# ChristophReich1996/Multi-StyleGAN

Hardware: AMD Instinct MI355X
Metric: training images/sec (G+D step, 256^2, seq=3x2ch) (higher is better)
Workload: dtype bf16

## Files before the change

### include/msg_hip.h

```cpp
#ifndef MSG_HIP_H
#define MSG_HIP_H

#ifdef __cplusplus
extern "C" {
#endif

enum { MSG_OK = 0, MSG_EINVAL = -1, MSG_EUNSUPPORTED = -2, MSG_ELAUNCH = -3 };
enum { MSG_F32 = 0, MSG_BF16 = 1, MSG_F16 = 2, MSG_F64 = 3, MSG_F32_SPLIT = 4 };

#define MSG_ABI_VERSION 5
int msg_abi_version(void);
const char* msg_build_arch(void);
const char* msg_strerror(int code);

int msg_upfirdn2d(const void* x, const float* fir, void* y, int dtype,
                  int major, int in_h, int in_w, int minor, int kh, int kw,
                  int up_x, int up_y, int down_x, int down_y,
                  int pad_x0, int pad_x1, int pad_y0, int pad_y1, void* stream);

int msg_upfirdn2d_pitched(const void* x, const float* fir, void* y, int dtype,
                          int major, int in_h, int in_w, int minor, int in_pitch, int kh, int kw,
                          int up_x, int up_y, int down_x, int down_y,
                          int pad_x0, int pad_x1, int pad_y0, int pad_y1, void* stream);

int msg_upfirdn2d_pitched2(const void* x, const float* fir, void* y, int dtype,
                           int major, int in_h, int in_w, int minor, int in_pitch, int out_pitch, int kh, int kw,
                           int up_x, int up_y, int down_x, int down_y,
                           int pad_x0, int pad_x1, int pad_y0, int pad_y1, void* stream);

int msg_upfirdn2d_separable(const void* x, const float* fir_y, const float* fir_x, void* y, int dtype,
                            int major, int in_h, int in_w, int minor, int kh, int kw,
                            int pad_x0, int pad_x1, int pad_y0, int pad_y1, void* stream);

int msg_upfirdn2d_separable_act(const void* x, const float* fir_y, const float* fir_x, void* y, int dtype,
                                int major, int in_h, int in_w, int minor, int kh, int kw,
                                int pad_x0, int pad_x1, int pad_y0, int pad_y1,
                                const float* act_bias, const float* noise, const float* noise_weight,
                                int noise_batch, float alpha, float scale, void* stream);
int msg_upfirdn2d_separable_act_mask(const void* x, const float* fir_y, const float* fir_x, void* y, int dtype,
                                     int major, int in_h, int in_w, int minor, int kh, int kw,
                                     int pad_x0, int pad_x1, int pad_y0, int pad_y1,
                                     const float* act_bias, const float* noise, const float* noise_weight,
                                     int noise_batch, float alpha, float scale, unsigned char* mask, void* stream);

int msg_fused_bias_act(const void* x, const float* bias, const void* ref, void* y, int dtype,
                       long long size_x, int step_b, int size_b,
                       const float* noise, const float* noise_weight, int noise_batch, int pix,
                       int act, int grad, float alpha, float scale, void* stream);

long long msg_bias_act_backward_workspace(long long size_x, int step_b, int size_b, int has_noise);
int msg_bias_act_backward(const void* gy, const void* out, void* gx, int dtype,
                          long long size_x, int step_b, int size_b,
                          float* grad_bias, const float* noise, float* grad_noise_weight,
                          int noise_batch, int pix, float alpha, float scale,
                          float* ws, long long ws_floats, void* stream);
int msg_channel_sums(const void* x, float* sums, int dtype, long long size_x, int C, float* ws, long long ws_floats,
                     void* stream);
int msg_bias_act_backward_mask(const void* gy, const unsigned char* mask, int tile_m, int tile_n, void* gx, int dtype,
                               long long size_x, int size_b,
                               float* grad_bias, const float* noise, float* grad_noise_weight,
                               int noise_batch, int pix, float alpha, float scale,
                               float* ws, long long ws_floats, void* stream);
int msg_sum_rows(const float* part, float* out, long long rows, int cols, void* stream);
int msg_bias_act_backward_mask_head(const void* gy, const void* ghead, const float* whead, const float* style,
                                    float wscale, int n_head, const unsigned char* mask, int tile_m, int tile_n,
                                    void* gx, int dtype, long long size_x, int size_b,
                                    float* grad_bias, const float* noise, float* grad_noise_weight,
                                    int noise_batch, int pix, float alpha, float scale,
                                    float* ws, long long ws_floats, void* stream);

int msg_conv2d_fprop(const void* x, const void* w, const float* bias, void* y, int dtype,
                     int B, int IH, int IW, int Cx, int Ck, int OH, int OW, int N, int ldy,
                     int kh, int kw, int stride, int pad, int in_up, int pixel_shuffle,
                     long long w_batch_stride, void* stream);
enum { MSG_WGRAD_K_AUTO = -1 };
int msg_conv2d_wgrad(const void* gy, const void* x, float* gw, int dtype,
                     int B, int IH, int IW, int Cx, int I, int OH, int OW, int ldgy, int O, int ldgw,
                     int kh, int kw, int stride, int pad, int pixel_shuffle,
                     int per_sample, int k_chunks, int oi_major, float gain,
                     float* ws, long long ws_floats, void* stream);
long long msg_conv2d_wgrad_workspace(int dtype, int B, int IH, int IW, int Cx, int I, int OH, int OW, int ldgy,
                                     int O, int ldgw, int kh, int kw, int stride, int pad, int pixel_shuffle,
                                     int per_sample, int k_chunks);

int msg_demod_coeff(const float* W, const float* s, float* d, int B, int O, int I, int taps,
                    float scale, float eps, void* stream);
int msg_scale_rows_cols(const float* base, const float* rowscale, const float* colscale, void* out,
                        int dtype, int B, int R, int T, int C, int Ck, float gain, void* stream);
int msg_modulate_weights(const float* base, const float* wsq, const float* style, void* out, float* d_out,
                         int dtype, int B, int R, int O, int T, int C, int Ck, float scale, float eps, void* stream);
int msg_modulate_backward(const float* gwk, const float* W, const float* s, const float* d, float* gW,
                          float* gs_part, int B, int O, int I, int taps, int ldg, int o_group,
                          float scale, void* stream);
int msg_scale_rows_cols2(const float* base, const float* row1, const float* col1, const float* row2, const float* col2,
                         void* out, int dtype, int B, int R, int T, int C, int Ck, float gain, void* stream);
int msg_modulate_backward2(const float* gwk, const float* W, const float* s, const float* d, const float* v,
                           float* gW, float* gs_part, int B, int O, int I, int taps, int ldg, int o_group,
                           float scale, void* stream);

int msg_relayout_weight(const float* w, void* fwd, void* dgrad, float* wsq, int dtype,
                        int O, int I, int T, int Ck, int Ok, int flip, int t_major, float gain, void* stream);

int msg_gather_taps(const void* x, void* y, int dtype, int B, int H, int W, int Cx, int C, int kh, int kw,
                    int pad, int Ko, void* stream);
int msg_fold_taps(const void* g, const void* add, void* gx, int dtype, int B, int H, int W, int Ko, int C, int kh, int kw,
                  int pad, int ldx, int ld_add, void* stream);

int msg_scaled_add(const void* a, const void* b, void* y, int dtype, long long n, float beta, float gain, void* stream);
int msg_rgb_skip_merge(const void* conv, int dtype, int ld, const float* bias, const float* skip, const float* fir,
                       float* out, int B, int C, int H, int W, void* stream);
int msg_rgb_skip_merge_backward(const float* g, void* g_conv, int dtype, int ld, float* g_skip, const float* fir,
                                int B, int C, int H, int W, void* stream);
int msg_gamma_merge(const void* a, const void* b, const float* gamma, void* y, int dtype, long long n, float gain, void* stream);
long long msg_gamma_merge_backward_workspace(void);
int msg_gamma_merge_backward(const void* gy, const void* a, const float* gamma, void* ga, void* gb, float* g_gamma, int dtype,
                             long long n, float gain, float* ws, void* stream);
int msg_scaled_add_rows(const void* a, const void* b, void* y, int dtype, long long rows, int cols,
                        long long lda, long long ldb, long long ldy, float beta, float gain, void* stream);

int msg_softmax_rows(const void* x, void* y, int dtype, long long rows, int cols, void* stream);
int msg_softmax_rows_backward(const void* y, const void* gy, void* gx, int dtype, long long rows, int cols,
                              void* stream);
int msg_softmax_rows_backward2(const void* y, const void* gy, const void* v, void* d_y, void* d_gy, int dtype,
                               long long rows, int cols, void* stream);

int msg_nonlocal_attention_supported(int B, int Nq, int Nk, int dk, int dv);
int msg_nonlocal_attention_fwd(const void* q, const void* k, const void* vt, void* o, float* lse, int dtype,
                               int B, int Nq, int Nk, int dk, int dv, void* stream);
int msg_maxpool2x2_fwd(const void* x, void* y, unsigned short* idx, int dtype, int B, int H, int W, int C, long long ldx,
                       void* stream);
int msg_maxpool2x2_bwd(const void* gy, const unsigned short* idx, void* gx, int dtype, int B, int H, int W, int C,
                       void* stream);
int msg_maxpool2x2_gather(const void* v, const unsigned short* idx, void* out, int dtype, int B, int H, int W, int C,
                          long long ldv, void* stream);

int msg_nonlocal_attention_bwd_splits(int B, int Nq, int Nk);
int msg_nonlocal_attention_bwd(const void* q, const void* qt, const void* k, const void* kt, const void* v,
                               const void* dO, const void* dOt, const void* o, const float* lse, float* delta,
                               void* dq, void* dk_out, void* dv_out, float* workspace, int dtype,
                               int B, int Nq, int Nk, int dk, int dv, void* stream);

int msg_affine_warp(const float* x, float* y, const float* angle_deg, float angle_const, const float* scale_xy,
                    const float* select_u, const float* p, int rot_prob, float cx, float cy, int padding,
                    int align_corners, int B, int C, int H, int W, int backward, void* workspace, void* stream);

long long msg_minibatch_stddev_workspace(int C, int H, int W, int groups, int dtype);
int msg_minibatch_stddev(const void* x, void* y, float* stat, float* workspace, int dtype,
                         int B, int C, int H, int W, int ldx, int ldy, int groups, float alpha, void* stream);
int msg_minibatch_stddev_backward(const void* x, const void* gy, const float* gstat, void* gx, int dtype,
                                  int B, int C, int H, int W, int ldx, int ldgy, int ldgx, int groups,
                                  float alpha, void* stream);

int msg_conv2d_fprop_act(const void* x, const void* w, void* y, int dtype,
                         int B, int IH, int IW, int Cx, int Ck, int OH, int OW, int N, int ldy,
                         int kh, int kw, int stride, int pad, long long w_batch_stride,
                         const float* act_bias, const float* noise, const float* noise_weight,
                         int noise_batch, float alpha, float scale, void* stream);
int msg_conv2d_fprop_act_mask(const void* x, const void* w, void* y, int dtype,
                              int B, int IH, int IW, int Cx, int Ck, int OH, int OW, int N, int ldy,
                              int kh, int kw, int stride, int pad, long long w_batch_stride,
                              const float* act_bias, const float* noise, const float* noise_weight,
                              int noise_batch, float alpha, float scale, unsigned char* mask, void* stream);

int msg_conv2d_fprop_residual(const void* x, const void* w, void* y, int dtype,
                              int B, int IH, int IW, int Cx, int Ck, int OH, int OW, int N, int ldy,
                              int kh, int kw, int stride, int pad, long long w_batch_stride,
                              const void* residual, int res_ld, float gain, void* stream);

int msg_conv2d_fprop_act_backward(const void* x, const void* w, void* y, int dtype,
                                  int B, int IH, int IW, int Cx, int Ck, int OH, int OW, int N, int ldy,
                                  int kh, int kw, int stride, int pad, long long w_batch_stride,
                                  const void* residual, int res_ld,
                                  const unsigned char* sign_mask, int mask_tile_m, int mask_tile_n,
                                  const void* sign_map, int sign_ld, float alpha, float scale,
                                  float* grad_bias, const float* noise, int noise_batch, float* grad_noise_weight,
                                  float* ws, long long ws_floats, void* stream);

int msg_act_pointwise_head(const void* x, const float* bias, const float* w, float* y, int dtype,
                           long long npix, int C, float wscale, float alpha, float scale, void* stream);
long long msg_act_pointwise_head_backward_workspace(long long npix, int C);
int msg_act_pointwise_head_backward(const void* x, const float* bias, const float* w, const float* gy, void* gx,
                                    float* grad_bias_and_w, int dtype, long long npix, int C, float wscale,
                                    float alpha, float scale, float* ws, long long ws_floats, void* stream);

int msg_linear_fprop(const float* x, const float* w, const float* bias, float* y, int M, int N, int K,
                     float gain, float bias_gain, void* stream);
int msg_linear_dgrad(const float* gy, const float* w, float* gx, int M, int N, int K, float gain, void* stream);
int msg_linear_wgrad(const float* gy, const float* x, float* gw, float* gb, int M, int N, int K,
                     float gain, float bias_gain, void* stream);

int msg_linear_grouped_fprop(const float* x, const int* slot, const float* const* w, const float* const* bias, float* y,
                             int G, int M, int N, int K, int L, float gain, float bias_gain, void* stream);
int msg_linear_grouped_dgrad(const float* gy, const float* const* w, float* gx, int G, int M, int N, int K, float gain,
                             void* stream);
int msg_linear_grouped_wgrad(const float* gy, const float* x, const int* slot, float* gw, float* gb, int G, int M, int N,
                             int K, int L, float gain, float bias_gain, void* stream);
int msg_linear_grouped_wgrad_ptrs(const float* gy, const float* x, const int* slot, float* const* gw, float* const* gb, int G,
                                  int M, int N, int K, int L, float gain, float bias_gain, void* stream);

enum {
    MSG_PLAN_REG = 0,
    MSG_PLAN_DMA = 1,
    MSG_PLAN_PP = 2,
    MSG_PLAN_ROW3 = 3,
    MSG_PLAN_ROW3N = 4,
    MSG_PLAN_THIN = 5,
    MSG_PLAN_UPCONV = 6,
    MSG_FPLAN_FIELDS = 5
};
int msg_conv2d_fprop_launch_plan(int dtype, int B, int IH, int IW, int Cx, int Ck, int OH, int OW, int N, int ldy,
                                 int kh, int kw, int stride, int pad, int in_up, int pixel_shuffle,
                                 long long w_batch_stride, int has_bias, int epilogue, long long* out, int n_out_fields);
enum {
    MSG_WPLAN_GENERIC = 0,
    MSG_WPLAN_DMA = 1,
    MSG_WPLAN_UNI = 2,
    MSG_WPLAN_ROW3 = 3,
    MSG_WPLAN_ROW3_W32 = 4,
    MSG_WPLAN_FIELDS = 11
};
int msg_conv2d_wgrad_plan(int dtype, int B, int IH, int IW, int Cx, int I, int OH, int OW, int ldgy,
                          int O, int ldgw, int kh, int kw, int stride, int pad, int pixel_shuffle,
                          int per_sample, int k_chunks, long long* out, int n_out_fields);
int msg_conv2d_fprop_plan(int dtype, int B, int IH, int IW, int Cx, int Ck, int OH, int OW, int N,
                          int kh, int kw, long long w_batch_stride);
long long msg_conv2d_fprop_act_backward_workspace(int dtype, int B, int IH, int IW, int Cx, int Ck, int OH, int OW,
                                                  int N, int kh, int kw, long long w_batch_stride, int has_noise);
int msg_conv2d_fprop_upconv_eligible(int B, int IH, int IW, int Cx, int Ck, int OH, int OW, int N, int kh, int kw,
                                     int stride, int pad, int in_up, int pixel_shuffle, long long w_batch_stride);
int msg_conv2d_fprop_thin_eligible(int B, int IH, int IW, int Cx, int Ck, int OH, int OW, int N, int ldy, int kh, int kw,
                                   int stride, int pad, int in_up, int pixel_shuffle, int act_mode);

int msg_flat_adam(float* param, const float* grad, float* exp_avg, float* exp_avg_sq, float* ema, long long n,
                  const float* coef, float lr, float beta1, float beta2, float eps, int step, float ema_decay,
                  void* stream);
int msg_flat_ema(float* ema, const float* param, long long n, float decay, void* stream);

long long msg_tlfm_prepare_workspace(int B, int T);
int msg_tlfm_prepare(const unsigned short* raw, const unsigned char* hflip, void* out, int dtype,
                     int B, int C, int T, int H, int W, int vflip,
                     float lo1, float div1, float lo2, float div2,
                     unsigned int* ws, void* stream);

int msg_tlfm_frame_range(const unsigned short* frames, long long N, int H, int W,
                         unsigned int* range, void* stream);
int msg_tlfm_gather(const unsigned short* frames, const unsigned int* range, long long N,
                    const int* index, const unsigned char* hflip, void* out, int dtype,
                    int B, int C, int T, int H, int W, int vflip,
                    float lo1, float div1, float lo2, float div2, void* stream);

int msg_sample_sheet(const void* seq, unsigned char* out, int dtype,
                     int B, int C, int T, int H, int W, int tints, void* stream);

enum { MSG_GAN_LOGISTIC = 0, MSG_GAN_WASSERSTEIN = 1, MSG_GAN_HINGE = 2 };
enum { MSG_GAN_AUX_NONE = 0, MSG_GAN_AUX_WEIGHT = 1, MSG_GAN_AUX_LABEL = 2 };
long long msg_gan_loss_workspace(long long n_real, long long n_fake);
int msg_gan_loss(const void* pred_real, const void* pred_fake, const float* aux, float* out, int dtype, int kind,
                 int aux_mode, long long n_real, long long n_fake, long long P, float* ws, long long ws_floats,
                 void* stream);
int msg_gan_loss_backward(const void* pred_real, const void* pred_fake, const float* aux, const float* grad_out,
                          void* grad_real, void* grad_fake, int dtype, int kind, int aux_mode,
                          long long n_real, long long n_fake, long long P, void* stream);

#define MSG_ELASTIC_MAX_SIGMA 32
long long msg_elastic_workspace(int B, int H, int W);
int msg_elastic_deform(const void* in, const float* noise, float* field, void* out, int dtype,
                       int B, int F, int H, int W, int sigma, float alpha, void* ws, void* stream);

#ifdef __cplusplus
}
#endif
#endif
```

### multi_stylegan_amd/build.py

```python
import glob
import os
import shutil
import subprocess
import sys

HERE = os.path.dirname(os.path.abspath(__file__))
CSRC = os.path.join(HERE, "csrc")
LIB = os.path.join(HERE, "libmsg_hip.so")
ARCH = "gfx950"


def _hipcc():
    return shutil.which("hipcc") or "/opt/rocm/bin/hipcc"


def sources():
    return sorted(glob.glob(os.path.join(CSRC, "*.hip")))


def lib_path(variant=None):
    return LIB if not variant else os.path.join(HERE, f"libmsg_hip_{variant}.so")


def is_stale(variant=None):
    lib = lib_path(variant)
    if not os.path.exists(lib):
        return True
    t = os.path.getmtime(lib)
    deps = sources() + glob.glob(os.path.join(CSRC, "*.h")) + [os.path.join(HERE, "..", "include", "msg_hip.h")]
    return any(os.path.getmtime(d) > t for d in deps)


def build(force=False, verbose=True, extra_flags=(), variant=None):
    lib = lib_path(variant)
    if not force and not is_stale(variant):
        build_fastcall(verbose=verbose)
        return lib
    objs = []
    objdir = os.path.join(HERE, "build" if not variant else f"build_{variant}")
    os.makedirs(objdir, exist_ok=True)
    procs = []
    for src in sources():
        obj = os.path.join(objdir, os.path.basename(src) + ".o")
        deps = [src] + glob.glob(os.path.join(CSRC, "*.h"))
        objs.append(obj)
        if not force and os.path.exists(obj) and all(os.path.getmtime(obj) > os.path.getmtime(d) for d in deps):
            continue
        cmd = [_hipcc(), "-O3", "-std=c++17", f"--offload-arch={ARCH}", "-fPIC", "-c", src, "-o", obj,
               "-Wno-unused-result", *extra_flags, *os.environ.get("MSG_EXTRA_HIPCC_FLAGS", "").split()]
        if verbose:
            print(" ".join(cmd), flush=True)
        procs.append((src, subprocess.Popen(cmd)))
    for src, pr in procs:
        if pr.wait() != 0:
            raise RuntimeError(f"hipcc failed on {src}")
    cmd = [_hipcc(), "-shared", "-fPIC", f"--offload-arch={ARCH}", "-o", lib, *objs]
    if verbose:
        print(" ".join(cmd), flush=True)
    subprocess.check_call(cmd)
    build_fastcall(force=force, verbose=verbose)
    return lib


FASTCALL = os.path.join(HERE, "_msg_fastcall.so")


def build_fastcall(force=False, verbose=True):
    import sysconfig
    gen = os.path.join(HERE, "csrc_host", "gen_fastcall.py")
    deps = [gen, os.path.join(HERE, "_lib.py"), os.path.join(HERE, "..", "include", "msg_hip.h")]
    if not force and os.path.exists(FASTCALL) and all(os.path.getmtime(FASTCALL) > os.path.getmtime(d) for d in deps):
        return FASTCALL
    sys.path.insert(0, os.path.dirname(HERE))
    try:
        from multi_stylegan_amd import _lib
        from multi_stylegan_amd.csrc_host.gen_fastcall import generate
    finally:
        sys.path.pop(0)
    objdir = os.path.join(HERE, "build")
    os.makedirs(objdir, exist_ok=True)
    src = os.path.join(objdir, "msg_fastcall.c")
    with open(src, "w") as f:
        f.write(generate(_lib._SIGNATURES))
    cmd = [shutil.which("gcc") or "gcc", "-O2", "-shared", "-fPIC", f"-I{sysconfig.get_paths()['include']}", src, "-o", FASTCALL, "-ldl"]
    if verbose:
        print(" ".join(cmd), flush=True)
    subprocess.check_call(cmd)
    return FASTCALL


if __name__ == "__main__":
    import argparse
    ap = argparse.ArgumentParser()
    ap.add_argument("--force", action="store_true")
    ap.add_argument("--variant", default=None)
    ap.add_argument("--flags", default="", help="extra hipcc flags, e.g. --flags=-DMSG_TUNING")
    a = ap.parse_args()
    print(build(force=a.force, extra_flags=tuple(a.flags.split()), variant=a.variant))
```

### multi_stylegan_amd/conv_ops.py

```python
import ctypes
import functools
import math
import os
from typing import Optional, Tuple

import torch
from torch.autograd import Function

from . import _lib
from ._autograd import _derive


def _vec(dtype) -> int:
    return 8 if dtype == torch.bfloat16 else 4


def _round_up(n: int, m: int) -> int:
    return (n + m - 1) // m * m


def _padded_nhwc(b, c, h, w, dtype, device):
    cx = _round_up(c, _vec(dtype))
    buf = torch.empty((b, h, w, cx), dtype=dtype, device=device)
    if cx != c:
# ... 197 lines not shown
            offs[(ph, e - u)] = t0 + 2 * u
    dmin = min(d for _, d in offs)
    dmax = max(d for _, d in offs)
    taps = dmax - dmin + 1
    table = [[offs.get((ph, tau + dmin), -1) for tau in range(taps)] for ph in (0, 1)]
    return taps, -dmin, table


def _relay_dgrad_s2(w: torch.Tensor, dtype, pad: int) -> Tuple[torch.Tensor, int, int, int]:
    *lead, o, i, kh, kw = w.shape
    assert kh == kw
    taps, pad2, table = _s2_plan(kh, pad)
    ok = _round_up(o, 128 // (2 if dtype == torch.bfloat16 else 4))
    src = [[(table[ph][th] * kw + table[pw][tw]) if table[ph][th] >= 0 and table[pw][tw] >= 0 else kh * kw
            for th in range(taps) for tw in range(taps)] for ph in (0, 1) for pw in (0, 1)]
    idx = torch.tensor(src, dtype=torch.long, device=w.device)
    wt = w.transpose(-4, -3).reshape(*lead, i, o, kh * kw)
    wz = torch.cat([wt, wt.new_zeros((*lead, i, o, 1))], dim=-1)
    picked = wz[..., idx]
    n = len(lead)
    picked = picked.permute(*range(n), n + 2, n, n + 3, n + 1)
    out = torch.zeros((*lead, 4, i, taps * taps, ok), dtype=dtype, device=w.device)
    out[..., :o] = picked
    return out.reshape(*lead, 4 * i, taps * taps, ok), ok, taps, pad2


_WEIGHT_GENERATION = [0]


def invalidate_weight_cache(params=None) -> None:
    if params is None:
        _WEIGHT_GENERATION[0] += 1
        return
    for p in params:
        p.__dict__["_msg_gen"] = p.__dict__.get("_msg_gen", 0) + 1


def _after_optimizer_step(optimizer, *_args, **_kwargs) -> None:
    for group in optimizer.param_groups:
        invalidate_weight_cache(group["params"])


def _stamp(w):
    return (w._version, _WEIGHT_GENERATION[0], w.__dict__.get("_msg_gen", 0), w.data_ptr())


from torch.optim.optimizer import register_optimizer_step_post_hook as _register_step_hook

_register_step_hook(_after_optimizer_step)


def _cached(w, tag, dtype, wscale, build):
    if not isinstance(w, torch.nn.Parameter):
        out = build()
        return (out[0] * wscale, *out[1:]) if wscale != 1.0 else out
    store = w.__dict__.setdefault("_msg_relay", {})
    key = (tag, dtype, wscale)
    stamp = _stamp(w)
    hit = store.get(key)
    if hit is not None and hit[0] == stamp:
        return hit[1]
    with torch.no_grad():
        out = build()
        if wscale != 1.0:
            out = (out[0] * wscale, *out[1:])
    store[key] = (stamp, out)
    return out


def _param_images(w, dtype, gain, kind, modulation=False):
    key = ("img", dtype, gain, kind, modulation)
    store = w.__dict__.get("_msg_relay")
    if store is not None:
        hit = store.get(key)
        if hit is not None and hit[0] == (w._version, _WEIGHT_GENERATION[0], w.__dict__.get("_msg_gen", 0), w.data_ptr()):
            return hit[1]
    if not (isinstance(w, torch.nn.Parameter) and w.is_cuda and w.dtype == torch.float32):
        return None
    o, i = _oi(w)
    t = w.numel() // (o * i)
    if t > 16 or w.numel() != o * i * t:
        return None
    store = w.__dict__.setdefault("_msg_relay", {})
    stamp = _stamp(w)
    dev = w.device
    unit = 1 if modulation else 128 // (2 if dtype == torch.bfloat16 else 4)
    ck, ok = _round_up(i, unit), _round_up(o, unit)
    up2 = kind == "up2"
    with torch.no_grad():
        w3 = w.detach().reshape(o, i, t).contiguous()
        fwd = torch.empty((t * o, 1, ck) if up2 else (o, t, ck), dtype=dtype, device=dev)
        dgr = torch.empty((i, t, ok), dtype=dtype, device=dev)
        wsq = torch.empty((o, i), dtype=torch.float32, device=dev) if modulation else None
        with _lib.on_device(dev):
            code = _lib.lib().msg_relayout_weight(w3.data_ptr(), fwd.data_ptr(), dgr.data_ptr(), _lib.ptr(wsq),
                                                  _lib.dtype_code(fwd), o, i, t, ck, ok, int(not up2), int(up2),
                                                  float(gain), _lib.stream_of(dev))
        _lib.check(code, "msg_relayout_weight")
    out = {"f": (fwd, ck), "d": (dgr, ok), "wsq": wsq}
    store[key] = (stamp, out)
    return out


_CLOCK_SHAPES = bool(int(os.environ.get("MSG_CLOCK_SHAPES", "0")))

FP32_CONTRACTION = "exact"
MSG_F32_SPLIT = _lib.MSG_F32_SPLIT
_SPLIT_CODES = {"split_bf16x3": MSG_F32_SPLIT}


class fp32_contraction:

    def __init__(self, mode: str):
        if mode not in ("exact", "split_bf16x3"):
            raise ValueError(f"fp32 contraction mode {mode!r}: 'exact' or 'split_bf16x3'")
        self.mode, self.prev = mode, None

    def __enter__(self):
        global FP32_CONTRACTION
        self.prev, FP32_CONTRACTION = FP32_CONTRACTION, self.mode
        return self

    def __exit__(self, *exc):
        global FP32_CONTRACTION
        FP32_CONTRACTION = self.prev
        return False

    @staticmethod
    def set(mode: str) -> None:
        fp32_contraction(mode).__enter__()


def _contraction_code(t: torch.Tensor, mode: Optional[str] = None) -> int:
    code = _lib.dtype_code(t)
    mode = FP32_CONTRACTION if mode is None else mode
    return _SPLIT_CODES[mode] if (code == _lib.MSG_F32 and mode != "exact") else code


_PLANS = {_lib.MSG_PLAN_REG: ("conv_fprop_reg", None), _lib.MSG_PLAN_DMA: ("conv_fprop_dma", None),
          _lib.MSG_PLAN_PP: ("conv_fprop_pp", None), _lib.MSG_PLAN_ROW3: ("conv_fprop_row3", 256),
          _lib.MSG_PLAN_ROW3N: ("conv_fprop_row3n", 128), _lib.MSG_PLAN_THIN: ("conv_fprop_thin", None),
          _lib.MSG_PLAN_UPCONV: ("conv_fprop_upconv", None)}


@functools.lru_cache(maxsize=None)
def _fprop_plan(*args):
    out = (ctypes.c_longlong * _lib.MSG_FPLAN_FIELDS)()
    ok = _lib.lib().msg_conv2d_fprop_launch_plan(*args, ctypes.addressof(out), len(out)) == _lib.MSG_OK
    kernel = out[0] if ok else None
    return (kernel,) + _PLANS.get(kernel, ("conv_fprop", None)) + (out[3] * args[8], out[4])


@functools.lru_cache(maxsize=None)
def _wgrad_plan(*geom):
    out = (ctypes.c_longlong * _lib.MSG_WPLAN_FIELDS)()
    _lib.check(_lib.lib().msg_conv2d_wgrad_plan(*geom, _lib.MSG_WGRAD_K_AUTO, ctypes.addressof(out), len(out)),
               "msg_conv2d_wgrad_plan")
    return out[10], out[1]


def _launch_fprop(x, wk, ck, bias, n, out_hw, kh, kw, stride, pad, in_up, pixel_shuffle, per_sample, c_real,
                  flops=None, act=None, residual=None, out=None, mode=None):
    dev = _lib.require_gpu(x, wk, bias)
    xv, cx = _nhwc_view(x)
    b, _, ih, iw = xv.shape
    oh, ow = out_hw
    if out is not None:
        y, ldy = _nhwc_view(out)
        if y is not out or pixel_shuffle or out.shape != (b, n, oh, ow) or out.dtype != x.dtype or n % _vec(x.dtype):
            raise _lib.MsgHipError(f"conv fprop: destination {tuple(out.shape)} / {out.stride()} for a {(b, n, oh, ow)} result")
    elif pixel_shuffle:
        y, ldy = _alloc_out(b, n // 4, 2 * oh, 2 * ow, x.dtype, dev)
    else:
        y, ldy = _alloc_out(b, n, oh, ow, x.dtype, dev)
    rows_needed = n * (1 if pixel_shuffle else kh * kw) * ck
    if per_sample:
        ws_ = wk.stride() if wk.ndim == 4 else None
        if ws_ is None or wk.shape[0] != b or ws_[0] < rows_needed or ws_[3] != 1 or \
                (wk.shape[2] > 1 and ws_[2] != wk.shape[3]) or (wk.shape[1] > 1 and ws_[1] != wk.shape[2] * wk.shape[3]):
            raise _lib.MsgHipError(f"conv fprop: per-sample weight image {tuple(wk.shape)} for batch {b}, {n} x {kh * kw} x {ck}")
    elif wk.numel() < rows_needed or not wk.is_contiguous():
        raise _lib.MsgHipError(f"conv fprop: weight image {tuple(wk.shape)} smaller than {n} x {kh * kw} x {ck}")
    wstride = wk.stride(0) if per_sample else 0
    if flops is None:
        flops = 2.0 * b * oh * ow * n * kh * kw * c_real / (in_up * in_up)
    key, sign_tile = "conv_fprop", None
    sign_holder = act[5] if act is not None and len(act) > 5 else None
    if _lib.kernel_clock.enabled or sign_holder is not None:
        _, key, sign_tile, _, _ = _fprop_plan(_lib.dtype_code(x), b, ih, iw, cx, ck, oh, ow, n, ldy, kh, kw, stride, pad, in_up,
                                              int(pixel_shuffle), wstride, int(bias is not None),
                                              2 if residual is not None else int(act is not None))
    if _lib.kernel_clock.enabled and _CLOCK_SHAPES:
        key += f"|B{b} {ih}x{iw}->{oh}x{ow} {c_real}->{n} {kh}x{kw} s{stride} up{in_up}" \
               f"{' ps' if pixel_shuffle else ''}{' per-sample' if per_sample else ''}|"
    with _lib.on_device(dev), _lib.kernel_clock.span((key, 'bf16' if x.dtype == torch.bfloat16 else 'f32'), flops):
        if residual is not None:
            assert bias is None and act is None and in_up == 1 and not pixel_shuffle
            rv, res_ld = _nhwc_view(residual[0])
            assert rv.shape == (b, n, oh, ow) and rv.dtype == x.dtype
            code = _lib.lib().msg_conv2d_fprop_residual(
                xv.data_ptr(), wk.data_ptr(), y.data_ptr(), _contraction_code(x, mode), b, ih, iw, cx, ck, oh, ow, n, ldy, kh, kw,
                stride, pad, wstride, rv.data_ptr(), res_ld, float(residual[1]), _lib.stream_of(dev))
        elif act is None:
            code = _lib.lib().msg_conv2d_fprop(
                xv.data_ptr(), wk.data_ptr(), _lib.ptr(bias), y.data_ptr(), _contraction_code(x, mode), b, ih, iw, cx, ck, oh,
                ow, n, ldy, kh, kw, stride, pad, in_up, int(pixel_shuffle), wstride, _lib.stream_of(dev))
        else:
            assert bias is None and in_up == 1 and not pixel_shuffle
            act_bias, noise, noise_w, alpha, scale = act[:5]
            _lib.require_gpu(x, act_bias, noise, noise_w)
            mask = None
            if sign_holder is not None and sign_tile:
                from .op_static.fused_act import sign_mask_for
                mask = sign_mask_for(b, n, oh, ow, x.dtype, dev)
                if mask is not None:
                    sign_holder.append((mask, sign_tile, sign_tile))
            code = _lib.lib().msg_conv2d_fprop_act_mask(
                xv.data_ptr(), wk.data_ptr(), y.data_ptr(), _contraction_code(x, mode), b, ih, iw, cx, ck, oh, ow, n, ldy, kh, kw,
                stride, pad, wstride, _lib.ptr(act_bias), _lib.ptr(noise), _lib.ptr(noise_w),
                1 if noise is None else noise.shape[0], float(alpha), float(scale), _lib.ptr(mask), _lib.stream_of(dev))
    _lib.check(code, "msg_conv2d_fprop")
    return y


def _grad_dest(param):
    if param is None or "_msg_grad_slot" not in getattr(param, "__dict__", ()):
        return None
    from .dist import grad_destination
    return grad_destination(param)


def _launch_wgrad(gy, x, o, i, kh, kw, stride, pad, pixel_shuffle, per_sample, low_hw, raw=False, gain=1.0, out=None,
                  mode=None):
    dev = _lib.require_gpu(gy, x)
    gv, ldgy = _nhwc_view(gy)
    xv, cx = _nhwc_view(x)
    b, _, ih, iw = xv.shape
    oh, ow = low_hw if pixel_shuffle else gv.shape[2:]
    taps = kh * kw
    ldgw = _round_up(i, 4)
    geom = (_contraction_code(x, mode), b, ih, iw, cx, i, oh, ow, ldgy, o, ldgw, kh, kw, stride, pad, int(pixel_shuffle),
            int(per_sample))
    need, nz = _wgrad_plan(*geom)
    ws = _lib.scratch_ptr(need, dev) if need else None
    if per_sample or raw:
        out = None
    oi_major = (bool(need) or out is not None) and not per_sample and not raw
    if oi_major:
        gw = out.view(o, i, kh, kw) if out is not None else torch.empty((o, i, kh, kw), dtype=torch.float32, device=dev)
    elif per_sample:
        gw = torch.empty((b, o, taps, ldgw), dtype=torch.float32, device=dev)
    else:
        gw = torch.empty((o, taps, ldgw), dtype=torch.float32, device=dev)
    flops = 2.0 * b * oh * ow * o * i * taps
    key = "conv_wgrad"
    if _CLOCK_SHAPES and _lib.kernel_clock.enabled:
        key += f"|B{b} {ih}x{iw}->{oh}x{ow} {i}->{o} {kh}x{kw} s{stride}{' ps' if pixel_shuffle else ''}" \
               f"{' per-sample' if per_sample else ' shared'}{f' slabs{nz}' if need else ''}|"
    with _lib.on_device(dev), _lib.kernel_clock.span((key, 'bf16' if x.dtype == torch.bfloat16 else 'f32'), flops):
        code = _lib.lib().msg_conv2d_wgrad(
            gv.data_ptr(), xv.data_ptr(), gw.data_ptr(), *geom, _lib.MSG_WGRAD_K_AUTO, int(oi_major), float(gain), ws, need,
            _lib.stream_of(dev))
    _lib.check(code, "msg_conv2d_wgrad")
    if raw:
        return gw, ldgw
    if oi_major:
        return gw
    lead = gw.shape[:-2]
    return gw.view(*lead, kh, kw, ldgw)[..., :i].permute(*range(len(lead)), len(lead) + 2, len(lead), len(lead) + 1)


class Geometry:
    __slots__ = ("kind", "kh", "kw", "stride", "pad", "x_hw", "y_hw", "per_sample", "wscale", "mode")

    def __init__(self, kind, kh, kw, stride, pad, x_hw, per_sample, wscale=1.0, mode=None):
        self.kind, self.kh, self.kw, self.stride, self.pad = kind, kh, kw, stride, pad
        self.x_hw, self.per_sample, self.wscale = tuple(x_hw), per_sample, float(wscale)
        self.mode = FP32_CONTRACTION if mode is None else mode
        if kind == "up2":
            self.y_hw = (2 * x_hw[0], 2 * x_hw[1])
        else:
            self.y_hw = ((x_hw[0] + 2 * pad - kh) // stride + 1, (x_hw[1] + 2 * pad - kw) // stride + 1)


def _oi(w):
    return (w.shape[0], w.shape[1]) if w.ndim == 2 else (w.shape[-4], w.shape[-3])


def _relay_fwd_kind(w, dtype, kind):
    wk, ck = _relay_fwd(w, dtype)
    if kind == "up2":
        o = _oi(w)[0]
        wk = wk.transpose(-3, -2).reshape(*wk.shape[:-3], 4 * o, 1, ck).contiguous()
    return wk, ck


def _thin_ok(dtype, i, g: Geometry) -> bool:
    taps = g.kh * g.kw
    return g.kind == "conv" and g.stride == 1 and not g.per_sample and taps > 1 and \
        2 * g.pad + 1 == g.kh and g.kh == g.kw and i * taps <= 128 // (2 if dtype == torch.bfloat16 else 4)


def _gather_taps(x, i, g: Geometry):
    dev = _lib.require_gpu(x)
    xv, cx = _nhwc_view(x)
    b, _, h, w = xv.shape
    ko = 128 // x.element_size()
    out = torch.empty((b, h, w, ko), dtype=x.dtype, device=dev)
    with _lib.on_device(dev):
        code = _lib.lib().msg_gather_taps(xv.data_ptr(), out.data_ptr(), _lib.dtype_code(x), b, h, w, cx, i, g.kh, g.kw,
                                          g.pad, ko, _lib.stream_of(dev))
    _lib.check(code, "msg_gather_taps")
    return out.permute(0, 3, 1, 2), ko


def _relay_thin(w, dtype):
    o, i, kh, kw = w.shape
    ko = 128 // (2 if dtype == torch.bfloat16 else 4)
    out = torch.zeros((o, 1, ko), dtype=dtype, device=w.device)
    out[:, 0, :kh * kw * i] = w.permute(0, 2, 3, 1).reshape(o, kh * kw * i)
    return out, ko


def _f_raw(x, w, bias, g: Geometry, act=None, residual=None, out=None):
    if w.ndim == 4 and _thin_ok(x.dtype, w.shape[1], g):
        xc, ko = _gather_taps(x, w.shape[1], g)
        wk, _ = _cached(w, "thin", x.dtype, g.wscale, lambda: _relay_thin(w, x.dtype))
        return _launch_fprop(xc, wk, ko, bias, w.shape[0], g.y_hw, 1, 1, 1, 0, 1, False, False,
                             w.shape[1] * g.kh * g.kw, act=act, residual=residual, out=out, mode=g.mode)
    if g.kind == "up2" and _oi(w)[0] % _vec(x.dtype):
        o_real = _oi(w)[0]
        wp = torch.zeros((*w.shape[:-4], _round_up(o_real, _vec(x.dtype)), *w.shape[-3:]), dtype=w.dtype, device=w.device)
        wp[..., :o_real, :, :, :] = w.detach()
        assert out is None
        return _f_raw(x, wp, bias, g, act=act, residual=residual)[:, :o_real]
    img = _param_images(w, x.dtype, g.wscale, g.kind) if not g.per_sample else None
    wk, ck = img["f"] if img is not None else \
        _cached(w, "f" + g.kind, x.dtype, g.wscale, lambda: _relay_fwd_kind(w, x.dtype, g.kind))
    o, _ = _oi(w)
    if g.kind == "up2":
        assert out is None
        return _launch_fprop(x, wk, ck, None, 4 * o, g.x_hw, 1, 1, 1, 0, 1, True, g.per_sample, _oi(w)[1], mode=g.mode)
    return _launch_fprop(x, wk, ck, bias, o, g.y_hw, g.kh, g.kw, g.stride, g.pad, 1, False, g.per_sample, _oi(w)[1],
                         act=act, residual=residual, out=out, mode=g.mode)


def _act_operands(bias, noise, noise_w, y_shape):
    b32 = None if bias is None else bias.detach().to(torch.float32).contiguous()
    nz = nw = None
    if noise is not None:
        if noise.shape[0] not in (1, y_shape[0]) or noise.shape[1] != 1 or tuple(noise.shape[2:]) != tuple(y_shape[2:]):
            raise _lib.MsgHipError(f"noise shape {tuple(noise.shape)} does not match output {tuple(y_shape)}")
        nz = noise.detach().to(torch.float32).contiguous()
        nw = noise_w.detach().to(torch.float32).contiguous()
    return b32, nz, nw


ACT_BACKWARD_IN_DGRAD = bool(int(os.environ.get("MSG_ACT_BACKWARD_IN_DGRAD", "1")))


class ActHandle:
    __slots__ = ("armed", "sign", "alpha", "scale", "bias_param", "has_bias", "noise", "done")

    def __init__(self):
        self.armed, self.sign, self.done = False, None, None
        self.alpha = self.scale = 0.0
        self.bias_param, self.has_bias, self.noise = None, False, None

    def arm(self, y, mask, alpha, scale, bias_param, has_bias, noise):
        if not ACT_BACKWARD_IN_DGRAD or y.dtype != torch.bfloat16 or not y.is_cuda:
            return
        self.sign = ("mask",) + tuple(mask) if mask is not None else ("map",)
        self.alpha, self.scale = float(alpha), float(scale)
# ... 278 lines not shown
        y = _f_raw(x, w, None, g, act=(b32, nz, nw, alpha, scale, holder))
        ctx.mask = holder[0] if holder else None
        ctx.slot, ctx.out_scale = slot, out_scale
        ctx.act_handle = ctx.input_act = None
        if act_handle is not None and out_scale is None and noise is None and holder is not None:
            act_handle.arm(y, ctx.mask, alpha, scale, act_bias, act_bias is not None, None)
            ctx.act_handle = act_handle if act_handle.armed else None
        if input_act is not None and input_act.armed:
            ctx.input_act = input_act
        ctx.bias_param = act_bias
        ctx.g, ctx.cfg = g, (alpha, scale, act_bias is not None, noise is not None)
        ctx.nw_shape = None if noise_w is None else noise_w.shape
        ctx.save_for_backward(x, w, y, noise)
        return y

    @staticmethod
    def backward(ctx, gy):
        from .op_static.fused_act import FusedLeakyReLUFunctionBackward
        x, w, y, noise = ctx.saved_tensors
        alpha, scale, has_bias, has_noise = ctx.cfg
        g = ctx.g
        owed = 1.0
        if ctx.out_scale is not None and ctx.out_scale.pending is not None:
            owed, ctx.out_scale.pending = ctx.out_scale.pending, None
        handed = ctx.act_handle.done if ctx.act_handle is not None else None
        if handed is not None:
            ctx.act_handle.done = None
            gpre, (gb, gnw) = gy, handed
        else:
            gpre, gb, gnw = _derive(FusedLeakyReLUFunctionBackward, gy, y, noise if has_noise else None,
                                    ctx.bias_param if has_bias else False, alpha, scale * owed, ctx.mask)
        gx = None
        if ctx.needs_input_grad[0]:
            other = ctx.slot.g if ctx.slot is not None else None
            pre = ctx.input_act if not torch.is_grad_enabled() else None
            if _dgrad_add_ok(other, x.shape, gpre.dtype, g):
                gx = _derive(_ConvD, gpre, w, g, other) if torch.is_grad_enabled() else \
                    _d_raw(gpre, w, g, residual=(other, 1.0), act_bwd=pre, sign_map=x)
                ctx.slot.merged = True
            elif pre is not None:
                gx = _d_raw(gpre, w, g, act_bwd=pre, sign_map=x)
            else:
                gx = _derive(_ConvD, gpre, w, g)
        gw = _derive(_ConvG, gpre, x, _oi(w), w.ndim, g, w) if _consumed(ctx, 1, 1) else None
        return gx, gw, (gb if has_bias and ctx.needs_input_grad[2] else None), None, \
            (gnw.reshape(ctx.nw_shape) if has_noise and ctx.needs_input_grad[4] else None), None, None, None, None, None, None, None


class _ConvResidualF(Function):

    @staticmethod
    def forward(ctx, x, w, main, g, gain, fork, slot=None, main_scale=None, out=None):
        y = _f_raw(x, w, None, g, residual=(main, gain), out=out)
        if out is not None:
            y = out.view_as(out)
        ctx.slot, ctx.main_scale = slot, main_scale
        ctx.g, ctx.gain, ctx.fork = g, float(gain), fork
        ctx.save_for_backward(x, w)
        return (y, y.view_as(y)) if fork else y

    @staticmethod
    def backward(ctx, *grads):
        from .op_static.fused_act import _ScaledAddRows, _rows_ok
        x, w = ctx.saved_tensors
        g1 = grads[0]
        g2 = grads[1] if ctx.fork else None
        if (g1 is None or g2 is None) and ctx.main_scale is not None and ctx.needs_input_grad[2]:
            gs = g1 if g1 is not None else g2
            ctx.main_scale.pending = ctx.gain
            gg = Geometry(ctx.g.kind, ctx.g.kh, ctx.g.kw, ctx.g.stride, ctx.g.pad, ctx.g.x_hw, ctx.g.per_sample,
                          ctx.g.wscale * ctx.gain, mode=ctx.g.mode)
            gs_main = gs
            if torch.is_grad_enabled() and ctx.needs_input_grad[0] and RESIDUAL_FORK_NODE:
                gx, gs_main = _ConvDFork.apply(gs, w, gg)
            else:
                gx = _derive(_ConvD, gs, w, gg) if ctx.needs_input_grad[0] else None
            if ctx.slot is not None and gx is not None:
                ctx.slot.g = gx
            gw = _derive(_ConvG, gs, x, _oi(w), w.ndim, gg, w) if _consumed(ctx, 1, 1) else None
            return gx, gw, gs_main, None, None, None, None, None, None
        if g1 is None or g2 is None:
            gs = (g1 if g1 is not None else g2) * ctx.gain
        elif _rows_ok(g1, g2):
            gs = _derive(_ScaledAddRows, g1, g2, ctx.gain)
        else:
            gs = (g1 + g2) * ctx.gain
        gx = _derive(_ConvD, gs, w, ctx.g) if ctx.needs_input_grad[0] else None
        if ctx.slot is not None and gx is not None:
            ctx.slot.g = gx
        gw = _derive(_ConvG, gs, x, _oi(w), w.ndim, ctx.g, w) if _consumed(ctx, 1, 1) else None
        return gx, gw, (gs if ctx.needs_input_grad[2] else None), None, None, None, None, None, None


class _MultiConvF(Function):

    @staticmethod
    def forward(ctx, x, geoms, *weights):
        ctx.geoms = geoms
        ctx.save_for_backward(x, *weights)
        return tuple(_f_raw(x, w, None, g) for w, g in zip(weights, geoms))

    @staticmethod
    def backward(ctx, *grads):
        x, *weights = ctx.saved_tensors
        second_order = torch.is_grad_enabled()
        gx, gws = None, []
        for k, (gy, w, g) in enumerate(zip(grads, weights, ctx.geoms)):
            if gy is None:
                gws.append(None)
                continue
            if ctx.needs_input_grad[0]:
                if gx is None or not _dgrad_add_ok(gx, x.shape, gy.dtype, g):
                    part = _derive(_ConvD, gy, w, g)
                    gx = part if gx is None else gx + part
                elif second_order:
                    gx = _derive(_ConvD, gy, w, g, gx)
                else:
                    gx = _d_raw(gy, w, g, residual=(gx, 1.0))
            gws.append(_derive(_ConvG, gy, x, _oi(w), w.ndim, g, w) if _consumed(ctx, 2 + k, 1 + k) else None)
        return (gx, None, *gws)


def conv2d_shared_input(x, weights_and_scales, padding=0):
    p = _square(padding, "padding")
    geoms = tuple(Geometry("conv", w.shape[2], w.shape[3], 1, p, x.shape[2:], False, ws) for w, ws in weights_and_scales)
    return _MultiConvF.apply(x, geoms, *[w for w, _ in weights_and_scales])


class GradScale:
    __slots__ = ("pending",)

    def __init__(self):
        self.pending = None


class GradSlot:
    __slots__ = ("g", "merged")

    def __init__(self):
        self.g, self.merged = None, False


class HeadGradSlot:
    __slots__ = ("head", "dgrad", "armed")

    def __init__(self):
        self.head = None
        self.dgrad = None
        self.armed = False

    def take(self):
        head, dgrad, self.head, self.dgrad = self.head, self.dgrad, None, None
        return head, dgrad


class _ForkInput(Function):

    @staticmethod
    def forward(ctx, x, slot):
        ctx.slot = slot
        return x.view_as(x), x.view_as(x)

    @staticmethod
    def backward(ctx, g_main, g_res):
        slot = ctx.slot
        merged, slot.g, slot.merged = slot.merged, None, False
        if merged or g_res is None:
            return g_main, None
        if g_main is None:
            return g_res, None
        return g_main + g_res, None


def _square(value, what: str) -> int:
    if isinstance(value, int):
        return value
    value = tuple(value)
    if len(value) != 2 or value[0] != value[1]:
        raise _lib.MsgHipError(f"conv2d: only square {what} is implemented, got {value}")
    return int(value[0])


def fork_input(x, slot: GradSlot):
    return _ForkInput.apply(x, slot)


def conv2d_add_residual(x, weight, main, gain, stride=1, padding=0, wscale=1.0, fork=False, grad_slot=None,
                        main_grad_scale=None, out=None):
    s, p = _square(stride, "stride"), _square(padding, "padding")
    g = Geometry("conv", weight.shape[2], weight.shape[3], s, p, x.shape[2:], False, wscale)
    return _ConvResidualF.apply(x, weight, main, g, float(gain), bool(fork), grad_slot, main_grad_scale, out)


def conv2d_bias_act(x, weight, act_bias, stride=1, padding=0, wscale=1.0, negative_slope=0.2, scale=1.0,
                    grad_slot=None, out_grad_scale=None, act_handle=None, input_act=None):
    s, p = _square(stride, "stride"), _square(padding, "padding")
    g = Geometry("conv", weight.shape[2], weight.shape[3], s, p, x.shape[2:], False, wscale)
    return _ConvActF.apply(x, weight, act_bias, None, None, g, float(negative_slope), float(scale), grad_slot,
                           out_grad_scale, act_handle, input_act)


def conv2d(x, weight, bias=None, stride=1, padding=0, wscale=1.0):
    s, p = _square(stride, "stride"), _square(padding, "padding")
    g = Geometry("conv", weight.shape[2], weight.shape[3], s, p, x.shape[2:], False, wscale)
    return _ConvF.apply(x, weight, None if bias is None else bias.float(), g)


def conv_transpose2d_2x2(x, weight, bias=None, wscale=1.0):
    if tuple(weight.shape[2:]) != (2, 2):
        raise _lib.MsgHipError("conv_transpose2d_2x2: 2x2 kernel, stride 2, padding 0 only")
    g = Geometry("up2", 2, 2, 1, 1, x.shape[2:], False, wscale)
    y = _ConvF.apply(x, weight.transpose(0, 1), None, g)
    return y if bias is None else y + bias.view(1, -1, 1, 1).to(y.dtype)


_LINEAR_MAX_ROWS = 256


def _lin_call(name, flops, *args):
    dev = args[0].device
    with _lib.on_device(dev), _lib.kernel_clock.span((name, "f32"), flops):
        code = getattr(_lib.lib(), f"msg_{name}")(*[a.data_ptr() if isinstance(a, torch.Tensor) else
                                                   (0 if a is None else a) for a in args], _lib.stream_of(dev))
    _lib.check(code, f"msg_{name}")


def _dense32(*ts):
    for t in ts:
        if t is not None and t.dtype != torch.float32:
            raise _lib.MsgHipError("the few-row linear kernels are fp32 (mapping network / style affines / heads)")
    return [None if t is None else t.contiguous() for t in ts]


class _LinF(Function):

    @staticmethod
    def forward(ctx, x, w, bias, gain, bias_gain=1.0):
        _lib.require_gpu(x, w, bias)
        x, w, bias = _dense32(x, w, bias)
        (m, k), n = x.shape, w.shape[0]
        y = torch.empty((m, n), dtype=torch.float32, device=x.device)
        _lin_call("linear_fprop", 2.0 * m * n * k, x, w, bias, y, m, n, k, float(gain), float(bias_gain))
        ctx.save_for_backward(x, w)
        ctx.gain, ctx.has_bias, ctx.bias_gain = float(gain), bias is not None, float(bias_gain)
        ctx.bias_param = bias
        return y

    @staticmethod
    def backward(ctx, gy):
        x, w = ctx.saved_tensors
        need_x, need_w, need_b = ctx.needs_input_grad[:3]
        gx = _derive(_LinD, gy, w, ctx.gain) if need_x else None
        gw = gb = None
        if need_w and need_b and ctx.has_bias and not torch.is_grad_enabled():
            (gy_,) = _dense32(gy)
            (m, n), k = gy_.shape, x.shape[1]
            gw, gb = _grad_dest(w), _grad_dest(ctx.bias_param)
            gw = gw if gw is not None else torch.empty((n, k), dtype=torch.float32, device=x.device)
            gb = gb if gb is not None else torch.empty((n,), dtype=torch.float32, device=x.device)
            _lin_call("linear_wgrad", 2.0 * m * n * k, gy_, x, gw, gb, m, n, k, ctx.gain, ctx.bias_gain)
        else:
            if need_w:
                gw = _derive(_LinG, gy, x, ctx.gain)
            if need_b and ctx.has_bias:
                gb = gy.sum(dim=0) if ctx.bias_gain == 1.0 else gy.sum(dim=0) * ctx.bias_gain
        return gx, gw, gb, None, None


class _LinD(Function):

    @staticmethod
    def forward(ctx, gy, w, gain):
        _lib.require_gpu(gy, w)
        gy, w = _dense32(gy, w)
        (m, n), k = gy.shape, w.shape[1]
        gx = torch.empty((m, k), dtype=torch.float32, device=gy.device)
        _lin_call("linear_dgrad", 2.0 * m * n * k, gy, w, gx, m, n, k, float(gain))
        ctx.save_for_backward(gy, w)
        ctx.gain = float(gain)
        return gx

    @staticmethod
    def backward(ctx, g):
        gy, w = ctx.saved_tensors
        d_gy = _derive(_LinF, g, w, None, ctx.gain) if ctx.needs_input_grad[0] else None
        d_w = _derive(_LinG, gy, g, ctx.gain) if ctx.needs_input_grad[1] else None
        return d_gy, d_w, None


class _LinG(Function):

    @staticmethod
    def forward(ctx, gy, x, gain):
        _lib.require_gpu(gy, x)
        gy, x = _dense32(gy, x)
        (m, n), k = gy.shape, x.shape[1]
        gw = torch.empty((n, k), dtype=torch.float32, device=gy.device)
        _lin_call("linear_wgrad", 2.0 * m * n * k, gy, x, gw, None, m, n, k, float(gain), 1.0)
        ctx.save_for_backward(gy, x)
        ctx.gain = float(gain)
        return gw

    @staticmethod
    def backward(ctx, g):
        gy, x = ctx.saved_tensors
        d_gy = _derive(_LinF, x, g, None, ctx.gain) if ctx.needs_input_grad[0] else None
# ... 262 lines not shown
    if upsample:
        return _launch_wgrad(gy, x, o, i, 2, 2, 1, 0, True, True, g.x_hw, raw=True, mode=g.mode)
    return _launch_wgrad(gy, x, o, i, kh, kw, 1, kh // 2, False, True, None, raw=True, mode=g.mode)


def _fold_weight_gradient(gwk, ldg, w3, s, dd, scale, style_dtype, cotangent=None, dest=None):
    b = gwk.shape[0]
    o, i, t = w3.shape
    dev = gwk.device
    og = 2 if o >= 512 or o < 256 else 1
    groups = (o + og - 1) // og
    out = _grad_dest(dest) if cotangent is None else None
    gw3 = out.view(o, i, t) if out is not None else torch.empty((o, i, t), dtype=torch.float32, device=dev)
    gs_part = _lib.scratch_ptr(groups * b * i, dev)
    gs = torch.empty((b, i), dtype=torch.float32, device=dev)
    with _lib.on_device(dev):
        st = _lib.stream_of(dev)
        if cotangent is None:
            code = _lib.lib().msg_modulate_backward(gwk.data_ptr(), w3.data_ptr(), s.data_ptr(), _lib.ptr(dd),
                                                    gw3.data_ptr(), gs_part, b, o, i, t, ldg, og, scale, st)
        else:
            code = _lib.lib().msg_modulate_backward2(gwk.data_ptr(), w3.data_ptr(), s.data_ptr(), _lib.ptr(dd),
                                                     cotangent.data_ptr(), gw3.data_ptr(), gs_part, b, o, i, t,
                                                     ldg, og, scale, st)
        _lib.check(code, "msg_modulate_backward" + ("2" if cotangent is not None else ""))
        code = _lib.lib().msg_sum_rows(gs_part, gs.data_ptr(), groups, b * i, st)
    _lib.check(code, "msg_sum_rows")
    return (out if out is not None else gw3), (gs if style_dtype == torch.float32 else gs.to(style_dtype))


def _modconv_backward(x, weight, style, d, gy, demodulate, upsample, g, scale, need, keep_gwk=False, direct=False,
                      act_bwd=None):
    _, o, i, kh, kw = weight.shape
    b, t = x.shape[0], kh * kw
    dev = x.device
    w3 = weight.detach().reshape(o, i, t)
    s = style.detach().float().contiguous()
    dd = d if demodulate else None
    esz = 2 if gy.dtype == torch.bfloat16 else 4
    gx = None
    if need[0]:
        okp = _round_up(o, 128 // esz)
        wd = torch.empty((b, i, t, okp), dtype=gy.dtype, device=dev)
        _scale_rows_cols(_dgrad_image_base(weight, w3, upsample, g.kind), s, dd, wd, scale)
        gx = _dgrad_modconv(gy, wd, okp, o, i, kh, kw, upsample, g, act_bwd=act_bwd, sign_map=x)
    gw = gs = gwk = None
    if need[1] or need[2]:
        gwk, ldg = _wgrad_modconv(gy, x, o, i, kh, kw, upsample, g)
        gw3, gs = _fold_weight_gradient(gwk, ldg, w3, s, dd, scale, style.dtype, dest=weight if direct else None)
        gw = gw3.reshape(1, o, i, kh, kw)
    return (gx, gw, gs, gwk) if keep_gwk else (gx, gw, gs)


_NATIVE_SECOND_ORDER = True


def _modconv_second_order_composite(gy, x, weight, style, demodulate, upsample, a, cot_w, cot_s, want):
    with torch.enable_grad():
        leaves = [t.detach().requires_grad_(True) for t in (gy, x, weight, style)]
        y2 = _modulated_composite(leaves[1], leaves[2], leaves[3], demodulate, upsample)
        first = torch.autograd.grad(y2, leaves[1:], leaves[0], create_graph=True, allow_unused=True)
        terms = [(c.to(f.dtype) * f).sum() for c, f in zip((a, cot_w, cot_s), first) if c is not None and f is not None]
        if not terms:
            return (None, None, None, None)
        grads = torch.autograd.grad(sum(terms), leaves, allow_unused=True)
    return tuple(gr if w else None for gr, w in zip(grads, want))


class _ModConvGrad(Function):

    @staticmethod
    def forward(ctx, gy, x, weight, style, d, demodulate, upsample, g, scale, need):
        gx, gw, gs, gwk = _modconv_backward(x, weight, style, d, gy, demodulate, upsample, g, scale, need, keep_gwk=True)
        ctx.set_materialize_grads(False)
        ctx.save_for_backward(gy, x, weight, style, d, gwk)
        ctx.cfg = (demodulate, upsample, g, scale)
        return gx, gw, gs

    @staticmethod
    @torch.autograd.function.once_differentiable
    def backward(ctx, a, cot_w, cot_s):
        gy, x, weight, style, d, gwk = ctx.saved_tensors
        demodulate, upsample, g, scale = ctx.cfg
        want = ctx.needs_input_grad[:4]
        _, o, i, kh, kw = weight.shape
        b, t = x.shape[0], kh * kw
        tail = (None,) * 6
        if a is None and cot_w is None and cot_s is None:
            return (None, None, None, None) + tail
        if cot_w is not None or i % 4 or i > 512 or t not in (1, 4, 9) or b > _MODCONV_BWD_BATCH or \
                (cot_s is not None and gwk is None):
            return _modconv_second_order_composite(gy, x, weight, style, demodulate, upsample, a, cot_w, cot_s, want) + tail
        dev = x.device
        w3 = weight.detach().reshape(o, i, t)
        s = style.detach().float().contiguous()
        dd = d if demodulate else None
        esz = 2 if gy.dtype == torch.bfloat16 else 4
        ck, okp = _round_up(i, 128 // esz), _round_up(o, 128 // esz)
        rows = t * o if upsample else o
        ggy = gx2 = gw3 = gs2 = None
        if a is not None:
            a = a.to(x.dtype)
            if want[0]:
                wk = torch.empty((b, rows, 1 if upsample else t, ck), dtype=x.dtype, device=dev)
                base = _fwd_image_base(weight, w3, upsample, g.kind)
                if demodulate:
                    _scale_rows_cols(base, d.repeat(1, t) if upsample else d, s, wk, scale)
                else:
                    _scale_rows_cols(base, None, s, wk, scale)
                ggy = _fprop_modconv(a, wk, ck, o, i, kh, kw, upsample, g)
            if want[2] or want[3]:
                gwk_a, ldg = _wgrad_modconv(gy, a, o, i, kh, kw, upsample, g)
                gw3, gs2 = _fold_weight_gradient(gwk_a, ldg, w3, s, dd, scale, style.dtype)
        if cot_s is not None:
            v = cot_s.detach().float().contiguous()
            if want[0] or want[1]:
                hf = torch.empty((b, rows, 1 if upsample else t, ck), dtype=x.dtype, device=dev)
                hd = torch.empty((b, i, t, okp), dtype=gy.dtype, device=dev)
                base_f = _fwd_image_base(weight, w3, upsample, g.kind)
                base_d = _dgrad_image_base(weight, w3, upsample, g.kind)
                if demodulate:
                    wsq = _tap_square_sums(weight, w3, g.kind)
                    ddir = -(scale * scale) * d.pow(3) * linear(s * v, wsq)
                    rows_d, rows_dd = (d.repeat(1, t), ddir.repeat(1, t)) if upsample else (d, ddir)
                    with _lib.on_device(dev):
                        lib, st = _lib.lib(), _lib.stream_of(dev)
                        code = lib.msg_scale_rows_cols2(base_f.data_ptr(), rows_d.contiguous().data_ptr(), v.data_ptr(),
                                                        rows_dd.contiguous().data_ptr(), s.data_ptr(), hf.data_ptr(),
                                                        _lib.dtype_code(hf), b, rows, 1 if upsample else t, i, ck, scale, st)
                        _lib.check(code, "msg_scale_rows_cols2")
                        code = lib.msg_scale_rows_cols2(base_d.data_ptr(), v.data_ptr(), d.data_ptr(), s.data_ptr(),
                                                        ddir.contiguous().data_ptr(), hd.data_ptr(), _lib.dtype_code(hd), b, i, t,
                                                        o, okp, scale, st)
                        _lib.check(code, "msg_scale_rows_cols2")
                else:
                    _scale_rows_cols(base_f, None, v, hf, scale)
                    _scale_rows_cols(base_d, v, None, hd, scale)
                if want[0]:
                    ggy = _fprop_modconv(x, hf, ck, o, i, kh, kw, upsample, g, add_to=ggy)
                if want[1]:
                    gx2 = _dgrad_modconv(gy, hd, okp, o, i, kh, kw, upsample, g)
            if want[2] or want[3]:
                gw3b, gs2b = _fold_weight_gradient(gwk, gwk.shape[-1], w3, s, dd, scale, style.dtype, cotangent=v)
                gw3 = gw3b if gw3 is None else gw3 + gw3b
                gs2 = gs2b if gs2 is None else gs2 + gs2b
        gw = gw3.reshape(1, o, i, kh, kw) if (gw3 is not None and want[2]) else None
        return (ggy, gx2, gw, gs2 if want[3] else None) + tail


class _ModulatedConv(Function):

    @staticmethod
    def forward(ctx, x, weight, style, demodulate, upsample, act_bias=None, noise=None, noise_w=None, alpha=0.2,
                act_scale=1.0, fuse_act=False, head_slot=None, input_act=None):
        dev = _lib.require_gpu(x, weight, style)
        ctx.input_act = input_act if input_act is not None and input_act.armed else None
        ctx.head_slot = head_slot
        if head_slot is not None and fuse_act:
            ctx.set_materialize_grads(False)
            head_slot.armed = True
        _, o, i, kh, kw = weight.shape
        b, t = x.shape[0], kh * kw
        scale = math.sqrt(2.0) / math.sqrt(i * t)
        w3 = weight.detach().reshape(o, i, t)
        s = style.detach().float().contiguous()
        d = None
        esz = 2 if x.dtype == torch.bfloat16 else 4
        ck = _round_up(i, 128 // esz)
        kind = "up2" if upsample else "conv"
        img = _param_images(weight, torch.float32, 1.0, kind, modulation=True)
        base = img["f"][0] if img is not None else _cached(weight, "mb" + kind, torch.float32, 1.0, lambda: (
            (w3.permute(2, 0, 1).reshape(t * o, 1, i) if upsample else w3.transpose(1, 2)).contiguous(), 0))[0]
        rows = t * o if upsample else o
        wk = torch.empty((b, rows, 1 if upsample else t, ck), dtype=x.dtype, device=dev)
        if demodulate:
            wsq = img["wsq"] if img is not None else \
                _cached(weight, "wsq", torch.float32, 1.0, lambda: (w3.square().sum(dim=2).contiguous(), 0))[0]
            d = torch.empty((b, o), dtype=torch.float32, device=dev)
            with _lib.on_device(dev):
                code = _lib.lib().msg_modulate_weights(base.data_ptr(), wsq.data_ptr(), s.data_ptr(), wk.data_ptr(),
                                                       d.data_ptr(), _lib.dtype_code(wk), b, rows, o,
                                                       1 if upsample else t, i, ck, scale, 1e-8, _lib.stream_of(dev))
            _lib.check(code, "msg_modulate_weights")
        else:
            _scale_rows_cols(base, None, s, wk, scale)
        g = Geometry(kind, kh, kw, 1, kh // 2, x.shape[2:], True)
        act = None
        holder = [] if any(ctx.needs_input_grad) else None
        if fuse_act:
            assert not upsample, "the upsampling layers blur before their activation"
            act = (*_act_operands(act_bias, noise, noise_w, (b, o, *g.y_hw)), alpha, act_scale, holder)
        if upsample:
            y = _launch_fprop(x, wk, ck, None, 4 * o, g.x_hw, 1, 1, 1, 0, 1, True, True, i, mode=g.mode)
        else:
            y = _launch_fprop(x, wk, ck, None, o, g.y_hw, kh, kw, 1, kh // 2, 1, False, True, i, act=act, mode=g.mode)
        ctx.save_for_backward(x, weight, style, d if d is not None else torch.empty(0, device=dev),
                              y if fuse_act else None, noise if fuse_act else None)
        ctx.cfg = (demodulate, upsample, g, scale)
        ctx.act = (alpha, act_scale, act_bias is not None, noise is not None,
                   None if noise_w is None else noise_w.shape) if fuse_act else None
        ctx.bias_param = act_bias
        ctx.mask = holder[0] if holder else None
        return y

    @staticmethod
    def backward(ctx, gy):
        x, weight, style, d, y_act, noise = ctx.saved_tensors
        demodulate, upsample, g, scale = ctx.cfg
        _, o, i, kh, kw = weight.shape
        b, t = x.shape[0], kh * kw
        need = list(ctx.needs_input_grad)
        need[1], need[2] = _consumed(ctx, 1, 1), _consumed(ctx, 2, 2)
        gb = gnw = None
        slot = ctx.head_slot
        if ctx.act is not None:
            from .op_static.fused_act import FusedLeakyReLUFunctionBackward, act_backward_with_head
            alpha, act_scale, has_bias, has_noise, nw_shape = ctx.act
            head, head_dgrad = slot.take() if slot is not None else (None, None)
            fused = None
            if head is not None:
                fused = act_backward_with_head(gy, head, y_act.shape, noise if has_noise else None,
                                               ctx.bias_param if has_bias else None, has_bias, alpha, act_scale, ctx.mask)
                if fused is None:
                    gh = head_dgrad()
                    gy = gh if gy is None else gy + gh
            if fused is not None:
                gy, gb, gnw = fused
            elif gy is None:
                return (None,) * 13
            else:
                gy, gb, gnw = _derive(FusedLeakyReLUFunctionBackward, gy, y_act, noise if has_noise else None,
                                      ctx.bias_param if has_bias else False, alpha, act_scale, ctx.mask)
            gb = gb if has_bias and need[5] else None
            gnw = gnw.reshape(nw_shape) if has_noise and need[7] else None
        tail = (None, None, gb, None, gnw, None, None, None, None, None)
        if ctx.act is None and slot is not None and slot.armed and need[0] and not torch.is_grad_enabled() and \
                fused_head_ok(gy, weight, b, demodulate, upsample):
            gyc, wt, st = gy, weight, style
            slot.head = (gyc, weight.detach().reshape(o, i).float().contiguous(), style.detach().float().contiguous(), scale)
            slot.dgrad = lambda: _modconv_backward(x, wt, st, d, gyc, demodulate, upsample, g, scale,
                                                   [True, False, False])[0]
            need[0] = False
        fused_ok = i <= 512 and t <= 9
        if torch.is_grad_enabled() and fused_ok and _NATIVE_SECOND_ORDER and b <= _MODCONV_BWD_BATCH and x.is_cuda:
            gx, gw, gs = _derive(_ModConvGrad, gy, x, weight, style, d if demodulate else None, demodulate, upsample, g, scale,
                                            tuple(need[:3]))
            return (gx, gw, gs) + tail
        if torch.is_grad_enabled() or not fused_ok:
            with torch.enable_grad():
                ins = [v for v, n in zip((x, weight, style), need[:3]) if n]
                y2 = _modulated_composite(x, weight, style, demodulate, upsample)
                grads = list(torch.autograd.grad(y2, ins, gy, create_graph=torch.is_grad_enabled(), allow_unused=True))
            out = [grads.pop(0) if n else None for n in need[:3]]
            return (out[0], out[1], out[2]) + tail
        if b > _MODCONV_BWD_BATCH:
            gxs, gws, gss = [], [], []
            for lo in range(0, b, _MODCONV_BWD_BATCH):
                hi = min(b, lo + _MODCONV_BWD_BATCH)
                cgx, cgw, cgs = _modconv_backward(x[lo:hi], weight, style[lo:hi], d[lo:hi] if demodulate else d,
                                                  gy[lo:hi], demodulate, upsample, g, scale, need)
                gxs.append(cgx); gws.append(cgw); gss.append(cgs)
            gx = torch.cat(gxs) if need[0] else None
            gw = torch.stack(gws).sum(dim=0) if gws[0] is not None else None
            gs = torch.cat(gss) if gss[0] is not None else None
            return (gx, gw, gs) + tail
        gx, gw, gs = _modconv_backward(x, weight, style, d, gy, demodulate, upsample, g, scale, need, direct=True,
                                       act_bwd=ctx.input_act)
        return (gx, gw, gs) + tail


def fused_head_ok(gy, weight, b, demodulate, upsample) -> bool:
    _, o, _, kh, kw = weight.shape
    return gy is not None and gy.is_cuda and gy.dtype == torch.bfloat16 and kh == 1 and kw == 1 and o <= 8 and \
        not demodulate and not upsample and b <= _MODCONV_BWD_BATCH and HEAD_GRAD_FUSION


HEAD_GRAD_FUSION = bool(int(os.environ.get("MSG_HEAD_GRAD_FUSION", "1")))


def modulated_conv2d_bias_act(x, weight, style, demodulate, act_bias, noise, noise_weight, negative_slope=0.2,
                              scale=1.0, head_slot=None, input_act=None):
    return _ModulatedConv.apply(x, weight, style, bool(demodulate), False, act_bias, noise, noise_weight,
                                float(negative_slope), float(scale), True, head_slot, input_act)


def modulated_conv2d(x, weight, style, demodulate, upsample, head_slot=None):
    if head_slot is None:
        return _ModulatedConv.apply(x, weight, style, bool(demodulate), bool(upsample))
    return _ModulatedConv.apply(x, weight, style, bool(demodulate), bool(upsample), None, None, None, 0.2, 1.0, False,
                                head_slot)
```

### multi_stylegan_amd/csrc/conv_dispatch.h

```cpp
#pragma once
#include "msg_common.h"

struct ConvProblem {
    int dtype;
    int split;
    int B, IH, IW, Cx, Ck, OH, OW, N, ldy;
    int kh, kw, stride, pad, in_up, pixel_shuffle;
    long long w_batch_stride;

    bool per_sample() const { return w_batch_stride != 0; }
    int samples() const { return per_sample() ? B : 1; }
    long long mtot() const { return per_sample() ? (long long)OH * OW : (long long)B * OH * OW; }
    int esz() const { return dtype == MSG_BF16 ? 2 : 4; }
    long long x_bstride() const { return (long long)IH * IW * Cx; }
    long long y_bstride() const { return (pixel_shuffle ? 4ll : 1ll) * OH * OW * ldy; }
    long long x_bytes() const { return (long long)(per_sample() ? 1 : B) * IH * IW * Cx * esz(); }
    long long w_bytes() const { return (long long)N * kh * kw * Ck * esz(); }
    bool fits31() const { return x_bytes() < 0x7ffffff0ll && w_bytes() < 0x7ffffff0ll; }
};

enum ConvKernel {
    CONV_THIN_N, CONV_THIN_K,
    CONV_UPCONV,
    CONV_ROW3, CONV_ROW3N,
    CONV_PP,
    CONV_DMA, CONV_REG, CONV_REG_LEAN, CONV_REG_SPLIT
};

struct ConvPlan {
    ConvKernel kernel;
    int tile_m, tile_n;
    bool supported;
};

inline int conv_act_mode(const ActEpilogue* act) { return act ? act->enabled : 0; }

template <typename P>
inline void conv_fill_common(P& p, const ConvProblem& q, const ActEpilogue* act) {
    p.B = q.B; p.IH = q.IH; p.IW = q.IW; p.Cx = q.Cx; p.Ck = q.Ck; p.OH = q.OH; p.OW = q.OW; p.N = q.N; p.ldy = q.ldy;
    p.per_sample = q.per_sample();
    if (act) p.act = *act;
    p.x_bstride = q.x_bstride();
    p.w_bstride = q.w_batch_stride;
    p.y_bstride = q.y_bstride();
    p.Mtot = (int)q.mtot();
}
template <typename P>
inline void conv_fill_taps(P& p, const ConvProblem& q) {
    p.kh = q.kh; p.kw = q.kw; p.stride = q.stride; p.pad = q.pad; p.in_up = q.in_up; p.pixel_shuffle = q.pixel_shuffle;
}

ConvPlan conv_fprop_select(const ConvProblem& q, const ActEpilogue* act, bool has_bias);

bool conv_thin_eligible(const ConvProblem& q, const ActEpilogue* act, ConvPlan* plan);
void conv_thin_launch(const ConvProblem& q, const ConvPlan& plan, const void* x, const void* w, const float* bias, void* y,
                      const ActEpilogue* act, void* stream);
bool conv_upconv_eligible(const ConvProblem& q, const ActEpilogue* act, bool has_bias, ConvPlan* plan);
void conv_upconv_launch(const ConvProblem& q, const ConvPlan& plan, const void* x, const void* w, void* y, void* stream);
bool conv_row3_eligible(const ConvProblem& q, const ActEpilogue* act, bool has_bias, ConvPlan* plan);
void conv_row3_launch(const ConvProblem& q, const ConvPlan& plan, const void* x, const void* w, const float* bias, void* y,
                      const ActEpilogue* act, void* stream);
bool conv_pp_eligible(const ConvProblem& q, ConvPlan* plan);
void conv_pp_launch(const ConvProblem& q, const ConvPlan& plan, const void* x, const void* w, const float* bias, void* y,
                    const ActEpilogue* act, void* stream);

struct WgradProblem {
    int dtype, split;
    int B, IH, IW, Cx, I, OH, OW, ldgy, O, ldgw;
    int kh, kw, stride, pad, pixel_shuffle;
    int per_sample, k_chunks, oi_major;
    float gain;
    int esz() const { return dtype == MSG_BF16 ? 2 : 4; }
    long long gy_bytes() const { return (long long)(pixel_shuffle ? 4 : 1) * OH * OW * ldgy * esz(); }
    long long x_bytes() const { return (long long)IH * IW * Cx * esz(); }
    long long slab() const { return (long long)O * kh * kw * ldgw; }
    long long gw_zstride() const { return oi_major ? (long long)O * I * kh * kw : slab(); }
};

enum WgradKernel {
    WGRAD_GENERIC, WGRAD_DMA, WGRAD_UNI,
    WGRAD_ROW3, WGRAD_ROW3_W32
};

struct WgradPlan {
    WgradKernel kernel;
    int nz, slice_pixels;
    int chunks_per_out, n_out;
    int OWv, OHv;
    int fold, xcd_slices;
    long long blocks, need;
    bool supported;
};

struct WgradSplitModel { int round_wgs, fixed_steps, slab_steps; long long max_chunks, max_wgs; bool by8; };
inline long long conv_wgrad_ksplit(long long steps, long long wgs, const WgradSplitModel& m) {
    long long chunks = 1, best = -1;
    for (long long c = 1; c <= m.max_chunks; c += (m.by8 && c >= 8 ? 8 : 1)) {
        if (m.by8 && c > 1 && c < 8) continue;
        const long long rounds = (wgs * c + m.round_wgs - 1) / m.round_wgs;
        const long long cost = rounds * ((steps + c - 1) / c + m.fixed_steps + (c > 1 ? m.slab_steps : 0));
        if (best < 0 || cost < best) { best = cost; chunks = c; }
        if (wgs * c > m.max_wgs) break;
    }
    return chunks;
}

inline int conv_wgrad_default_chunks(const WgradProblem& q) {
    const long long kp = q.dtype == MSG_BF16 ? 64 : 32, npix = (long long)q.OH * q.OW;
    long long tiles = (long long)((q.O + 127ll) / 128) * ((q.I + 127ll) / 128);
    for (const int n : {q.kh, q.kw, q.B}) tiles = tiles < 1024 ? tiles * n : 1024;
    if (q.per_sample) {
        if (tiles >= 256) return 1;
        return (int)std::max(1ll, std::min(npix / (16 * kp), 1024 / tiles));
    }
    long long chunks = std::max(1ll, std::min((npix + 4 * kp - 1) / (4 * kp), (1024 + tiles - 1) / tiles));
    while (q.B * chunks > 65535) --chunks;
    return (int)chunks;
}

WgradPlan conv_wgrad_select(const WgradProblem& q);
bool conv_wgrad_row3_eligible(const WgradProblem& q, WgradPlan* plan);
void conv_wgrad_row3_launch(const WgradProblem& q, const WgradPlan& plan, const void* gy, const void* x, float* gw, float* ws,
                            void* stream);
```

### multi_stylegan_amd/csrc/conv_fprop.hip

```cpp
#include "conv_dispatch.h"
#include <stdlib.h>

typedef __bf16 bf16v8 __attribute__((ext_vector_type(8)));
typedef const __attribute__((address_space(1))) char* gptr_t;
typedef const __attribute__((address_space(1))) u32x4* gvec_t;
typedef __attribute__((address_space(3))) char* lds_t;

struct ConvParams {
    int B, IH, IW, Cx, Ck, OH, OW, N, ldy;
    int kh, kw, stride, pad, in_up, pixel_shuffle, per_sample;
    long long x_bstride, w_bstride, y_bstride;
    int Mtot, n_chunks, n_iters, m_tiles, n_tiles;
    ActEpilogue act;
};

constexpr int BM = 128, BN = 128, ROWB = 128;
constexpr int STAGE_BYTES = (BM + BN) * ROWB;
__device__ __attribute__((aligned(256))) unsigned int g_zero_page[16384];

__device__ __forceinline__ int swz(int row, int slot) { return row * ROWB + ((slot ^ ((row >> 1) & 7)) << 4); }

template <int SPLIT>
__device__ __forceinline__ void split_park(const u32x4& raw, char* dst) {
    uint2 pl[3];
// ... 324 lines not shown
        const bool want_noise = p.act.enabled == 1 && p.act.noise;
        const float nw = want_noise ? p.act.noise_w[0] : 0.f;
        if (p.act.enabled == 1) {
#pragma unroll
            for (int e = 0; e < VEC; ++e) a_bias[e] = (p.act.bias && n + e < p.N) ? p.act.bias[n + e] : 0.f;
        }
#pragma unroll
        for (int pass = 0; pass < NPASS; ++pass) {
            const bool ok = m0 + wm * 64 + pass * RPP + er < p.Mtot;
            const int pix = oh * p.OW + ow;
            const int g = p.pixel_shuffle ? ((b * 2 * p.OH + 2 * oh + (q >> 1)) * (2 * p.OW) + 2 * ow + (q & 1))
                                          : b * ohw + pix;
            gp[pass] = ok ? g : -1;
            a_noise[pass] = (want_noise && ok) ? nw * p.act.noise[(long long)(p.act.noise_batch == 1 ? 0 : b) * ohw + pix] : 0.f;
            ow += RPP;
            while (ow >= p.OW) { ow -= p.OW; ++oh; }
            if (!p.per_sample) while (oh >= p.OH) { oh -= p.OH; ++b; }
        }
    }
    __syncthreads();
    u32x4 v[NPASS];
#pragma unroll
    for (int pass = 0; pass < NPASS; ++pass) {
        const int row = pass * RPP + er;
        if constexpr (sizeof(T) == 2)
            v[pass] = *reinterpret_cast<const u32x4*>(ep + row * PITCH + (((lane & 7) ^ ((row & 15) >> 1)) << 4));
        else
            v[pass] = *reinterpret_cast<const u32x4*>(ep + row * PITCH + (((lane & 15) ^ (row & 15)) << 4));
    }
    if constexpr (sizeof(T) == 2) {
        if (er & 1) {
#pragma unroll
            for (int pass = 0; pass < NPASS; ++pass) v[pass] = u32x4{v[pass][2], v[pass][3], v[pass][0], v[pass][1]};
        }
    }
    if (p.act.enabled == 1) {
#pragma unroll
        for (int pass = 0; pass < NPASS; ++pass) v[pass] = act_epilogue_apply<T>(v[pass], a_bias, a_noise[pass], p.act.alpha, p.act.scale);
    } else if (p.act.enabled == 2) {
        const T* rbase = reinterpret_cast<const T*>(p.act.residual) + (n_ok ? n : 0);
        u32x4 r[NPASS];
#pragma unroll
        for (int pass = 0; pass < NPASS; ++pass)
            r[pass] = *reinterpret_cast<const u32x4*>(rbase + (long long)max(gp[pass], 0) * p.act.res_ld);
#pragma unroll
        for (int pass = 0; pass < NPASS; ++pass) v[pass] = residual_epilogue_apply<T>(v[pass], r[pass], p.act.res_gain);
    }
    T* ybase = y + (p.pixel_shuffle ? nn : n);
    if (n_ok && lim >= VEC) {
#pragma unroll
        for (int pass = 0; pass < NPASS; ++pass)
            if (gp[pass] >= 0) *reinterpret_cast<u32x4*>(ybase + (long long)gp[pass] * p.ldy) = v[pass];
    } else if (n_ok) {
#pragma unroll
        for (int pass = 0; pass < NPASS; ++pass) {
            if (gp[pass] < 0) continue;
            T tmp[VEC];
            *reinterpret_cast<u32x4*>(tmp) = v[pass];
            T* dst = ybase + (long long)gp[pass] * p.ldy;
            for (int e = 0; e < lim; ++e) dst[e] = tmp[e];
        }
    }
}

static ConvPlan conv_generic_select(const ConvProblem& q) {
    const int n_iters = q.kh * q.kw * (q.Ck / (ROWB / q.esz()));
    static const int variant = msg_tunable("MSG_CONV_VARIANT", 0);
    const bool dma = q.fits31() && (variant == 1 || (variant == 0 && n_iters >= 8));
    static const int lean_max = msg_tunable("MSG_CONV_LEAN", 4);
    ConvPlan plan{CONV_REG, BM, BN, true};
    if (q.split) plan.kernel = CONV_REG_SPLIT;
    else if (dma) plan.kernel = CONV_DMA;
    else if (q.dtype == MSG_BF16 && n_iters <= lean_max) plan.kernel = CONV_REG_LEAN;
    const long long mtot = q.mtot(), blocks = ((mtot + BM - 1) / BM) * ((q.N + BN - 1) / BN);
    plan.supported = mtot < (1ll << 31) && blocks < (1ll << 31) &&
                     (long long)(n_iters + 1) * ROWB + 128 <= 65536;
    return plan;
}

static void conv_generic_launch(const ConvProblem& q, const ConvPlan& plan, const void* x, const void* w, const float* bias, void* y,
                                const ActEpilogue* act, void* stream) {
    ConvParams p{};
    conv_fill_common(p, q, act);
    conv_fill_taps(p, q);
    p.n_chunks = q.Ck / (ROWB / q.esz());
    p.n_iters = q.kh * q.kw * p.n_chunks;
    p.m_tiles = (int)((q.mtot() + BM - 1) / BM);
    p.n_tiles = (q.N + BN - 1) / BN;
    dim3 grid((unsigned)((long long)p.m_tiles * p.n_tiles), 1, q.samples());
#define GENERIC(T, ...) hipLaunchKernelGGL((conv_fprop_kernel<T, __VA_ARGS__>), grid, dim3(256), 0, (hipStream_t)stream, \
                                           (const T*)x, (const T*)w, (T*)y, bias, p)
    const bool bf16 = q.dtype == MSG_BF16;
    if (bf16 && plan.kernel == CONV_REG_LEAN) GENERIC(bf16_t, false, 3);
    else if (bf16 && plan.kernel == CONV_DMA) GENERIC(bf16_t, true);
    else if (bf16) GENERIC(bf16_t, false);
    else if (plan.kernel == CONV_REG_SPLIT) GENERIC(float, false, 0, 3);
    else if (plan.kernel == CONV_DMA) GENERIC(float, true);
    else GENERIC(float, false);
#undef GENERIC
}

ConvPlan conv_fprop_select(const ConvProblem& q, const ActEpilogue* act, bool has_bias) {
    ConvPlan plan;
    if (conv_thin_eligible(q, act, &plan)) return plan;
    if (conv_upconv_eligible(q, act, has_bias, &plan)) return plan;
    if (conv_row3_eligible(q, act, has_bias, &plan)) return plan;
    if (conv_pp_eligible(q, &plan)) return plan;
    return conv_generic_select(q);
}

static ConvProblem conv_problem(int dtype, int B, int IH, int IW, int Cx, int Ck, int OH, int OW, int N, int ldy,
                                int kh, int kw, int stride, int pad, int in_up, int pixel_shuffle, long long w_batch_stride) {
    const int split = dtype == MSG_F32_SPLIT ? 3 : 0;
    return ConvProblem{split ? (int)MSG_F32 : dtype, split, B, IH, IW, Cx, Ck, OH, OW, N, ldy, kh, kw, stride, pad, in_up, pixel_shuffle,
                       w_batch_stride};
}

static ConvPlan fprop_select(const ConvProblem& q, int act_mode, bool has_bias) {
    ActEpilogue act{};
    act.enabled = act_mode;
    return conv_fprop_select(q, &act, has_bias);
}

static int fprop_check(const ConvProblem& q, const void* const* io) {
    if (q.B < 0 || q.IH <= 0 || q.IW <= 0 || q.OH <= 0 || q.OW <= 0 || q.N <= 0 || q.kh <= 0 || q.kw <= 0 || q.stride <= 0 ||
        q.in_up <= 0 || q.Cx <= 0 || q.Ck <= 0 || q.ldy <= 0 || (io && (!io[0] || !io[1] || !io[2])))
        return MSG_EINVAL;
    if (q.dtype != MSG_F32 && q.dtype != MSG_BF16) return MSG_EUNSUPPORTED;
    const int vec = 16 / q.esz(), bke = ROWB / q.esz();
    if (q.Ck % bke || q.Cx % vec || (io && (((uintptr_t)io[0] | (uintptr_t)io[1] | (uintptr_t)io[2]) & 15u))) return MSG_EUNSUPPORTED;
    if (q.ldy % vec || (q.pixel_shuffle && (q.N % 4 || (q.N / 4) % vec))) return MSG_EUNSUPPORTED;
    if (q.in_up > 1 && q.stride != 1) return MSG_EUNSUPPORTED;
    return MSG_OK;
}

static int fprop_plan_for(const ConvProblem& q, int act_mode, bool has_bias, const void* const* io, ConvPlan* plan) {
    if (q.B == 0) return MSG_OK;
    const int rc = fprop_check(q, io);
    if (rc != MSG_OK) return rc;
    *plan = fprop_select(q, act_mode, has_bias);
    return plan->supported ? MSG_OK : MSG_EUNSUPPORTED;
}

static bool is_row3(const ConvPlan& plan) { return plan.kernel == CONV_ROW3 || plan.kernel == CONV_ROW3N; }

static void act_backward_partials(const ConvProblem& q, const ConvPlan& plan, long long* rows, long long* entries) {
    *rows = *entries = 0;
    if (!is_row3(plan) || q.ldy != q.N) return;
    const long long tiles = (q.mtot() / plan.tile_m) * q.samples();
    *rows = tiles * 2;
    *entries = tiles * (q.N / plan.tile_n) * 4;
}

static int plan_code(ConvKernel kernel) {
    switch (kernel) {
        case CONV_THIN_N: case CONV_THIN_K: return MSG_PLAN_THIN;
        case CONV_UPCONV: return MSG_PLAN_UPCONV;
        case CONV_ROW3: return MSG_PLAN_ROW3;
        case CONV_ROW3N: return MSG_PLAN_ROW3N;
        case CONV_PP: return MSG_PLAN_PP;
        case CONV_DMA: return MSG_PLAN_DMA;
        default: return MSG_PLAN_REG;
    }
}

extern "C" int msg_conv2d_fprop_launch_plan(int dtype, int B, int IH, int IW, int Cx, int Ck, int OH, int OW, int N, int ldy,
                                            int kh, int kw, int stride, int pad, int in_up, int pixel_shuffle,
                                            long long w_batch_stride, int has_bias, int epilogue, long long* out, int n_out_fields) {
    if (epilogue < 0 || epilogue > 3 || (epilogue && (has_bias || in_up != 1 || pixel_shuffle))) return MSG_EINVAL;
    const ConvProblem q = conv_problem(dtype, B, IH, IW, Cx, Ck, OH, OW, N, ldy, kh, kw, stride, pad, in_up, pixel_shuffle, w_batch_stride);
    ConvPlan plan;
    const int rc = fprop_plan_for(q, epilogue, has_bias != 0, nullptr, &plan);
    if (rc != MSG_OK) return rc;
    long long fields[MSG_FPLAN_FIELDS] = {};
    if (q.B) {
        fields[0] = plan_code(plan.kernel); fields[1] = plan.tile_m; fields[2] = plan.tile_n;
        if (epilogue == 3) act_backward_partials(q, plan, &fields[3], &fields[4]);
    }
    for (int k = 0; k < MSG_FPLAN_FIELDS && k < n_out_fields; ++k) out[k] = fields[k];
    return MSG_OK;
}

static ConvProblem conv_query_problem(int dtype, int B, int IH, int IW, int Cx, int Ck, int OH, int OW, int N, int kh, int kw,
                                      long long w_batch_stride) {
    return conv_problem(dtype, B, IH, IW, Cx, Ck, OH, OW, N, N <= 8 ? 8 : (N + 7) / 8 * 8, kh, kw, 1, kh / 2, 1, 0, w_batch_stride);
}
extern "C" int msg_conv2d_fprop_plan(int dtype, int B, int IH, int IW, int Cx, int Ck, int OH, int OW, int N,
                                     int kh, int kw, long long w_batch_stride) {
    return plan_code(fprop_select(conv_query_problem(dtype, B, IH, IW, Cx, Ck, OH, OW, N, kh, kw, w_batch_stride), 0, false).kernel);
}
extern "C" long long msg_conv2d_fprop_act_backward_workspace(int dtype, int B, int IH, int IW, int Cx, int Ck, int OH, int OW,
                                                             int N, int kh, int kw, long long w_batch_stride, int has_noise) {
    const ConvProblem q = conv_query_problem(dtype, B, IH, IW, Cx, Ck, OH, OW, N, kh, kw, w_batch_stride);
    long long rows, entries;
    act_backward_partials(q, fprop_select(q, 3, false), &rows, &entries);
    return rows ? rows * N + (has_noise ? entries : 0) : 0;
}
extern "C" int msg_conv2d_fprop_upconv_eligible(int B, int IH, int IW, int Cx, int Ck, int OH, int OW, int N, int kh, int kw,
                                                int stride, int pad, int in_up, int pixel_shuffle, long long w_batch_stride) {
    return fprop_select(conv_problem(MSG_BF16, B, IH, IW, Cx, Ck, OH, OW, N, N / 4, kh, kw, stride, pad, in_up, pixel_shuffle,
                                     w_batch_stride), 0, false).kernel == CONV_UPCONV;
}
extern "C" int msg_conv2d_fprop_thin_eligible(int B, int IH, int IW, int Cx, int Ck, int OH, int OW, int N, int ldy,
                                              int kh, int kw, int stride, int pad, int in_up, int pixel_shuffle,
                                              int act_mode) {
    const ConvKernel kernel = fprop_select(conv_problem(MSG_BF16, B, IH, IW, Cx, Ck, OH, OW, N, ldy, kh, kw, stride, pad, in_up,
                                                        pixel_shuffle, 0), act_mode, false).kernel;
    return kernel == CONV_THIN_N ? 1 : kernel == CONV_THIN_K ? 2 : 0;
}

static int conv2d_fprop_impl(const void* x, const void* w, const float* bias, void* y, const ConvProblem& q,
                             const ActEpilogue& act, void* stream) {
    const void* const io[3] = {x, w, y};
    ConvPlan plan;
    const int rc = fprop_plan_for(q, act.enabled, bias != nullptr, io, &plan);
    if (rc != MSG_OK || q.B == 0) return rc;
    if (act.mask && !is_row3(plan)) return MSG_EUNSUPPORTED;
    switch (plan.kernel) {
        case CONV_THIN_N: case CONV_THIN_K: conv_thin_launch(q, plan, x, w, bias, y, &act, stream); break;
        case CONV_UPCONV: conv_upconv_launch(q, plan, x, w, y, stream); break;
        case CONV_ROW3: case CONV_ROW3N: conv_row3_launch(q, plan, x, w, bias, y, &act, stream); break;
        case CONV_PP: conv_pp_launch(q, plan, x, w, bias, y, &act, stream); break;
        case CONV_DMA: case CONV_REG: case CONV_REG_LEAN: case CONV_REG_SPLIT:
            conv_generic_launch(q, plan, x, w, bias, y, &act, stream); break;
    }
    return MSG_CHECK_LAUNCH();
}

extern "C" int msg_conv2d_fprop(const void* x, const void* w, const float* bias, void* y, int dtype,
                                int B, int IH, int IW, int Cx, int Ck, int OH, int OW, int N, int ldy,
                                int kh, int kw, int stride, int pad, int in_up, int pixel_shuffle,
                                long long w_batch_stride, void* stream) {
    ActEpilogue act{};
    return conv2d_fprop_impl(x, w, bias, y, conv_problem(dtype, B, IH, IW, Cx, Ck, OH, OW, N, ldy, kh, kw, stride, pad, in_up,
                                                         pixel_shuffle, w_batch_stride), act, stream);
}

extern "C" int msg_conv2d_fprop_act_mask(const void* x, const void* w, void* y, int dtype,
                                         int B, int IH, int IW, int Cx, int Ck, int OH, int OW, int N, int ldy,
                                         int kh, int kw, int stride, int pad, long long w_batch_stride,
                                         const float* act_bias, const float* noise, const float* noise_weight,
                                         int noise_batch, float alpha, float scale, unsigned char* mask, void* stream) {
    if (noise && (!noise_weight || (noise_batch != 1 && noise_batch != B))) return MSG_EINVAL;
    ActEpilogue act{act_bias, noise, noise_weight, noise_batch, 1, alpha, scale, nullptr, 0, 0.f, mask};
    return conv2d_fprop_impl(x, w, nullptr, y, conv_problem(dtype, B, IH, IW, Cx, Ck, OH, OW, N, ldy, kh, kw, stride, pad, 1, 0,
                                                            w_batch_stride), act, stream);
}

extern "C" int msg_conv2d_fprop_act(const void* x, const void* w, void* y, int dtype,
                                    int B, int IH, int IW, int Cx, int Ck, int OH, int OW, int N, int ldy,
                                    int kh, int kw, int stride, int pad, long long w_batch_stride,
                                    const float* act_bias, const float* noise, const float* noise_weight,
                                    int noise_batch, float alpha, float scale, void* stream) {
    return msg_conv2d_fprop_act_mask(x, w, y, dtype, B, IH, IW, Cx, Ck, OH, OW, N, ldy, kh, kw, stride, pad, w_batch_stride,
                                     act_bias, noise, noise_weight, noise_batch, alpha, scale, nullptr, stream);
}

extern "C" int msg_conv2d_fprop_residual(const void* x, const void* w, void* y, int dtype,
                                         int B, int IH, int IW, int Cx, int Ck, int OH, int OW, int N, int ldy,
                                         int kh, int kw, int stride, int pad, long long w_batch_stride,
                                         const void* residual, int res_ld, float gain, void* stream) {
    if (!residual || res_ld < N || (((uintptr_t)residual) & 15u) || res_ld % (dtype == MSG_BF16 ? 8 : 4)) return MSG_EINVAL;
    ActEpilogue act{};
    act.enabled = 2; act.residual = residual; act.res_ld = res_ld; act.res_gain = gain;
    return conv2d_fprop_impl(x, w, nullptr, y, conv_problem(dtype, B, IH, IW, Cx, Ck, OH, OW, N, ldy, kh, kw, stride, pad, 1, 0,
                                                            w_batch_stride), act, stream);
}

extern "C" int msg_conv2d_fprop_act_backward(const void* x, const void* w, void* y, int dtype,
                                             int B, int IH, int IW, int Cx, int Ck, int OH, int OW, int N, int ldy,
                                             int kh, int kw, int stride, int pad, long long w_batch_stride,
                                             const void* residual, int res_ld,
                                             const unsigned char* sign_mask, int mask_tile_m, int mask_tile_n,
                                             const void* sign_map, int sign_ld, float alpha, float scale,
                                             float* grad_bias, const float* noise, int noise_batch, float* grad_noise_weight,
                                             float* ws, long long ws_floats, void* stream) {
    if (B == 0) return MSG_OK;
    if (!sign_mask == !sign_map) return MSG_EINVAL;
    const ConvProblem q = conv_problem(dtype, B, IH, IW, Cx, Ck, OH, OW, N, ldy, kh, kw, stride, pad, 1, 0, w_batch_stride);
    const void* const io[3] = {x, w, y};
    ConvPlan plan;
    const int rc = fprop_plan_for(q, 3, false, io, &plan);
    if (rc != MSG_OK) return rc;
    long long rows, entries;
    act_backward_partials(q, plan, &rows, &entries);
    if (!rows) return MSG_EUNSUPPORTED;
    if (sign_mask && (mask_tile_m <= 0 || mask_tile_n <= 0 || mask_tile_n % 128 || N % mask_tile_n || (((uintptr_t)sign_mask) & 15u) ||
                      (mask_tile_m != 1 && mask_tile_m % 64) || ((long long)B * OH * OW) % mask_tile_m))
        return MSG_EINVAL;
    if (sign_map && (sign_ld < N || sign_ld % 8 || (((uintptr_t)sign_map) & 15u))) return MSG_EINVAL;
    if (residual && (res_ld < N || res_ld % 8 || (((uintptr_t)residual) & 15u))) return MSG_EINVAL;
    const bool has_noise = noise && grad_noise_weight;
    if (has_noise && noise_batch != 1 && noise_batch != B) return MSG_EINVAL;
    const long long need_b = grad_bias ? rows * N : 0, need_n = has_noise ? entries : 0;
    if (need_b + need_n > 0 && (!ws || ws_floats < need_b + need_n)) return MSG_EINVAL;
    ActEpilogue act{};
    act.enabled = 3; act.alpha = alpha; act.scale = scale;
    act.residual = residual; act.res_ld = res_ld; act.res_gain = 1.f;
    act.mask = const_cast<unsigned char*>(sign_mask); act.mask_tile_m = mask_tile_m; act.mask_tile_n = mask_tile_n;
    act.sign_src = sign_map; act.sign_ld = sign_ld;
    act.noise = has_noise ? noise : nullptr; act.noise_batch = noise_batch;
    act.part_b = grad_bias ? ws : nullptr;
    act.part_n = has_noise ? ws + need_b : nullptr;
    conv_row3_launch(q, plan, x, w, nullptr, y, &act, stream);
    if (MSG_CHECK_LAUNCH() != MSG_OK) return MSG_ELAUNCH;
    return msg_bias_act_reduce_launch(act.part_b, grad_bias, N, rows, act.part_n, grad_noise_weight, entries, stream);
}
```

### multi_stylegan_amd/csrc/conv_fprop_row3.hip

```cpp
#include "conv_dispatch.h"
#include <stdlib.h>
#include <type_traits>

typedef __bf16 bf16v8 __attribute__((ext_vector_type(8)));
typedef __attribute__((address_space(3))) char* lds_t;

struct ConvParamsR3 {
    int B, IH, IW, Cx, Ck, OH, OW, N, ldy;
    int per_sample, seg_len, n_seg;
    long long x_bstride, w_bstride, y_bstride;
    int Mtot, n_chunks, n_iters, m_tiles, n_tiles;
    int seg_magic;
    int ow_shift, ohw_shift;
    ActEpilogue act;
};

constexpr int HROW = 128;
constexpr int H_OOB = (int)0x80000000;

#ifdef MSG_ROW3_STAMPS
__device__ unsigned long long g_row3_stamps[256 * 4 * 3 * 8];
#define R3_STAMP(k) do { if (it >= 9 && it < 12 && L + 256 >= gridDim.x && blockIdx.z == gridDim.z - 1 && lane == 0) { unsigned long long tt; \
    asm volatile("s_memtime %0\n\ts_waitcnt lgkmcnt(0)" : "=s"(tt) :: "memory"); \
    g_row3_stamps[(((L + 256 - gridDim.x) * 4 + wid_u) * 3 + (it - 9)) * 8 + (k)] = tt; } } while (0)
extern "C" int msg_row3_debug_read(void* host_dst, int nbytes) {
    return hipMemcpyFromSymbol(host_dst, HIP_SYMBOL(g_row3_stamps), nbytes) == hipSuccess ? 0 : -1;
}
__device__ unsigned long long g_row3_clock[256 * 4 * 8];
#define R3_CLOCK(k) do { if (L + 256 >= gridDim.x && blockIdx.z == gridDim.z - 1 && lane == 0) { unsigned long long tc, tr; \
    const unsigned cl_ = L + 256 - gridDim.x; \
    asm volatile("s_memtime %0\n\ts_memrealtime %1\n\ts_waitcnt lgkmcnt(0)" : "=s"(tc), "=s"(tr) :: "memory"); \
    g_row3_clock[(cl_ * 4 + wid_u) * 8 + 2 * (k)] = tc; g_row3_clock[(cl_ * 4 + wid_u) * 8 + 2 * (k) + 1] = tr; } } while (0)
extern "C" int msg_row3_clock_read(void* host_dst, int nbytes) {
    return hipMemcpyFromSymbol(host_dst, HIP_SYMBOL(g_row3_clock), nbytes) == hipSuccess ? 0 : -1;
}
#else
#define R3_STAMP(k) do {} while (0)
#define R3_CLOCK(k) do {} while (0)
#endif

template <int MI, int NCOLB, bool S16, int EPI = 0>
__global__ __launch_bounds__(256, MI == 2 ? 2 : 1) void conv_fprop_row3_kernel(const bf16_t* __restrict__ x, const bf16_t* __restrict__ w,
                                                                 bf16_t* __restrict__ y, const float* __restrict__ bias,
                                                                 ConvParamsR3 p) {
    constexpr int VEC = 8, ESZ = 2;
    constexpr int HN = 64 * NCOLB, HB = HN * HROW, WN = 32 * NCOLB;
    constexpr int NBP = 2 * NCOLB;
    constexpr int HM = 64 * MI, WM = 32 * MI;
    constexpr int NAP = 2 * MI;
    constexpr int HA = (HM + 8) * HROW;
#if defined(MSG_ROW3_NO_STAGGER)
    constexpr bool STAGGER = false;
#else
    constexpr bool STAGGER = true;
#endif
    constexpr int EP_OFF = 2 * HA + 2 * HB;
    constexpr int SIGN_OFF = EP_OFF + (HM + HN) * 4;
    __shared__ __attribute__((aligned(16))) char smem[SIGN_OFF + (EPI == 1 ? HM * (HN / 8) : 0)];
    float* const ep_noise = reinterpret_cast<float*>(smem + EP_OFF);
    float* const ep_bias = ep_noise + HM;

    const int tid = threadIdx.x, lane = tid & 63, wid = tid >> 6;
    const int wid_u = __builtin_amdgcn_readfirstlane(wid);
    const int wm = wid_u >> 1, wn = wid_u & 1;
    constexpr int BLK = S16 ? 16 : 32;
    constexpr int NSUB = S16 ? 2 : 4, SLOTS = S16 ? 4 : 2;
    constexpr int NA = WM / BLK, NB = WN / BLK;
    const int lr = lane & (BLK - 1), lh = lane / BLK;
    const unsigned L = xcd_remap(blockIdx.x, gridDim.x);
    const int n0 = (int)(L % p.n_tiles) * HN;
    const int m0 = (int)(L / p.n_tiles) * HM;
    const int bz = blockIdx.z;
    const int ohw = p.OH * p.OW;
    const int seg = p.seg_len;
    R3_CLOCK(0);
    if (p.act.enabled == 1 || (EPI == 1 && p.act.noise)) {
        const bool want_noise = p.act.noise != nullptr;
        const float nw = EPI == 1 ? 1.f : (want_noise ? p.act.noise_w[0] : 0.f);
        for (int t = tid; t < HM; t += 256) {
            const int m = m0 + t;
            const bool ok = want_noise && m < p.Mtot;
            const int mm = ok ? m : 0;
            long long idx = p.per_sample ? (long long)(p.act.noise_batch == 1 ? 0 : bz) * ohw + mm : (long long)mm;
            if (!p.per_sample && p.act.noise_batch == 1) idx = p.ohw_shift >= 0 ? mm & (ohw - 1) : mm % ohw;
            ep_noise[t] = ok ? nw * p.act.noise[idx] : 0.f;
        }
        if (EPI == 0)
            for (int t = tid; t < HN; t += 256) ep_bias[t] = (p.act.bias && n0 + t < p.N) ? p.act.bias[n0 + t] : 0.f;
    }
    if constexpr (EPI == 1) {
        if (p.act.mask) {
            constexpr int UPR = HN / 128;
            const int vpt = p.act.mask_tile_n >> 3, ntn = p.N / p.act.mask_tile_n;
            for (int t = tid; t < HM * UPR; t += 256) {
                const int row = t / UPR, un = t - row * UPR;
                const long long qg = (p.per_sample ? (long long)bz * ohw : 0) + m0 + row;
                const int cvg = (n0 >> 3) + 16 * un;
                const long long trow = qg / p.act.mask_tile_m;
                const int tn = cvg / vpt;
                const unsigned char* src = p.act.mask +
                    ((trow * ntn + tn) * p.act.mask_tile_m + (qg - trow * p.act.mask_tile_m)) * vpt + (cvg - tn * vpt);
                *reinterpret_cast<u32x4*>(smem + SIGN_OFF + row * (HN / 8) + 16 * un) = *reinterpret_cast<const u32x4*>(src);
            }
        }
    }

    const int slot_phys = lane & 7;
    const char* xb = (const char*)x + (p.per_sample ? (long long)bz * p.x_bstride * ESZ : 0);
    const char* wb = (const char*)w + (p.per_sample ? (long long)bz * p.w_bstride * ESZ : 0);
    const __amdgpu_buffer_rsrc_t rs_a = __builtin_amdgcn_make_buffer_rsrc((void*)xb, 0, 0x7ffffff0, 0x00020000);
    const __amdgpu_buffer_rsrc_t rs_b = __builtin_amdgcn_make_buffer_rsrc((void*)wb, 0, 0x7ffffff0, 0x00020000);
    int a_b32[NAP + 1];
    unsigned a_flags = 0;
    auto piece_offsets = [&](auto pow2_tag) __attribute__((always_inline)) {
        constexpr bool POW2 = decltype(pow2_tag)::value;
#pragma unroll
        for (int j = 0; j < NAP + 1; ++j) {
            const int row = (j < NAP ? wid * (HM / 4) + 8 * j : HM) + (lane >> 3);
            const int sl = slot_phys ^ ((row >> 1) & 7);
            const int s = (row * p.seg_magic) >> 16, pos = row - s * (seg + 2);
            const int inner = min(max(pos - 1, 0), seg - 1);
            const int m = m0 + s * seg + inner;
            bool ok = (s < p.n_seg) & (m < p.Mtot) & (j < NAP || wid == 0);
            const int mm = ok ? m : 0;
            int b, pix, oh, ow;
            if (POW2) {
                b = p.per_sample ? 0 : mm >> p.ohw_shift;
                pix = p.per_sample ? mm : mm & (ohw - 1);
                oh = pix >> p.ow_shift, ow = pix & (p.OW - 1);
            } else {
                b = p.per_sample ? 0 : mm / ohw;
                pix = p.per_sample ? mm : mm - b * ohw;
                oh = pix / p.OW, ow = pix - oh * p.OW;
            }
            const int iw = ow + (pos == 0 ? -1 : (pos == seg + 1 ? 1 : 0));
            ok = ok & ((unsigned)iw < (unsigned)p.IW);
            a_flags |= (ok ? 1u : 0u) << j | (oh == 0 ? 1u : 0u) << (9 + j) | (oh == p.IH - 1 ? 1u : 0u) << (18 + j);
            a_b32[j] = (int)(((long long)b * p.x_bstride + sl * VEC) * ESZ) + ((oh - 1) * p.IW + iw) * p.Cx * ESZ;
        }
    };
    if (p.ow_shift >= 0) piece_offsets(std::true_type{});
    else piece_offsets(std::false_type{});
    static_assert(NAP + 1 <= 9, "flag bits");
    int vb2[2];
#pragma unroll
    for (int j = 0; j < 2; ++j) {
        const int wrow = wid * (WN / 2) + 8 * j + (lane >> 3);
        const int slb = slot_phys ^ ((wrow >> 1) & 7);
        vb2[j] = (int)(((long long)(n0 + wrow) * 9 * p.Ck + slb * VEC) * ESZ);
    }
    const int w_piece2 = 16 * 9 * p.Ck * ESZ;
    int va[NAP + 1];
    auto set_kh = [&](int kh) __attribute__((always_inline)) {
        const int tap_off = kh * p.IW * p.Cx * ESZ;
        const unsigned bad = kh >= 3 ? ~0u : (~a_flags | (kh == 0 ? a_flags >> 9 : 0u) | (kh == 2 ? a_flags >> 18 : 0u));
#pragma unroll
        for (int j = 0; j < NAP + 1; ++j) va[j] = ((bad >> j) & 1u) ? H_OOB : a_b32[j] + tap_off;
    };
    auto dma_a = [&](int j, int abuf, int chunk) __attribute__((always_inline)) {
        if (j == NAP && wid_u != 0) return;
        lds_t la = (lds_t)(smem + abuf * HA + (j < NAP ? wid_u * (HM / 4) + 8 * j : HM) * HROW);
#if defined(__HIP_DEVICE_COMPILE__)
        __builtin_amdgcn_raw_ptr_buffer_load_lds(rs_a, la, 16, va[j], chunk * HROW, 0, 0);
#endif
    };
    auto dma_b = [&](int j, int bbuf, int tap, int chunk, bool live) __attribute__((always_inline)) {
        lds_t la = (lds_t)(smem + 2 * HA + bbuf * HB + (wid_u * (WN / 2) + 8 * j) * HROW);
#if defined(__HIP_DEVICE_COMPILE__)
        __builtin_amdgcn_raw_ptr_buffer_load_lds(rs_b, la, 16, live ? vb2[j & 1] : H_OOB,
                                                 (tap * p.n_chunks + chunk) * HROW + (j >> 1) * w_piece2, 0, 0);
#endif
    };

    typedef float accv_t __attribute__((ext_vector_type(S16 ? 4 : 16)));
    accv_t acc[NA][NB];
#pragma unroll
    for (int i = 0; i < NA; ++i)
#pragma unroll
        for (int j = 0; j < NB; ++j)
#pragma unroll
            for (int e = 0; e < (S16 ? 4 : 16); ++e) acc[i][j][e] = 0.f;

    set_kh(0);
#pragma unroll
    for (int j = 0; j < NAP + 1; ++j) dma_a(j, 0, 0);
#pragma unroll
    for (int j = 0; j < NBP; ++j) dma_b(j, 0, 0, 0, true);

    int seg_of[MI];
#pragma unroll
    for (int i = 0; i < MI; ++i) seg_of[i] = (wm * WM + i * 32) / seg;
    const int sxb = (lr >> 1) & 7;
    const int fb_base = 2 * HA + (wn * WN + lr) * HROW;

    struct Pos { int kh, chunk, kw; };
    auto k_loop = [&](auto wv_tag) __attribute__((always_inline)) {
        constexpr int WV = decltype(wv_tag)::value;
        constexpr int RPG = 3;
        constexpr int ACT_IN_FLIGHT = NAP + (WV == 0 ? 1 : 0);
        bf16v8 fa[2][NA], fb[2][NB];
        int a_addr[MI][NSUB];
        auto frag_row = [&](int i, int kw_, int buf) __attribute__((always_inline)) {
            const int r = wm * WM + i * 32 + lr + kw_ + 2 * seg_of[i];
            const int row = buf * HA + r * HROW, sx = (r >> 1) & 7;
#pragma unroll
            for (int sub = 0; sub < NSUB; ++sub) a_addr[i][sub] = row + (((SLOTS * sub + lh) ^ sx) << 4);
        };
        auto read_a = [&](int sub, int ia) __attribute__((always_inline)) {
            const int i32 = ia * BLK / 32, extra = (ia * BLK % 32) * HROW;
            fa[sub & 1][ia] = *reinterpret_cast<const bf16v8*>(smem + a_addr[i32][sub] + extra);
        };
        auto read_b = [&](int sub, int jb, const char* sB) __attribute__((always_inline)) {
            fb[sub & 1][jb] = *reinterpret_cast<const bf16v8*>(sB + fb_base + jb * BLK * HROW + (((SLOTS * sub + lh) ^ sxb) << 4));
        };
        auto read_nth = [&](int sub, int t, const char* sB) __attribute__((always_inline)) {
            if (t == 0) read_b(sub, 0, sB);
            else if (t == 1) read_a(sub, 0);
            else if (t <= NB) read_b(sub, t - 1, sB);
            else read_a(sub, t - NB);
        };
        auto mfma = [&](int set, int ia, int jb) __attribute__((always_inline)) {
            if constexpr (S16) {
                accv_t& c = acc[ia][jb];
                const bf16v8& wf = fb[set][jb];
                const bf16v8& xf = fa[set][ia];
#if defined(__HIP_DEVICE_COMPILE__)
                asm("v_mfma_f32_16x16x32_bf16 %0, %1, %2, %0" : "+a"(c) : "v"(wf), "v"(xf));
#endif
            } else {
                acc[ia][jb] = __builtin_amdgcn_mfma_f32_32x32x16_bf16(fb[set][jb], fa[set][ia], acc[ia][jb], 0, 0, 0);
            }
        };
        int kh = 0, chunk = 0;
        int kh_l = 0, chunk_l = 0;
        int abuf = 0;
        asm volatile("s_waitcnt vmcnt(0)" ::: "memory");
        __syncthreads();
#pragma unroll
        for (int i = 0; i < MI; ++i) frag_row(i, 0, 0);
#pragma unroll
        for (int t = 0; t < NA + NB; ++t) read_nth(0, t, smem);
#pragma unroll
        for (int q = 0; q < (WV >= 0 ? NA : 2 * NA); ++q) if (q < NBP) dma_b(q, 1, 1, 0, true);

        auto k_step = [&](auto kw_tag, int it) __attribute__((always_inline)) {
            constexpr int KW = decltype(kw_tag)::value;
            R3_STAMP(0);
            const int bbuf = it & 1;
            const bool live1 = it + 1 < p.n_iters, live2 = it + 2 < p.n_iters;
            const int abuf_n = KW == 2 ? abuf ^ 1 : abuf;
            if (KW == 0) {
                chunk_l = chunk + 1; kh_l = kh;
                if (chunk_l == p.n_chunks) { chunk_l = 0; ++kh_l; }
                if (kh_l != kh) set_kh(kh_l);
            }
            const Pos n1 = KW < 2 ? Pos{kh, chunk, KW + 1} : Pos{kh_l, chunk_l, 0};
// ... 54 lines not shown
                                }
                            }
                        }
                        __builtin_amdgcn_sched_barrier(0);
                    }
                }
                R3_STAMP(tail ? 6 : 1 + sub);
            }
            if (KW == 2) { kh = kh_l; chunk = chunk_l; }
        };
        R3_CLOCK(1);
        for (int it = 0; it < p.n_iters; it += 3) {
            k_step(std::integral_constant<int, 0>{}, it);
            k_step(std::integral_constant<int, 1>{}, it + 1);
            k_step(std::integral_constant<int, 2>{}, it + 2);
        }
        R3_CLOCK(2);
    };
    if (STAGGER) {
        switch (wid_u) {
            case 0: k_loop(std::integral_constant<int, 0>{}); break;
            case 1: k_loop(std::integral_constant<int, 1>{}); break;
            case 2: k_loop(std::integral_constant<int, 2>{}); break;
            default: k_loop(std::integral_constant<int, 3>{}); break;
        }
    } else {
        k_loop(std::integral_constant<int, -1>{});
    }
    if (S16) asm volatile("s_nop 7\n\ts_nop 7\n\ts_nop 7" ::: "memory");
    asm volatile("s_waitcnt vmcnt(0)" ::: "memory");
    __syncthreads();

    constexpr int PITCH = WN * ESZ;
    char* ep = smem + wid * (WM * PITCH);
    constexpr int G = S16 ? 1 : 4;
#pragma unroll
    for (int j = 0; j < NB; ++j)
#pragma unroll
        for (int g = 0; g < G; ++g) {
            const int unit = S16 ? 4 * j + lh : 8 * j + 2 * g + lh;
            float bv[4] = {0.f, 0.f, 0.f, 0.f};
            if (bias) {
                const int nb = n0 + wn * WN + 4 * unit;
#pragma unroll
                for (int e = 0; e < 4; ++e) bv[e] = bias[nb + e];
            }
#pragma unroll
            for (int i = 0; i < NA; ++i) {
                const int row = i * BLK + lr;
                uint2 pk;
                pk.x = (unsigned)f2bf(acc[i][j][4 * g + 0] + bv[0]) | ((unsigned)f2bf(acc[i][j][4 * g + 1] + bv[1]) << 16);
                pk.y = (unsigned)f2bf(acc[i][j][4 * g + 2] + bv[2]) | ((unsigned)f2bf(acc[i][j][4 * g + 3] + bv[3]) << 16);
                *reinterpret_cast<uint2*>(ep + row * PITCH + ((unit ^ (row & 15)) << 3)) = pk;
            }
        }
    constexpr int LPR = WN / VEC;
    constexpr int RPP = 64 / LPR;
    constexpr int NP = 64 / RPP;
    const int er = lane / LPR, u16 = lane % LPR, ec = u16 * VEC;
    const int n = n0 + wn * WN + ec;
    if constexpr (EPI == 1) {
        float cs[VEC], sn = 0.f;
#pragma unroll
        for (int e = 0; e < VEC; ++e) cs[e] = 0.f;
        const unsigned char* ep_sign = reinterpret_cast<const unsigned char*>(smem + SIGN_OFF) + (wn * WN + ec) / 8;
#pragma unroll 1
        for (int half = 0; half < MI / 2; ++half) {
            const int m_first = m0 + wm * WM + half * 64 + er;
            const long long qg = (p.per_sample ? (long long)bz * ohw : 0) + m_first;
            float a_noise[NP];
            if (p.act.noise) {
#pragma unroll
                for (int pass = 0; pass < NP; ++pass) a_noise[pass] = ep_noise[wm * WM + half * 64 + pass * RPP + er];
            }
            if (half == 0) __syncthreads();
            u32x4 v[NP];
#pragma unroll
            for (int pass = 0; pass < NP; ++pass) {
                const int row = half * 64 + pass * RPP + er;
                v[pass] = *reinterpret_cast<const u32x4*>(ep + row * PITCH + ((u16 ^ ((row & 15) >> 1)) << 4));
            }
            unsigned sbits[NP];
            if (p.act.mask) {
#pragma unroll
                for (int pass = 0; pass < NP; ++pass) sbits[pass] = ep_sign[(wm * WM + half * 64 + pass * RPP + er) * (HN / 8)];
            } else {
                const bf16_t* srow = reinterpret_cast<const bf16_t*>(p.act.sign_src) + n + qg * p.act.sign_ld;
                u32x4 sv[NP];
#pragma unroll
                for (int pass = 0; pass < NP; ++pass)
                    sv[pass] = *reinterpret_cast<const u32x4*>(srow + (long long)(pass * RPP) * p.act.sign_ld);
#pragma unroll
                for (int pass = 0; pass < NP; ++pass) sbits[pass] = act_sign_byte(sv[pass]);
            }
            u32x4 r[NP];
            const bool has_res = p.act.residual != nullptr;
            if (has_res) {
                const bf16_t* rrow = reinterpret_cast<const bf16_t*>(p.act.residual) + n + qg * p.act.res_ld;
#pragma unroll
                for (int pass = 0; pass < NP; ++pass)
                    r[pass] = *reinterpret_cast<const u32x4*>(rrow + (long long)(pass * RPP) * p.act.res_ld);
            }
            if (er & 1) {
#pragma unroll
                for (int pass = 0; pass < NP; ++pass) v[pass] = u32x4{v[pass][2], v[pass][3], v[pass][0], v[pass][1]};
            }
#pragma unroll
            for (int pass = 0; pass < NP; ++pass) {
#pragma clang fp contract(off)
                float f[VEC], rowsum = 0.f;
#pragma unroll
                for (int e = 0; e < VEC; ++e) {
                    const unsigned w = v[pass][e >> 1];
                    float val = (e & 1) ? __uint_as_float(w & 0xffff0000u) : __uint_as_float(w << 16);
                    if (has_res) {
                        const unsigned wr = r[pass][e >> 1];
                        val += (e & 1) ? __uint_as_float(wr & 0xffff0000u) : __uint_as_float(wr << 16);
                        val = bf2f(f2bf(val));
                    }
                    f[e] = val * p.act.scale * (((sbits[pass] >> e) & 1u) ? 1.f : p.act.alpha);
                    cs[e] += f[e];
                    rowsum += f[e];
                }
                if (p.act.noise) sn = fmaf(rowsum, a_noise[pass], sn);
#pragma unroll
                for (int e = 0; e < 4; ++e) v[pass][e] = (unsigned)f2bf(f[2 * e]) | ((unsigned)f2bf(f[2 * e + 1]) << 16);
            }
            bf16_t* yrow = y + (p.per_sample ? (long long)bz * p.y_bstride : 0) + n + (long long)m_first * p.ldy;
#pragma unroll
            for (int pass = 0; pass < NP; ++pass) *reinterpret_cast<u32x4*>(yrow + (long long)(pass * RPP) * p.ldy) = v[pass];
        }
        const long long mt = (long long)(p.per_sample ? bz : 0) * p.m_tiles + L / p.n_tiles;
        if (p.act.part_b) {
#pragma unroll
            for (int e = 0; e < VEC; ++e) {
                float t = cs[e];
#pragma unroll
                for (int off = 32; off >= LPR; off >>= 1) t += __shfl_xor(t, off, 64);
                cs[e] = t;
            }
            if (er == 0) {
                float* dst = p.act.part_b + (mt * 2 + wm) * p.N + n;
#pragma unroll
                for (int e = 0; e < VEC; ++e) dst[e] = cs[e];
            }
        }
        if (p.act.part_n) {
            sn = wave_sum(sn);
            if (lane == 0) p.act.part_n[(mt * p.n_tiles + L % p.n_tiles) * 4 + wid] = sn;
        }
        R3_CLOCK(3);
        return;
    }
#pragma unroll 1
    for (int half = 0; half < MI / 2; ++half) {
        const int m_first = m0 + wm * WM + half * 64 + er;
        float a_bias[VEC], a_noise[NP];
        if (p.act.enabled == 1) {
#pragma unroll
            for (int e = 0; e < VEC; ++e) a_bias[e] = ep_bias[wn * WN + ec + e];
#pragma unroll
            for (int pass = 0; pass < NP; ++pass) a_noise[pass] = ep_noise[wm * WM + half * 64 + pass * RPP + er];
        }
        if (half == 0) __syncthreads();
        u32x4 v[NP];
#pragma unroll
        for (int pass = 0; pass < NP; ++pass) {
            const int row = half * 64 + pass * RPP + er;
            v[pass] = *reinterpret_cast<const u32x4*>(ep + row * PITCH + ((u16 ^ ((row & 15) >> 1)) << 4));
        }
        if (er & 1) {
#pragma unroll
            for (int pass = 0; pass < NP; ++pass) v[pass] = u32x4{v[pass][2], v[pass][3], v[pass][0], v[pass][1]};
        }
        if (p.act.enabled == 1) {
            if (p.act.alpha >= 0.f && p.act.alpha <= 1.f) {
#pragma unroll
                for (int pass = 0; pass < NP; ++pass)
                    v[pass] = act_epilogue_apply<bf16_t, true>(v[pass], a_bias, a_noise[pass], p.act.alpha, p.act.scale);
            } else {
#pragma unroll
                for (int pass = 0; pass < NP; ++pass)
                    v[pass] = act_epilogue_apply<bf16_t>(v[pass], a_bias, a_noise[pass], p.act.alpha, p.act.scale);
            }
        } else if (p.act.enabled == 2) {
            const bf16_t* rrow = reinterpret_cast<const bf16_t*>(p.act.residual) + n +
                                 ((p.per_sample ? (long long)bz * ohw : 0) + m_first) * p.act.res_ld;
            u32x4 r[NP];
#pragma unroll
            for (int pass = 0; pass < NP; ++pass)
                r[pass] = *reinterpret_cast<const u32x4*>(rrow + (long long)(pass * RPP) * p.act.res_ld);
#pragma unroll
            for (int pass = 0; pass < NP; ++pass) v[pass] = residual_epilogue_apply<bf16_t>(v[pass], r[pass], p.act.res_gain);
        }
        bf16_t* yrow = y + (p.per_sample ? (long long)bz * p.y_bstride : 0) + n + (long long)m_first * p.ldy;
#pragma unroll
        for (int pass = 0; pass < NP; ++pass) *reinterpret_cast<u32x4*>(yrow + (long long)(pass * RPP) * p.ldy) = v[pass];
        if (p.act.enabled == 1 && p.act.mask) {
            const long long tile = (long long)((p.per_sample ? (long long)bz * ohw : 0) + m0) / HM * p.n_tiles + n0 / HN;
            unsigned char* mb = p.act.mask + tile * (HM * (HN / 8)) + (wn * WN + ec) / 8 + (wm * WM + half * 64 + er) * (HN / 8);
#pragma unroll
            for (int pass = 0; pass < NP; ++pass) mb[pass * RPP * (HN / 8)] = (unsigned char)act_sign_byte(v[pass]);
        }
    }
    R3_CLOCK(3);
}

static int row3_tile_columns(int N) {
    if (N >= 256 && (long long)((N + 255) / 256) * 256 * 100 <= (long long)N * 115) return 256;
    if (N >= 128 && (long long)((N + 127) / 128) * 128 * 100 <= (long long)N * 115) return 128;
    return 0;
}

bool conv_row3_eligible(const ConvProblem& q, const ActEpilogue* act, bool has_bias, ConvPlan* plan) {
    static const int enabled = msg_tunable("MSG_CONV_ROW3", 1);
    const int IH = q.IH, IW = q.IW, Cx = q.Cx, Ck = q.Ck, OH = q.OH, OW = q.OW, N = q.N;
    if (q.dtype != MSG_BF16 || q.stride != 1 || q.pad != 1 || q.in_up != 1 || q.pixel_shuffle) return false;
    if (!enabled || q.kh != 3 || q.kw != 3 || IH != OH || IW != OW || Ck % 64 || Cx % 64) return false;
    if (conv_act_mode(act) == 3 && has_bias) return false;
    const long long mtot = q.mtot();
    static const int narrow = msg_tunable("MSG_CONV_ROW3_NARROW", 1);
    static const int w32 = msg_tunable("MSG_CONV_ROW3_W32", 1);
    int hn = row3_tile_columns(N);
    static const int shortk = msg_tunable("MSG_CONV_ROW3_SHORTK", 128);
    if (hn == 256 && Ck <= shortk && N % 128 == 0) hn = 128;
    if (OW == 32 && w32 && N >= 128 && (long long)((N + 127) / 128) * 128 * 100 <= (long long)N * 115) hn = 128;
    if (!hn || (hn == 128 && !narrow) || N % hn) return false;
    const int hm = hn;
    if (!((OW >= 64 && hm % OW == 0) || OW % hm == 0 || (OW == 32 && hm == 128))) return false;
    if (mtot < 1024 || mtot >= (1ll << 31) || mtot % hm) return false;
    if (!q.fits31()) return false;
    if ((long long)9 * (Ck / 64) * HROW >= (1ll << 24)) return false;
    const long long blocks = (mtot / hm) * ((N + hn - 1) / hn);
    if (blocks * q.samples() < (hm == 256 ? 224 : 448) || blocks >= (1ll << 31)) return false;
    const int seg_len = OW < hm ? OW : hm, seg_magic = 65536 / (seg_len + 2) + 1;
    for (int row = 0; row < hm + 16; ++row)
        if (((row * seg_magic) >> 16) != row / (seg_len + 2)) return false;
    *plan = ConvPlan{hm == 256 ? CONV_ROW3 : CONV_ROW3N, hm, hn, true};
    return true;
}

void conv_row3_launch(const ConvProblem& q, const ConvPlan& plan, const void* x, const void* w, const float* bias, void* y,
                      const ActEpilogue* act, void* stream) {
    const int hm = plan.tile_m, hn = plan.tile_n, n_chunks = q.Ck / 64;
    ConvParamsR3 p{};
    conv_fill_common(p, q, act);
    p.seg_len = q.OW < hm ? q.OW : hm;
    p.n_seg = hm / p.seg_len;
    p.n_chunks = n_chunks;
    p.n_iters = 9 * n_chunks;
    p.m_tiles = (int)(q.mtot() / hm);
    p.seg_magic = 65536 / (p.seg_len + 2) + 1;
    auto log2_exact = [](long long v) { int sh = 0; while ((1ll << sh) < v) ++sh; return (1ll << sh) == v ? sh : -1; };
    p.ow_shift = log2_exact(q.OW);
    p.ohw_shift = log2_exact((long long)q.OH * q.OW);
    if (p.ohw_shift < 0) p.ow_shift = -1;
    p.n_tiles = (q.N + hn - 1) / hn;
    dim3 grid((unsigned)((long long)p.m_tiles * p.n_tiles), 1, q.samples());
    static const int s16 = msg_tunable("MSG_CONV_ROW3_S16", 1);
    static const int s16n = msg_tunable("MSG_CONV_ROW3N_S16", 1);
#define ROW3(...) hipLaunchKernelGGL((conv_fprop_row3_kernel<__VA_ARGS__>), grid, dim3(256), 0, (hipStream_t)stream, (const bf16_t*)x, \
                                     (const bf16_t*)w, (bf16_t*)y, bias, p)
    if (p.act.enabled == 3 && hn == 256) ROW3(4, 4, true, 1);
    else if (p.act.enabled == 3) ROW3(2, 2, true, 1);
    else if (hn == 256 && s16) ROW3(4, 4, true);
    else if (hn == 256) ROW3(4, 4, false);
    else if (s16n) ROW3(2, 2, true);
    else ROW3(2, 2, false);
#undef ROW3
}
```

### multi_stylegan_amd/csrc/rgb_skip.hip

```cpp
#include "msg_common.h"

namespace {

struct RgbSkipParams {
    int B, C, H, W, ld;
    const float* fir;
};

struct Taps {
    float kf[16];
    __device__ __forceinline__ explicit Taps(const float* fir) {
#pragma unroll
        for (int i = 0; i < 16; ++i) kf[i] = fir ? fir[15 - i] : 0.f;
    }
};

template <typename T> __device__ __forceinline__ float ld_elem(const T* p);
template <> __device__ __forceinline__ float ld_elem<float>(const float* p) { return *p; }
template <> __device__ __forceinline__ float ld_elem<bf16_t>(const bf16_t* p) { return bf2f(*p); }
template <typename T> __device__ __forceinline__ void st_elem(T* p, float v);
template <> __device__ __forceinline__ void st_elem<float>(float* p, float v) { *p = v; }
template <> __device__ __forceinline__ void st_elem<bf16_t>(bf16_t* p, float v) { *p = f2bf(v); }

template <typename T, int MAXC>
__global__ __launch_bounds__(256) void rgb_skip_fwd_kernel(const T* __restrict__ conv, const float* __restrict__ bias,
                                                          const float* __restrict__ skip, float* __restrict__ out,
                                                          RgbSkipParams p) {
    const int w4 = p.W >> 2;
    const Taps tp(p.fir);
    const long long t = (long long)blockIdx.x * 256 + threadIdx.x;
    if (t >= (long long)p.B * p.H * w4) return;
    const int x0 = (int)(t % w4) * 4;
    const int oy = (int)((t / w4) % p.H);
    const int b = (int)(t / ((long long)w4 * p.H));
    const int h2 = p.H >> 1, w2 = p.W >> 1;
    const T* cp = conv + ((long long)(b * p.H + oy) * p.W + x0) * p.ld;
    const int py = oy & 1;
    const int sy0 = (oy >> 1) - 1 + py;
    const int sx0 = (x0 >> 1) - 1;
    float cv[4][MAXC];
    if (sizeof(T) == 2 && p.ld == 8 && !((uintptr_t)conv & 15u)) {
#pragma unroll
        for (int e = 0; e < 4; ++e) {
            Vec16<bf16_t> q;
            q.raw = *reinterpret_cast<const uint4*>(reinterpret_cast<const bf16_t*>(cp) + e * 8);
#pragma unroll
            for (int c = 0; c < MAXC; ++c) cv[e][c] = q.get(c);
        }
    } else {
#pragma unroll
        for (int e = 0; e < 4; ++e)
#pragma unroll
            for (int c = 0; c < MAXC; ++c) cv[e][c] = c < p.C ? ld_elem<T>(cp + e * p.ld + c) : 0.f;
    }
#pragma unroll
    for (int c = 0; c < MAXC; ++c) {
        if (c >= p.C) break;
        float v[4];
        const float bc = bias ? bias[c] : 0.f;
#pragma unroll
        for (int e = 0; e < 4; ++e) v[e] = cv[e][c] + bc;
        if (skip) {
            const float* sp = skip + ((long long)b * p.C + c) * h2 * w2;
            float up[4] = {0.f, 0.f, 0.f, 0.f};
#pragma unroll
            for (int a = 0; a < 2; ++a) {
                const int sy = sy0 + a, ky = py + 2 * a;
                if ((unsigned)sy >= (unsigned)h2) continue;
                float s[4];
#pragma unroll
                for (int k = 0; k < 4; ++k) s[k] = (unsigned)(sx0 + k) < (unsigned)w2 ? sp[(long long)sy * w2 + sx0 + k] : 0.f;
#pragma unroll
                for (int e = 0; e < 4; ++e) {
                    const int px = e & 1, k0 = (e >> 1) + px;
                    up[e] = fmaf(s[k0], tp.kf[ky * 4 + px], up[e]);
                    up[e] = fmaf(s[k0 + 1], tp.kf[ky * 4 + px + 2], up[e]);
                }
            }
#pragma unroll
            for (int e = 0; e < 4; ++e) v[e] += up[e];
        }
        *reinterpret_cast<f32x4*>(out + (((long long)b * p.C + c) * p.H + oy) * p.W + x0) = f32x4{v[0], v[1], v[2], v[3]};
    }
}

template <typename T, int MAXC>
__global__ __launch_bounds__(256) void rgb_skip_bwd_kernel(const float* __restrict__ g, T* __restrict__ g_conv,
                                                          float* __restrict__ g_skip, RgbSkipParams p) {
    const int h2 = p.H >> 1, w2 = p.W >> 1;
    const Taps tp(p.fir);
    const long long t = (long long)blockIdx.x * 256 + threadIdx.x;
    if (t >= (long long)p.B * h2 * w2) return;
    const int sx = (int)(t % w2), sy = (int)((t / w2) % h2), b = (int)(t / ((long long)w2 * h2));
    const int oy_hi = 2 * sy + 2, ox_hi = 2 * sx + 2;
    float ownv[4][MAXC];
#pragma unroll
    for (int c = 0; c < MAXC; ++c) {
#pragma unroll
        for (int q = 0; q < 4; ++q) ownv[q][c] = 0.f;
        if (c >= p.C) continue;
        const float* gp = g + ((long long)b * p.C + c) * p.H * p.W;
        float acc = 0.f;
#pragma unroll
        for (int ky = 0; ky < 4; ++ky) {
            const int oy = oy_hi - ky;
            if ((unsigned)oy >= (unsigned)p.H) continue;
#pragma unroll
            for (int kx = 0; kx < 4; ++kx) {
                const int ox = ox_hi - kx;
                if ((unsigned)ox >= (unsigned)p.W) continue;
                const float gv = gp[(long long)oy * p.W + ox];
                acc = fmaf(gv, tp.kf[ky * 4 + kx], acc);
                if (ky >= 1 && ky <= 2 && kx >= 1 && kx <= 2) ownv[(2 - ky) * 2 + (2 - kx)][c] = gv;
            }
        }
        if (g_skip) g_skip[(((long long)b * p.C + c) * h2 + sy) * w2 + sx] = acc;
    }
    if (!g_conv) return;
#pragma unroll
    for (int q = 0; q < 4; ++q) {
        T* dst = g_conv + ((long long)(b * p.H + 2 * sy + (q >> 1)) * p.W + 2 * sx + (q & 1)) * p.ld;
        if (sizeof(T) == 2 && p.ld == 8 && !((uintptr_t)g_conv & 15u)) {
            Vec16<bf16_t> o;
#pragma unroll
            for (int e = 0; e < 4; ++e) o.set2(e, ownv[q][2 * e], ownv[q][2 * e + 1]);
            *reinterpret_cast<uint4*>(dst) = o.raw;
        } else {
#pragma unroll
            for (int c = 0; c < MAXC; ++c)
                if (c < p.ld) st_elem<T>(dst + c, ownv[q][c]);
            for (int c = MAXC; c < p.ld; ++c) st_elem<T>(dst + c, 0.f);
        }
    }
}

bool fill(RgbSkipParams& p, const float* fir, int B, int C, int H, int W, int ld) {
    if (B <= 0 || C <= 0 || C > 8 || H <= 0 || W <= 0 || (W & 3) || (H & 1) || ld < C) return false;
    p = RgbSkipParams{B, C, H, W, ld, fir};
    return true;
}

}

extern "C" int msg_rgb_skip_merge(const void* conv, int dtype, int ld, const float* bias, const float* skip,
                                  const float* fir, float* out, int B, int C, int H, int W, void* stream) {
    if (B == 0) return MSG_OK;
    if (!conv || !out || (skip && !fir)) return MSG_EINVAL;
    if (dtype != MSG_F32 && dtype != MSG_BF16) return MSG_EUNSUPPORTED;
    RgbSkipParams p;
    if (!fill(p, fir, B, C, H, W, ld)) return MSG_EUNSUPPORTED;
    if (((uintptr_t)out & 15u) || ((uintptr_t)conv & 3u)) return MSG_EUNSUPPORTED;
    const long long threads = (long long)B * H * (W / 4);
    const dim3 grid((unsigned)((threads + 255) / 256));
    if (dtype == MSG_BF16)
        hipLaunchKernelGGL((rgb_skip_fwd_kernel<bf16_t, 8>), grid, dim3(256), 0, (hipStream_t)stream, (const bf16_t*)conv, bias, skip, out, p);
    else
        hipLaunchKernelGGL((rgb_skip_fwd_kernel<float, 8>), grid, dim3(256), 0, (hipStream_t)stream, (const float*)conv, bias, skip, out, p);
    return MSG_CHECK_LAUNCH();
}

extern "C" int msg_rgb_skip_merge_backward(const float* g, void* g_conv, int dtype, int ld, float* g_skip,
                                           const float* fir, int B, int C, int H, int W, void* stream) {
    if (B == 0) return MSG_OK;
    if (!g || (!g_conv && !g_skip) || (g_skip && !fir)) return MSG_EINVAL;
    if (dtype != MSG_F32 && dtype != MSG_BF16) return MSG_EUNSUPPORTED;
    RgbSkipParams p;
    if (!fill(p, fir, B, C, H, W, ld)) return MSG_EUNSUPPORTED;
    const long long threads = (long long)B * (H / 2) * (W / 2);
    const dim3 grid((unsigned)((threads + 255) / 256));
    if (dtype == MSG_BF16)
        hipLaunchKernelGGL((rgb_skip_bwd_kernel<bf16_t, 8>), grid, dim3(256), 0, (hipStream_t)stream, g, (bf16_t*)g_conv, g_skip, p);
    else
        hipLaunchKernelGGL((rgb_skip_bwd_kernel<float, 8>), grid, dim3(256), 0, (hipStream_t)stream, g, (float*)g_conv, g_skip, p);
    return MSG_CHECK_LAUNCH();
}
```

### multi_stylegan_amd/multi_stylegan_generator.py

```python
import math
from typing import Any, Dict, Iterable, List, Optional, Tuple, Union

import numpy as np
import torch
import torch.nn as nn

from . import conv_ops, equalized_layer
from .op_static import FusedLeakyReLU, blur_bias_act, fused_bias_noise_leaky_relu, rgb_skip, upfirdn2d



def _fir2d(taps, gain=1.0):
    t = torch.tensor(list(taps), dtype=torch.float32)
    k = torch.outer(t, t)
    return k / k.sum() * gain


class Upsample(nn.Module):

    def __init__(self, blur_kernel: List[int] = [1, 3, 3, 1], factor: int = 2) -> None:
        super().__init__()
        self.factor = factor
        self.register_buffer("kernel", _fir2d(blur_kernel))
        p = len(blur_kernel) - factor
        self.padding = ((p + 1) // 2 + factor - 1, p // 2)

    def forward(self, input: torch.Tensor) -> torch.Tensor:
        return upfirdn2d(input, self.kernel, up=self.factor, pad=self.padding)


class Blur(nn.Module):
    def __init__(self, kernel: List[int], sampling_factor: int = 1, sampling_factor_padding: int = 2,
                 kernel_size: int = 3) -> None:
        super().__init__()
        p = (len(kernel) - sampling_factor_padding) + (kernel_size - 1)
        self.padding = ((p + 1) // 2, p // 2)
        self.register_buffer("kernel", _fir2d(kernel, float(sampling_factor ** 2) if sampling_factor > 1 else 1.0))

    def forward(self, input: torch.Tensor) -> torch.Tensor:
        return upfirdn2d(input, self.kernel, pad=self.padding)


class ConstantInput(nn.Module):
    def __init__(self, channel: int, size: Tuple[int, int] = (4, 4)) -> None:
        super().__init__()
        self.input = nn.Parameter(torch.ones(1, channel, size[0], size[1]))

    def forward(self, input: torch.Tensor) -> torch.Tensor:
        return self.input.expand(input.shape[0], -1, -1, -1)


class NoiseInjection(nn.Module):

    def __init__(self) -> None:
        super().__init__()
        self.weight = nn.Parameter(torch.zeros(1, dtype=torch.float32))

    @staticmethod
    def draw(input: torch.Tensor) -> torch.Tensor:
        return torch.randn(input.shape[0], 1, input.shape[2], input.shape[3], device=input.device,
                           dtype=torch.float32)

    def forward(self, input: torch.Tensor, noise: Optional[torch.Tensor] = None) -> torch.Tensor:
        if noise is None:
            noise = self.draw(input)
        return input + (self.weight * noise).to(input.dtype)


class _Premodulated:
    __slots__ = ("value",)

    def __init__(self, value: torch.Tensor) -> None:
        self.value = value


def _modulated_style(mc: "ModulatedConv2d", style, bsz: int) -> torch.Tensor:
    if isinstance(style, _Premodulated):
        return style.value.view(bsz, 1, mc.in_channels, 1, 1)
    if mc.modulation_mapping is not None:
        return mc.modulation_mapping(style).view(bsz, 1, mc.in_channels, 1, 1)
    return style


class ModulatedConv2d(nn.Module):
    def __init__(self, in_channels: int, out_channels: int, style_dimension: int,
                 kernel_size: Union[int, Tuple[int, int]] = (3, 3), demodulate: bool = True, upsampling: bool = True,
                 blur_kernel: List[int] = [1, 3, 3, 1], modulation_mapping: bool = True) -> None:
        super().__init__()
        self.in_channels, self.out_channels = in_channels, out_channels
        self.demodulate, self.upsampling = demodulate, upsampling
        self.kernel_size = kernel_size if isinstance(kernel_size, tuple) else (kernel_size, kernel_size)
        self.blur = Blur(kernel=blur_kernel, sampling_factor=2, sampling_factor_padding=2,
                         kernel_size=self.kernel_size[0]) if upsampling else None
        self.scale = math.sqrt(2) / math.sqrt(in_channels * self.kernel_size[0] * self.kernel_size[1])
        self.weight = nn.Parameter(torch.randn(1, out_channels, in_channels, *self.kernel_size))
        self.modulation_mapping = None
        if modulation_mapping:
            self.modulation_mapping = equalized_layer.EqualizedLinear(style_dimension, in_channels, bias=True)
            self.modulation_mapping.bias.data.fill_(1.0)

    def extra_repr(self):
        return f"{self.in_channels}, {self.out_channels}, kernel_size={self.kernel_size}, " \
               f"demodulate={self.demodulate}, upsampling={self.upsampling}"

    def forward(self, input: torch.Tensor, style: torch.Tensor, skip_blur: bool = False):
        bsz, feats = input.shape[:2]
        assert feats == self.in_channels, f"Expect input feature shape of {self.in_channels} but get {feats}."
        modulated_style = _modulated_style(self, style, bsz)
        output = conv_ops.modulated_conv2d(input, self.weight, modulated_style.reshape(bsz, self.in_channels),
                                           demodulate=self.demodulate, upsample=self.upsampling)
        if self.upsampling and not skip_blur:
            output = self.blur(output)
        if self.modulation_mapping is not None:
            return output, modulated_style
        return output


class StyledConv2d(nn.Module):
    def __init__(self, in_channels: int, out_channels: int, kernel_size: Union[int, Tuple[int, int]],
                 style_dimension: int, demodulate: bool = True, upsampling: bool = False,
                 blur_kernel: List[int] = [1, 3, 3, 1], modulation_mapping: bool = True) -> None:
        super().__init__()
        self.modulation_mapping = modulation_mapping
        self.modulated_convolution = ModulatedConv2d(in_channels, out_channels, style_dimension, kernel_size,
                                                     demodulate, upsampling, blur_kernel, modulation_mapping)
        self.noise_injection = NoiseInjection()
        self.activation = FusedLeakyReLU(out_channels)

    def forward(self, input: torch.Tensor, style: torch.Tensor, noise: torch.Tensor = None, head_slot=None, act_handle=None,
                input_act=None):
        mc = self.modulated_convolution
        if not mc.upsampling and input.is_cuda:
            bsz = input.shape[0]
            style_out = _modulated_style(mc, style, bsz)
            if noise is None:
                noise = torch.randn(bsz, 1, input.shape[2], input.shape[3], device=input.device, dtype=torch.float32)
            output = conv_ops.modulated_conv2d_bias_act(
                input, mc.weight, style_out.reshape(bsz, mc.in_channels), mc.demodulate, self.activation.bias, noise,
                self.noise_injection.weight, self.activation.negative_slope, self.activation.scale, head_slot=head_slot,
                input_act=input_act)
            return (output, style_out) if self.modulation_mapping else output
        if mc.upsampling and input.is_cuda:
            result = mc(input, style, skip_blur=True)
            output, style_out = result if self.modulation_mapping else (result, None)
            p0, p1 = mc.blur.padding
            oh, ow = output.shape[2] + p0 + p1 - 3, output.shape[3] + p0 + p1 - 3
            if noise is None:
                noise = torch.randn(output.shape[0], 1, oh, ow, device=input.device, dtype=torch.float32)
            output = blur_bias_act(output, mc.blur.kernel, mc.blur.padding, self.activation.bias, noise,
                                   self.noise_injection.weight, self.activation.negative_slope, self.activation.scale,
                                   act_handle=act_handle)
            return (output, style_out) if self.modulation_mapping else output
        result = self.modulated_convolution(input, style)
        output, style_out = result if self.modulation_mapping else (result, None)
        if noise is None:
            noise = NoiseInjection.draw(output)
        output = fused_bias_noise_leaky_relu(output, self.activation.bias, noise, self.noise_injection.weight,
                                             self.activation.negative_slope, self.activation.scale)
        if self.modulation_mapping:
            return output, style_out
        return output


def _merge_rgb(conv: torch.Tensor, bias: torch.Tensor, skip: Optional[torch.Tensor], upsampling: nn.Module) -> torch.Tensor:
    fir = getattr(upsampling, "kernel", None) if skip is not None else None
    if skip is None or isinstance(upsampling, Upsample):
        factor, pad = (upsampling.factor, upsampling.padding) if skip is not None else (2, (2, 1))
        if rgb_skip.supported(conv, skip, fir, factor, pad):
            return rgb_skip.rgb_skip_merge(conv, bias.reshape(-1).float(), skip, fir)
    output = conv.float().contiguous() + bias
    if skip is not None:
        output = output + upsampling(skip)
    return output


class OutputBlock(nn.Module):

    def __init__(self, in_channels: int, style_dimension: int, out_channels: int = 1, upsampling: bool = False,
                 blur_kernel: List[int] = [1, 3, 3, 1], modulation_mapping: bool = True) -> None:
        super().__init__()
        self.modulation_mapping = modulation_mapping
        self.upsampling = Upsample(blur_kernel=blur_kernel, factor=2) if upsampling else nn.Identity()
        self.modulated_convolution = ModulatedConv2d(in_channels, out_channels, style_dimension, (1, 1),
                                                     demodulate=False, upsampling=False,
                                                     modulation_mapping=modulation_mapping)
        self.bias = nn.Parameter(torch.zeros(1, 1, 1, 1, dtype=torch.float32))

    def forward(self, input: torch.Tensor, style: torch.Tensor, skip: torch.Tensor = None):
        result = self.modulated_convolution(input, style)
        output, style_out = result if self.modulation_mapping else (result, None)
        output = _merge_rgb(output, self.bias.expand(1, output.shape[1], 1, 1), skip, self.upsampling)
        if self.modulation_mapping:
            return output, style_out
        return output


class StyleMapping(nn.Module):
    def __init__(self, latent_dimensions: int = 512, depth: int = 8) -> None:
        super().__init__()
        layers: List[nn.Module] = [equalized_layer.PixelwiseNormalization()]
        for _ in range(depth):
            layers += [equalized_layer.EqualizedLinear(latent_dimensions, latent_dimensions, bias=False),
                       FusedLeakyReLU(latent_dimensions)]
        self.layers = nn.Sequential(*layers)

    def forward(self, noise: torch.Tensor) -> torch.Tensor:
        return self.layers(noise)


class Generator(nn.Module):
    def __init__(self, config: Dict[str, Any]) -> None:
        super().__init__()
        channels = [int(c // config["channel_factor"]) for c in config["channels"]]
        self.out_channels: int = 3
        self.latent_dimensions: int = config["latent_dimensions"]
        self.starting_resolution: Tuple[int, int] = config["starting_resolution"]
        ld, c0 = self.latent_dimensions, channels[0]
        self.style_mapping = StyleMapping(latent_dimensions=ld, depth=config["depth_style_mapping"])
        self.constant_input_1 = ConstantInput(channel=c0, size=self.starting_resolution)
        self.constant_input_2 = ConstantInput(channel=c0, size=self.starting_resolution)
        self.starting_convolution_1 = StyledConv2d(c0, c0, (3, 3), ld)
        self.starting_convolution_2 = StyledConv2d(c0, c0, (3, 3), ld, modulation_mapping=False)
        self.starting_output_block_1 = OutputBlock(c0, ld, self.out_channels)
        self.starting_output_block_2 = OutputBlock(c0, ld, self.out_channels, modulation_mapping=False)
        self.main_convolutions_1, self.output_blocks_1 = nn.ModuleList(), nn.ModuleList()
        self.main_convolutions_2, self.output_blocks_2 = nn.ModuleList(), nn.ModuleList()
        for c_in, c_out in zip(channels[:-1], channels[1:]):
            for convs, heads, mapped in ((self.main_convolutions_1, self.output_blocks_1, True),
                                         (self.main_convolutions_2, self.output_blocks_2, False)):
                convs.append(StyledConv2d(c_in, c_out, (2, 2), ld, upsampling=True, modulation_mapping=mapped))
                convs.append(StyledConv2d(c_out, c_out, (3, 3), ld, modulation_mapping=mapped))
                heads.append(OutputBlock(c_out, ld, self.out_channels, upsampling=True, modulation_mapping=mapped))
        self.noises = nn.Module()
        self.noises.register_buffer("noise_start", torch.randn(1, 1, *self.starting_resolution))
        for level in range(len(channels) - 1):
            res = 2 ** (level + 3)
            self.noises.register_buffer(f"noise_{2 * level}", torch.randn(1, 1, res, res))
            self.noises.register_buffer(f"noise_{2 * level + 1}", torch.randn(1, 1, res, res))
        self.compute_dtype = torch.float32
        self.elide_dead_branch = False

    def get_parameters(self, lr_main: float = 1e-03, lr_style: float = 1e-05) -> Iterable:
        order = ["constant_input_1", "starting_convolution_1", "starting_output_block_1", "main_convolutions_1",
                 "output_blocks_1", "constant_input_2", "starting_convolution_2", "starting_output_block_2",
                 "main_convolutions_2", "output_blocks_2"]
        groups = [{"params": getattr(self, name).parameters(), "lr": lr_main} for name in order]
        groups.append({"params": self.style_mapping.parameters(), "lr": lr_style})
        return groups

    def live_parameters(self) -> List[nn.Parameter]:
        return [p for n, p in self.named_parameters() if not n.startswith("main_convolutions_2.")]

    def _latent(self, input, inject_index, input_is_latent):
        n = len(self.main_convolutions_1) + 2
        if input_is_latent:
            if input.ndim < 3:
                return input.unsqueeze(1).repeat(1, n, 1)
            if input.shape[1] != n:
                return input.repeat(1, n, 1)
            return input
        if isinstance(input, (list, tuple)):
            if len(input) > 1 and all(z.shape == input[0].shape for z in input):
                styles = self.style_mapping(torch.cat(list(input), dim=0)).chunk(len(input), dim=0)
            else:
                styles = [self.style_mapping(z) for z in input]
            if inject_index is None:
                inject_index = np.random.randint(1, n - 1)
            return torch.cat([styles[0].unsqueeze(1).repeat(1, inject_index, 1),
                              styles[1].unsqueeze(1).repeat(1, n - inject_index, 1)], dim=1)
        return self.style_mapping(input).unsqueeze(1).repeat(1, n, 1)

    def _style_groups(self):
        groups = [(self.starting_convolution_1.modulated_convolution, 0),
                  (self.starting_output_block_1.modulated_convolution, 1)]
        for i in range(len(self.main_convolutions_1) // 2):
            groups += [(self.main_convolutions_1[2 * i].modulated_convolution, 2 * i + 1),
                       (self.main_convolutions_1[2 * i + 1].modulated_convolution, 2 * i + 2),
                       (self.output_blocks_1[i].modulated_convolution, 2 * i + 3)]
        return groups

    def _all_styles(self, latent: torch.Tensor):
        if not (latent.is_cuda and latent.dtype == torch.float32):
            return None
        groups = self._style_groups()
        maps = [mc.modulation_mapping for mc, _ in groups]
        first = maps[0]
        if any(m is None or m.bias is None or m.weight.shape != first.weight.shape for m in maps):
            return None
        out = conv_ops.grouped_linear(latent, [slot for _, slot in groups], [m.weight for m in maps],
                                      [m.bias for m in maps], first.scale, first.scale_bias)
        return out.unbind(0)

    def _heads_pairable(self, features: torch.Tensor) -> bool:
        if not features.is_cuda:
            return False
        for h1, h2 in zip(self.output_blocks_1, self.output_blocks_2):
            m1, m2 = h1.modulated_convolution, h2.modulated_convolution
            if m1.modulation_mapping is None or m2.modulation_mapping is not None or m1.demodulate or m2.demodulate \
                    or m1.weight.shape != m2.weight.shape:
                return False
        return True

    @staticmethod
    def _paired_heads(head1: "OutputBlock", head2: "OutputBlock", features: torch.Tensor, latent_w, skip: torch.Tensor,
                      head_slot=None):
        mc1, mc2 = head1.modulated_convolution, head2.modulated_convolution
        bsz, o1, o2 = features.shape[0], mc1.out_channels, mc2.out_channels
        style = _modulated_style(mc1, latent_w, bsz)
        both = conv_ops.modulated_conv2d(features, torch.cat([mc1.weight, mc2.weight], dim=1),
                                         style.reshape(bsz, mc1.in_channels), demodulate=False, upsample=False,
                                         head_slot=head_slot)
        bias = torch.cat([head1.bias.expand(1, o1, 1, 1), head2.bias.expand(1, o2, 1, 1)], dim=1)
        return _merge_rgb(both, bias, skip, head1.upsampling), style

    def forward(self, input: Union[List[torch.Tensor], torch.Tensor], return_main_style_vectors: bool = False,
                noise: Optional[List[torch.Tensor]] = None, randomize_noise: bool = True,
                inject_index: Optional[int] = None, input_is_latent: bool = False,
                return_path_length_grads: bool = False, path_length_noise: Optional[torch.Tensor] = None):
        return self._forward(input, return_main_style_vectors, noise, randomize_noise, inject_index, input_is_latent,
                             bool(return_path_length_grads), path_length_noise)

    def _draw_layer_noise(self, latent):
        if not latent.is_cuda:
            return None
        b = latent.shape[0]
        res0 = tuple(self.constant_input_1.input.shape[2:])
        shapes = [res0, res0]
        h, w = res0
        for i in range(len(self.main_convolutions_1)):
            if i % 2 == 0:
                h, w = 2 * h, 2 * w
            shapes += [(h, w), (h, w)]
        sizes = [b * hh * ww for hh, ww in shapes]
        flat = torch.randn(sum(sizes), device=latent.device, dtype=torch.float32)
        maps = [t.view(b, 1, hh, ww) for t, (hh, ww) in zip(flat.split(sizes), shapes)]
        return maps[0], maps[1], maps[2::2], maps[3::2]

    def _forward(self, input, return_main_style_vectors, noise, randomize_noise, inject_index, input_is_latent,
                 return_path_length_grads, path_length_noise):
        latent = self._latent(input, inject_index, input_is_latent)
        n_main = len(self.main_convolutions_1)
        layer_noise_2 = None
        if noise is None:
            if randomize_noise:
                noise_start, layer_noise = None, [None] * n_main
                drawn = self._draw_layer_noise(latent)
                if drawn is not None:
                    noise_start, noise_start_2, layer_noise, layer_noise_2 = drawn
            else:
                noise_start = self.noises.noise_start
                layer_noise = [getattr(self.noises, f"noise_{i}") for i in range(n_main)]
        else:
            noise_start, layer_noise = noise[0], list(noise[1:])
        dt = self.compute_dtype
        pre = self._all_styles(latent)
        w_of = (lambda group, slot: _Premodulated(pre[group])) if pre is not None else \
            (lambda group, slot: latent[:, slot])
        out1 = conv_ops.to_compute_layout(self.constant_input_1(latent), dt)
        out2 = conv_ops.to_compute_layout(self.constant_input_2(latent), dt)
        out1, style = self.starting_convolution_1(out1, w_of(0, 0), noise=noise_start)
        out2 = self.starting_convolution_2(out2, style, noise=noise_start if layer_noise_2 is None else noise_start_2)
        skip1, style = self.starting_output_block_1(out1, w_of(1, 1))
        skip2 = self.starting_output_block_2(out2, style)
        run_stream2 = not self.elide_dead_branch
        paired = n_main >= 2 and skip1.shape == skip2.shape and self._heads_pairable(out1)
        skip = torch.cat([skip1, skip2], dim=1) if paired else None
        for i in range(n_main // 2):
            handle = conv_ops.ActHandle() if out1.is_cuda and torch.is_grad_enabled() and not return_path_length_grads else None
            out1, style = self.main_convolutions_1[2 * i](out1, w_of(2 + 3 * i, 2 * i + 1),
                                                           noise=layer_noise[2 * i], act_handle=handle)
            if run_stream2:
                out2 = self.main_convolutions_2[2 * i](out2, style, noise=(layer_noise_2 or layer_noise)[2 * i])
            slot = conv_ops.HeadGradSlot() if paired and out1.dtype == torch.bfloat16 and torch.is_grad_enabled() and \
                not return_path_length_grads else None
            out1, style = self.main_convolutions_1[2 * i + 1](out1, w_of(3 + 3 * i, 2 * i + 2),
                                                               noise=layer_noise[2 * i + 1], head_slot=slot, input_act=handle)
            if run_stream2:
                out2 = self.main_convolutions_2[2 * i + 1](out2, style, noise=(layer_noise_2 or layer_noise)[2 * i + 1])
            if paired:
                skip, style = self._paired_heads(self.output_blocks_1[i], self.output_blocks_2[i], out1,
                                                 w_of(4 + 3 * i, 2 * i + 3), skip, head_slot=slot)
            else:
                skip1, style = self.output_blocks_1[i](out1, w_of(4 + 3 * i, 2 * i + 3), skip=skip1)
                skip2 = self.output_blocks_2[i](out1, style, skip=skip2)
        if paired:
            image = skip.view(skip.shape[0], 2, skip.shape[1] // 2, *skip.shape[2:])
        else:
            image = torch.stack([skip1, skip2], dim=1)
        if return_path_length_grads:
            if path_length_noise is None:
                path_length_noise = torch.randn(image.shape, device=image.device, dtype=torch.float32)
            pl_noise = path_length_noise / math.sqrt(image.shape[2] * image.shape[3] * image.shape[4])
            return torch.autograd.grad((image * pl_noise).sum(), latent, create_graph=True, retain_graph=True)[0]
        if return_main_style_vectors:
            return image, latent
        return image
```

### multi_stylegan_amd/op_static/rgb_skip.py

```python
from typing import Optional

import torch
from torch.autograd import Function

from .. import _lib
from .._autograd import _derive


def supported(conv: torch.Tensor, skip: Optional[torch.Tensor], fir: Optional[torch.Tensor], up: int, pad) -> bool:
    if not (conv.is_cuda and conv.ndim == 4 and conv.dtype in (torch.float32, torch.bfloat16)):
        return False
    b, c, h, w = conv.shape
    if c > 8 or w % 4 or h % 2:
        return False
    if skip is None:
        return True
    return (fir is not None and tuple(fir.shape) == (4, 4) and fir.dtype == torch.float32 and up == 2
            and tuple(pad) == (2, 1) and skip.dtype == torch.float32 and tuple(skip.shape) == (b, c, h // 2, w // 2))


def _launch_fwd(conv, bias, skip, fir):
    from .. import conv_ops
    dev = _lib.require_gpu(conv, bias, skip, fir)
    b, c, h, w = conv.shape
    cv, ld = conv_ops._nhwc_view(conv)
    out = torch.empty((b, c, h, w), dtype=torch.float32, device=dev)
    skip_c = skip.contiguous() if skip is not None else None
    bias_c = bias.contiguous() if bias is not None else None
    nbytes = conv.numel() * conv.element_size() + out.numel() * 4 + (skip.numel() * 4 if skip is not None else 0)
    with _lib.on_device(dev), _lib.kernel_clock.span("rgb_skip_merge/f32", nbytes):
        code = _lib.lib().msg_rgb_skip_merge(cv.data_ptr(), _lib.dtype_code(conv), ld, _lib.ptr(bias_c), _lib.ptr(skip_c),
                                             _lib.ptr(fir if skip is not None else None), out.data_ptr(), b, c, h, w,
                                             _lib.stream_of(dev))
    _lib.check(code, "msg_rgb_skip_merge")
    return out


def _launch_bwd(g, conv_dtype, want_conv, want_skip, fir):
    from .. import conv_ops
    dev = _lib.require_gpu(g, fir)
    b, c, h, w = g.shape
    g = g.contiguous()
    g_conv, ld = (conv_ops._alloc_out(b, c, h, w, conv_dtype, dev) if want_conv else (None, 8))
    g_skip = torch.empty((b, c, h // 2, w // 2), dtype=torch.float32, device=dev) if want_skip else None
    nbytes = g.numel() * 4 + (g_conv.numel() * g_conv.element_size() if want_conv else 0) + \
        (g_skip.numel() * 4 if want_skip else 0)
    with _lib.on_device(dev), _lib.kernel_clock.span("rgb_skip_merge_bwd/f32", nbytes):
        code = _lib.lib().msg_rgb_skip_merge_backward(g.data_ptr(), _lib.ptr(g_conv), _lib.dtype_code(
            g_conv if want_conv else g), ld, _lib.ptr(g_skip), _lib.ptr(fir if want_skip else None), b, c, h, w,
            _lib.stream_of(dev))
    _lib.check(code, "msg_rgb_skip_merge_backward")
    return g_conv, g_skip


class _RgbSkipMerge(Function):
    @staticmethod
    def forward(ctx, conv, bias, skip, fir):
        ctx.save_for_backward(fir)
        ctx.meta = (conv.dtype, skip is not None, bias is not None)
        return _launch_fwd(conv, bias, skip, fir)

    @staticmethod
    def backward(ctx, g):
        fir, = ctx.saved_tensors
        conv_dtype, has_skip, has_bias = ctx.meta
        need = ctx.needs_input_grad
        g_conv, g_bias, g_skip = _derive(_RgbSkipMergeBackward, g, fir, conv_dtype, need[0], has_bias and need[1],
                                                             has_skip and need[2])
        return g_conv if need[0] else None, g_bias if has_bias and need[1] else None, \
            g_skip if has_skip and need[2] else None, None


class _RgbSkipMergeBackward(Function):

    @staticmethod
    def forward(ctx, g, fir, conv_dtype, want_conv, want_bias, want_skip):
        ctx.save_for_backward(fir)
        ctx.meta = (want_conv, want_bias, want_skip, g.shape)
        g_conv, g_skip = (None, None)
        if want_conv or want_skip:
            g_conv, g_skip = _launch_bwd(g, conv_dtype, want_conv, want_skip, fir)
        g_bias = g.sum(dim=(0, 2, 3)) if want_bias else None
        zero = g.new_zeros(0)
        outs = (g_conv if want_conv else zero, g_bias if want_bias else zero, g_skip if want_skip else zero)
        ctx.mark_non_differentiable(*[o for o, wanted in zip(outs, (want_conv, want_bias, want_skip)) if not wanted])
        return outs

    @staticmethod
    def backward(ctx, gg_conv, gg_bias, gg_skip):
        fir, = ctx.saved_tensors
        want_conv, want_bias, want_skip, shape = ctx.meta
        b, c, h, w = shape
        if not want_conv:
            gg_conv = torch.zeros((b, c, h, w), dtype=torch.float32, device=fir.device).contiguous(
                memory_format=torch.channels_last)
        gg = _RgbSkipMerge.apply(gg_conv, gg_bias if want_bias else None, gg_skip if want_skip else None, fir)
        return gg, None, None, None, None, None


def rgb_skip_merge(conv: torch.Tensor, bias: Optional[torch.Tensor], skip: Optional[torch.Tensor],
                   fir: Optional[torch.Tensor]) -> torch.Tensor:
    return _RgbSkipMerge.apply(conv, bias, skip, fir)
```

Measured before the change: 156.9.

## Fuse the 1x1 RGB head projection into the preceding conv's activation epilogue

The modulated 1x1 output-head convolution is folded into the epilogue of the preceding fused-activation 3x3 conv. Each N-tile writes per-tile partial 8-channel projections, and a new rgb_skip_merge_partials kernel sums them with the bias and the upsampled skip. The standalone head conv then returns a placeholder tensor and skips its own launch. This removes one re-read of the full feature map and one kernel launch per resolution, at the cost of extra partial-plane traffic, more epilogue work, and more complex autograd plumbing.

After: 157.2 (median of 6 runs). Within noise of the previous version (+0.2%).

```diff
diff --git a/include/msg_hip.h b/include/msg_hip.h
--- a/include/msg_hip.h
+++ b/include/msg_hip.h
@@ -111,6 +111,8 @@
                        float* out, int B, int C, int H, int W, void* stream);
 int msg_rgb_skip_merge_backward(const float* g, void* g_conv, int dtype, int ld, float* g_skip, const float* fir,
                                 int B, int C, int H, int W, void* stream);
+int msg_rgb_skip_merge_partials(const float* parts, int n_parts, const float* bias, const float* skip, const float* fir,
+                                float* out, int B, int C, int H, int W, void* stream);
 int msg_gamma_merge(const void* a, const void* b, const float* gamma, void* y, int dtype, long long n, float gain, void* stream);
 long long msg_gamma_merge_backward_workspace(void);
 int msg_gamma_merge_backward(const void* gy, const void* a, const float* gamma, void* ga, void* gb, float* g_gamma, int dtype,
@@ -162,6 +164,14 @@
                               const float* act_bias, const float* noise, const float* noise_weight,
                               int noise_batch, float alpha, float scale, unsigned char* mask, void* stream);
 
+int msg_conv2d_fprop_act_head(const void* x, const void* w, void* y, int dtype,
+                              int B, int IH, int IW, int Cx, int Ck, int OH, int OW, int N, int ldy,
+                              int kh, int kw, int stride, int pad, long long w_batch_stride,
+                              const float* act_bias, const float* noise, const float* noise_weight,
+                              int noise_batch, float alpha, float scale, unsigned char* mask,
+                              const void* head_w, int head_rows, float* head_part, long long head_part_floats, int tile,
+                              void* stream);
+
 int msg_conv2d_fprop_residual(const void* x, const void* w, void* y, int dtype,
                               int B, int IH, int IW, int Cx, int Ck, int OH, int OW, int N, int ldy,
                               int kh, int kw, int stride, int pad, long long w_batch_stride,
@@ -206,7 +216,8 @@
     MSG_PLAN_ROW3N = 4,
     MSG_PLAN_THIN = 5,
     MSG_PLAN_UPCONV = 6,
-    MSG_FPLAN_FIELDS = 5
+    MSG_FPLAN_FIELDS = 5,
+    MSG_EPILOGUE_ACT_HEAD = 5
 };
 int msg_conv2d_fprop_launch_plan(int dtype, int B, int IH, int IW, int Cx, int Ck, int OH, int OW, int N, int ldy,
                                  int kh, int kw, int stride, int pad, int in_up, int pixel_shuffle,
diff --git a/multi_stylegan_amd/build.py b/multi_stylegan_amd/build.py
--- a/multi_stylegan_amd/build.py
+++ b/multi_stylegan_amd/build.py
@@ -42,7 +42,7 @@
     procs = []
     for src in sources():
         obj = os.path.join(objdir, os.path.basename(src) + ".o")
-        deps = [src] + glob.glob(os.path.join(CSRC, "*.h"))
+        deps = [src] + glob.glob(os.path.join(CSRC, "*.h")) + [os.path.join(HERE, "..", "include", "msg_hip.h")]
         objs.append(obj)
         if not force and os.path.exists(obj) and all(os.path.getmtime(obj) > os.path.getmtime(d) for d in deps):
             continue
diff --git a/multi_stylegan_amd/conv_ops.py b/multi_stylegan_amd/conv_ops.py
--- a/multi_stylegan_amd/conv_ops.py
+++ b/multi_stylegan_amd/conv_ops.py
@@ -373,6 +373,13 @@
 
 
 @functools.lru_cache(maxsize=None)
+def _head_plan(*args):
+    out = (ctypes.c_longlong * _lib.MSG_FPLAN_FIELDS)()
+    ok = _lib.lib().msg_conv2d_fprop_launch_plan(*args, _lib.MSG_EPILOGUE_ACT_HEAD, ctypes.addressof(out), len(out)) == _lib.MSG_OK
+    return (out[3], out[4]) if ok else (0, 0)
+
+
+@functools.lru_cache(maxsize=None)
 def _wgrad_plan(*geom):
     out = (ctypes.c_longlong * _lib.MSG_WPLAN_FIELDS)()
     _lib.check(_lib.lib().msg_conv2d_wgrad_plan(*geom, _lib.MSG_WGRAD_K_AUTO, ctypes.addressof(out), len(out)),
@@ -407,10 +414,19 @@
         flops = 2.0 * b * oh * ow * n * kh * kw * c_real / (in_up * in_up)
     key, sign_tile = "conv_fprop", None
     sign_holder = act[5] if act is not None and len(act) > 5 else None
+    head = act[6] if act is not None and len(act) > 6 else None
+    parts = None
+    if head is not None and ldy == n and per_sample:
+        floats, n_parts = _head_plan(_lib.dtype_code(x), b, ih, iw, cx, ck, oh, ow, n, ldy, kh, kw, stride, pad, in_up,
+                                     int(pixel_shuffle), wstride, 0)
+        if floats:
+            parts = torch.empty((n_parts, b, oh, ow, 8), dtype=torch.float32, device=dev)
     if _lib.kernel_clock.enabled or sign_holder is not None:
         _, key, sign_tile, _, _ = _fprop_plan(_lib.dtype_code(x), b, ih, iw, cx, ck, oh, ow, n, ldy, kh, kw, stride, pad, in_up,
                                               int(pixel_shuffle), wstride, int(bias is not None),
                                               2 if residual is not None else int(act is not None))
+        if parts is not None:
+            key += "_head"
     if _lib.kernel_clock.enabled and _CLOCK_SHAPES:
         key += f"|B{b} {ih}x{iw}->{oh}x{ow} {c_real}->{n} {kh}x{kw} s{stride} up{in_up}" \
                f"{' ps' if pixel_shuffle else ''}{' per-sample' if per_sample else ''}|"
@@ -436,10 +452,18 @@
                 mask = sign_mask_for(b, n, oh, ow, x.dtype, dev)
                 if mask is not None:
                     sign_holder.append((mask, sign_tile, sign_tile))
-            code = _lib.lib().msg_conv2d_fprop_act_mask(
-                xv.data_ptr(), wk.data_ptr(), y.data_ptr(), _contraction_code(x, mode), b, ih, iw, cx, ck, oh, ow, n, ldy, kh, kw,
-                stride, pad, wstride, _lib.ptr(act_bias), _lib.ptr(noise), _lib.ptr(noise_w),
-                1 if noise is None else noise.shape[0], float(alpha), float(scale), _lib.ptr(mask), _lib.stream_of(dev))
+            if parts is not None:
+                code = _lib.lib().msg_conv2d_fprop_act_head(
+                    xv.data_ptr(), wk.data_ptr(), y.data_ptr(), _contraction_code(x, mode), b, ih, iw, cx, ck, oh, ow, n, ldy, kh,
+                    kw, stride, pad, wstride, _lib.ptr(act_bias), _lib.ptr(noise), _lib.ptr(noise_w),
+                    1 if noise is None else noise.shape[0], float(alpha), float(scale), _lib.ptr(mask), head[0].data_ptr(),
+                    head[1], parts.data_ptr(), parts.numel(), 0, _lib.stream_of(dev))
+                head[2].parts = parts
+            else:
+                code = _lib.lib().msg_conv2d_fprop_act_mask(
+                    xv.data_ptr(), wk.data_ptr(), y.data_ptr(), _contraction_code(x, mode), b, ih, iw, cx, ck, oh, ow, n, ldy, kh,
+                    kw, stride, pad, wstride, _lib.ptr(act_bias), _lib.ptr(noise), _lib.ptr(noise_w),
+                    1 if noise is None else noise.shape[0], float(alpha), float(scale), _lib.ptr(mask), _lib.stream_of(dev))
     _lib.check(code, "msg_conv2d_fprop")
     return y
 
@@ -1024,6 +1048,26 @@
     def take(self):
         head, dgrad, self.head, self.dgrad = self.head, self.dgrad, None, None
         return head, dgrad
+
+
+class HeadForward:
+    __slots__ = ("weight", "style", "style_out", "parts")
+
+    def __init__(self, weight, style, style_out=None):
+        self.weight, self.style, self.style_out, self.parts = weight, style, style_out, None
+
+    def image(self, b: int, n: int, dtype, dev):
+        _, o, i, kh, kw = self.weight.shape
+        if not HEAD_EPILOGUE or dtype != torch.bfloat16 or kh != 1 or kw != 1 or o > 8 or i != n or i % 64 or \
+                self.style.shape != (b, i):
+            return None
+        base = torch.nn.functional.pad(self.weight.detach().reshape(o, 1, i).float(), (0, 0, 0, 0, 0, 8 - o))
+        image = torch.empty((b, 8, 1, i), dtype=dtype, device=dev)
+        _scale_rows_cols(base, None, self.style.detach().float().contiguous(), image, math.sqrt(2.0) / math.sqrt(i))
+        return image, o
+
+
+HEAD_EPILOGUE = bool(int(os.environ.get("MSG_HEAD_EPILOGUE", "1")))
 
 
 class _ForkInput(Function):
@@ -1592,7 +1636,7 @@
 
     @staticmethod
     def forward(ctx, x, weight, style, demodulate, upsample, act_bias=None, noise=None, noise_w=None, alpha=0.2,
-                act_scale=1.0, fuse_act=False, head_slot=None, input_act=None):
+                act_scale=1.0, fuse_act=False, head_slot=None, input_act=None, head_fwd=None):
         dev = _lib.require_gpu(x, weight, style)
         ctx.input_act = input_act if input_act is not None and input_act.armed else None
         ctx.head_slot = head_slot
@@ -1602,6 +1646,12 @@
         _, o, i, kh, kw = weight.shape
         b, t = x.shape[0], kh * kw
         scale = math.sqrt(2.0) / math.sqrt(i * t)
+        if head_fwd is not None and not fuse_act and head_fwd.parts is not None:
+            assert not demodulate and not upsample and t == 1
+            ctx.save_for_backward(x, weight, style, torch.empty(0, device=dev), None, None)
+            ctx.cfg = (False, False, Geometry("conv", 1, 1, 1, 0, x.shape[2:], True), scale)
+            ctx.act = ctx.bias_param = ctx.mask = None
+            return x.new_empty(1).expand(b, o, *x.shape[2:])
         w3 = weight.detach().reshape(o, i, t)
         s = style.detach().float().contiguous()
         d = None
@@ -1629,7 +1679,9 @@
         holder = [] if any(ctx.needs_input_grad) else None
         if fuse_act:
             assert not upsample, "the upsampling layers blur before their activation"
-            act = (*_act_operands(act_bias, noise, noise_w, (b, o, *g.y_hw)), alpha, act_scale, holder)
+            head = head_fwd.image(b, o, x.dtype, dev) if head_fwd is not None else None
+            act = (*_act_operands(act_bias, noise, noise_w, (b, o, *g.y_hw)), alpha, act_scale, holder,
+                   None if head is None else (*head, head_fwd))
         if upsample:
             y = _launch_fprop(x, wk, ck, None, 4 * o, g.x_hw, 1, 1, 1, 0, 1, True, True, i, mode=g.mode)
         else:
@@ -1667,13 +1719,13 @@
             if fused is not None:
                 gy, gb, gnw = fused
             elif gy is None:
-                return (None,) * 13
+                return (None,) * 14
             else:
                 gy, gb, gnw = _derive(FusedLeakyReLUFunctionBackward, gy, y_act, noise if has_noise else None,
                                       ctx.bias_param if has_bias else False, alpha, act_scale, ctx.mask)
             gb = gb if has_bias and need[5] else None
             gnw = gnw.reshape(nw_shape) if has_noise and need[7] else None
-        tail = (None, None, gb, None, gnw, None, None, None, None, None)
+        tail = (None, None, gb, None, gnw, None, None, None, None, None, None)
         if ctx.act is None and slot is not None and slot.armed and need[0] and not torch.is_grad_enabled() and \
                 fused_head_ok(gy, weight, b, demodulate, upsample):
             gyc, wt, st = gy, weight, style
@@ -1719,13 +1771,13 @@
 
 
 def modulated_conv2d_bias_act(x, weight, style, demodulate, act_bias, noise, noise_weight, negative_slope=0.2,
-                              scale=1.0, head_slot=None, input_act=None):
+                              scale=1.0, head_slot=None, input_act=None, head_fwd=None):
     return _ModulatedConv.apply(x, weight, style, bool(demodulate), False, act_bias, noise, noise_weight,
-                                float(negative_slope), float(scale), True, head_slot, input_act)
-
-
-def modulated_conv2d(x, weight, style, demodulate, upsample, head_slot=None):
-    if head_slot is None:
+                                float(negative_slope), float(scale), True, head_slot, input_act, head_fwd)
+
+
+def modulated_conv2d(x, weight, style, demodulate, upsample, head_slot=None, head_fwd=None):
+    if head_slot is None and head_fwd is None:
         return _ModulatedConv.apply(x, weight, style, bool(demodulate), bool(upsample))
     return _ModulatedConv.apply(x, weight, style, bool(demodulate), bool(upsample), None, None, None, 0.2, 1.0, False,
-                                head_slot)
+                                head_slot, None, head_fwd)
diff --git a/multi_stylegan_amd/csrc/conv_dispatch.h b/multi_stylegan_amd/csrc/conv_dispatch.h
--- a/multi_stylegan_amd/csrc/conv_dispatch.h
+++ b/multi_stylegan_amd/csrc/conv_dispatch.h
@@ -58,8 +58,9 @@
 bool conv_upconv_eligible(const ConvProblem& q, const ActEpilogue* act, bool has_bias, ConvPlan* plan);
 void conv_upconv_launch(const ConvProblem& q, const ConvPlan& plan, const void* x, const void* w, void* y, void* stream);
 bool conv_row3_eligible(const ConvProblem& q, const ActEpilogue* act, bool has_bias, ConvPlan* plan);
+bool conv_row3_fits(const ConvProblem& q, int tile);
 void conv_row3_launch(const ConvProblem& q, const ConvPlan& plan, const void* x, const void* w, const float* bias, void* y,
-                      const ActEpilogue* act, void* stream);
+                      const ActEpilogue* act, void* stream, const void* head_w = nullptr, float* head_part = nullptr);
 bool conv_pp_eligible(const ConvProblem& q, ConvPlan* plan);
 void conv_pp_launch(const ConvProblem& q, const ConvPlan& plan, const void* x, const void* w, const float* bias, void* y,
                     const ActEpilogue* act, void* stream);
diff --git a/multi_stylegan_amd/csrc/conv_fprop.hip b/multi_stylegan_amd/csrc/conv_fprop.hip
--- a/multi_stylegan_amd/csrc/conv_fprop.hip
+++ b/multi_stylegan_amd/csrc/conv_fprop.hip
@@ -500,6 +500,13 @@
     *entries = tiles * (q.N / plan.tile_n) * 4;
 }
 
+static long long head_stage_tiles(const ConvProblem& q, const ConvPlan& plan) {
+    static const int narrow = msg_tunable("MSG_CONV_HEAD_ROW3N", 1);
+    if (!is_row3(plan) || q.ldy != q.N || !q.per_sample() || q.dtype != MSG_BF16) return 0;
+    if (plan.kernel == CONV_ROW3N && !narrow) return 0;
+    return q.N / plan.tile_n;
+}
+
 static int plan_code(ConvKernel kernel) {
     switch (kernel) {
         case CONV_THIN_N: case CONV_THIN_K: return MSG_PLAN_THIN;
@@ -515,15 +522,19 @@
 extern "C" int msg_conv2d_fprop_launch_plan(int dtype, int B, int IH, int IW, int Cx, int Ck, int OH, int OW, int N, int ldy,
                                             int kh, int kw, int stride, int pad, int in_up, int pixel_shuffle,
                                             long long w_batch_stride, int has_bias, int epilogue, long long* out, int n_out_fields) {
-    if (epilogue < 0 || epilogue > 3 || (epilogue && (has_bias || in_up != 1 || pixel_shuffle))) return MSG_EINVAL;
+    if (epilogue < 0 || epilogue == 4 || epilogue > MSG_EPILOGUE_ACT_HEAD || (epilogue && (has_bias || in_up != 1 || pixel_shuffle))) return MSG_EINVAL;
     const ConvProblem q = conv_problem(dtype, B, IH, IW, Cx, Ck, OH, OW, N, ldy, kh, kw, stride, pad, in_up, pixel_shuffle, w_batch_stride);
     ConvPlan plan;
-    const int rc = fprop_plan_for(q, epilogue, has_bias != 0, nullptr, &plan);
+    const int rc = fprop_plan_for(q, epilogue == MSG_EPILOGUE_ACT_HEAD ? 1 : epilogue, has_bias != 0, nullptr, &plan);
     if (rc != MSG_OK) return rc;
     long long fields[MSG_FPLAN_FIELDS] = {};
     if (q.B) {
         fields[0] = plan_code(plan.kernel); fields[1] = plan.tile_m; fields[2] = plan.tile_n;
         if (epilogue == 3) act_backward_partials(q, plan, &fields[3], &fields[4]);
+        if (epilogue == MSG_EPILOGUE_ACT_HEAD) {
+            fields[4] = head_stage_tiles(q, plan);
+            fields[3] = fields[4] * q.B * q.OH * q.OW * 8;
+        }
     }
     for (int k = 0; k < MSG_FPLAN_FIELDS && k < n_out_fields; ++k) out[k] = fields[k];
     return MSG_OK;
@@ -602,6 +613,35 @@
                                     int noise_batch, float alpha, float scale, void* stream) {
     return msg_conv2d_fprop_act_mask(x, w, y, dtype, B, IH, IW, Cx, Ck, OH, OW, N, ldy, kh, kw, stride, pad, w_batch_stride,
                                      act_bias, noise, noise_weight, noise_batch, alpha, scale, nullptr, stream);
+}
+
+extern "C" int msg_conv2d_fprop_act_head(const void* x, const void* w, void* y, int dtype,
+                                         int B, int IH, int IW, int Cx, int Ck, int OH, int OW, int N, int ldy,
+                                         int kh, int kw, int stride, int pad, long long w_batch_stride,
+                                         const float* act_bias, const float* noise, const float* noise_weight,
+                                         int noise_batch, float alpha, float scale, unsigned char* mask,
+                                         const void* head_w, int head_rows, float* head_part, long long head_part_floats,
+                                         int tile, void* stream) {
+    if (B == 0) return MSG_OK;
+    if (noise && (!noise_weight || (noise_batch != 1 && noise_batch != B))) return MSG_EINVAL;
+    const bool head = head_w || head_part;
+    if (head && (!head_w || !head_part || head_rows <= 0 || ((((uintptr_t)head_w) | ((uintptr_t)head_part)) & 15u))) return MSG_EINVAL;
+    if (!head && !tile) return MSG_EINVAL;
+    const ConvProblem q = conv_problem(dtype, B, IH, IW, Cx, Ck, OH, OW, N, ldy, kh, kw, stride, pad, 1, 0, w_batch_stride);
+    const void* const io[3] = {x, w, y};
+    ConvPlan plan;
+    const int rc = fprop_plan_for(q, 1, false, io, &plan);
+    if (rc != MSG_OK) return rc;
+    if (tile) {
+        if (!conv_row3_fits(q, tile)) return MSG_EUNSUPPORTED;
+        plan = ConvPlan{tile == 256 ? CONV_ROW3 : CONV_ROW3N, tile, tile, true};
+    }
+    const long long tiles = head ? head_stage_tiles(q, plan) : 1;
+    if (!tiles || (head && head_rows > 8)) return MSG_EUNSUPPORTED;
+    if (head && head_part_floats < tiles * q.B * q.OH * q.OW * 8) return MSG_EINVAL;
+    ActEpilogue act{act_bias, noise, noise_weight, noise_batch, 1, alpha, scale, nullptr, 0, 0.f, mask};
+    conv_row3_launch(q, plan, x, w, nullptr, y, &act, stream, head_w, head_part);
+    return MSG_CHECK_LAUNCH();
 }
 
 extern "C" int msg_conv2d_fprop_residual(const void* x, const void* w, void* y, int dtype,
diff --git a/multi_stylegan_amd/csrc/conv_fprop_row3.hip b/multi_stylegan_amd/csrc/conv_fprop_row3.hip
--- a/multi_stylegan_amd/csrc/conv_fprop_row3.hip
+++ b/multi_stylegan_amd/csrc/conv_fprop_row3.hip
@@ -13,6 +13,8 @@
     int seg_magic;
     int ow_shift, ohw_shift;
     ActEpilogue act;
+    const bf16_t* head_w;
+    float* head_part;
 };
 
 constexpr int HROW = 128;
@@ -56,7 +58,8 @@
 #endif
     constexpr int EP_OFF = 2 * HA + 2 * HB;
     constexpr int SIGN_OFF = EP_OFF + (HM + HN) * 4;
-    __shared__ __attribute__((aligned(16))) char smem[SIGN_OFF + (EPI == 1 ? HM * (HN / 8) : 0)];
+    constexpr int HEAD_OFF = SIGN_OFF, RED_OFF = HEAD_OFF + 8 * HN * ESZ;
+    __shared__ __attribute__((aligned(16))) char smem[SIGN_OFF + (EPI == 1 ? HM * (HN / 8) : 0) + (EPI == 2 ? 8 * HN * ESZ + 2 * HM * 8 * 4 : 0)];
     float* const ep_noise = reinterpret_cast<float*>(smem + EP_OFF);
     float* const ep_bias = ep_noise + HM;
 
@@ -85,7 +88,7 @@
             if (!p.per_sample && p.act.noise_batch == 1) idx = p.ohw_shift >= 0 ? mm & (ohw - 1) : mm % ohw;
             ep_noise[t] = ok ? nw * p.act.noise[idx] : 0.f;
         }
-        if (EPI == 0)
+        if (EPI != 1)
             for (int t = tid; t < HN; t += 256) ep_bias[t] = (p.act.bias && n0 + t < p.N) ? p.act.bias[n0 + t] : 0.f;
     }
     if constexpr (EPI == 1) {
@@ -102,6 +105,14 @@
                     ((trow * ntn + tn) * p.act.mask_tile_m + (qg - trow * p.act.mask_tile_m)) * vpt + (cvg - tn * vpt);
                 *reinterpret_cast<u32x4*>(smem + SIGN_OFF + row * (HN / 8) + 16 * un) = *reinterpret_cast<const u32x4*>(src);
             }
+        }
+    }
+    if constexpr (EPI == 2) {
+        constexpr int UPR = HN / VEC;
+        const bf16_t* hw = p.head_w + (long long)bz * 8 * p.N + n0;
+        for (int t = tid; t < 8 * UPR; t += 256) {
+            const int r = t / UPR, u = t - r * UPR;
+            *reinterpret_cast<u32x4*>(smem + HEAD_OFF + t * 16) = *reinterpret_cast<const u32x4*>(hw + (long long)r * p.N + u * VEC);
         }
     }
 
@@ -462,6 +473,19 @@
         R3_CLOCK(3);
         return;
     }
+    constexpr int HKS = WN / 32;
+    const int hl = lane & 15, hh = lane >> 4;
+    bf16v8 hwf[EPI == 2 ? HKS : 1];
+    if constexpr (EPI == 2) {
+#pragma unroll
+        for (int ks = 0; ks < HKS; ++ks) {
+            hwf[ks] = *reinterpret_cast<const bf16v8*>(smem + HEAD_OFF + (((hl & 7) * HN + wn * WN + 32 * ks + 8 * hh) * ESZ));
+            if (hl >= 8) {
+#pragma unroll
+                for (int e = 0; e < 8; ++e) hwf[ks][e] = (__bf16)0.f;
+            }
+        }
+    }
 #pragma unroll 1
     for (int half = 0; half < MI / 2; ++half) {
         const int m_first = m0 + wm * WM + half * 64 + er;
@@ -503,14 +527,46 @@
 #pragma unroll
             for (int pass = 0; pass < NP; ++pass) v[pass] = residual_epilogue_apply<bf16_t>(v[pass], r[pass], p.act.res_gain);
         }
+        if constexpr (EPI == 2) {
+#pragma unroll
+            for (int pass = 0; pass < NP; ++pass) {
+                const int row = half * 64 + pass * RPP + er;
+                *reinterpret_cast<u32x4*>(ep + row * PITCH + ((u16 ^ ((row & 15) >> 1)) << 4)) = v[pass];
+            }
+        }
         bf16_t* yrow = y + (p.per_sample ? (long long)bz * p.y_bstride : 0) + n + (long long)m_first * p.ldy;
 #pragma unroll
         for (int pass = 0; pass < NP; ++pass) *reinterpret_cast<u32x4*>(yrow + (long long)(pass * RPP) * p.ldy) = v[pass];
+        if constexpr (EPI == 2) {
+            __builtin_amdgcn_wave_barrier();
+#pragma unroll
+            for (int i = 0; i < 4; ++i) {
+                f32x4 hp = {0.f, 0.f, 0.f, 0.f};
+                const int row = half * 64 + i * 16 + hl;
+#pragma unroll
+                for (int ks = 0; ks < HKS; ++ks) {
+                    const bf16v8 xa = *reinterpret_cast<const bf16v8*>(ep + row * PITCH + (((4 * ks + hh) ^ (hl >> 1)) << 4));
+#if defined(__HIP_DEVICE_COMPILE__)
+                    hp = __builtin_amdgcn_mfma_f32_16x16x32_bf16(hwf[ks], xa, hp, 0, 0, 0);
+#endif
+                }
+                if (hh < 2) *reinterpret_cast<f32x4*>(smem + RED_OFF + (((wn * HM + wm * WM + row) * 8 + 4 * hh) << 2)) = hp;
+            }
+        }
         if (p.act.enabled == 1 && p.act.mask) {
             const long long tile = (long long)((p.per_sample ? (long long)bz * ohw : 0) + m0) / HM * p.n_tiles + n0 / HN;
             unsigned char* mb = p.act.mask + tile * (HM * (HN / 8)) + (wn * WN + ec) / 8 + (wm * WM + half * 64 + er) * (HN / 8);
 #pragma unroll
             for (int pass = 0; pass < NP; ++pass) mb[pass * RPP * (HN / 8)] = (unsigned char)act_sign_byte(v[pass]);
+        }
+    }
+    if constexpr (EPI == 2) {
+        __syncthreads();
+        const float* red = reinterpret_cast<const float*>(smem + RED_OFF);
+        float* dst = p.head_part + (((long long)(L % p.n_tiles) * p.B + bz) * ohw + m0) * 8;
+        for (int t = tid; t < HM * 2; t += 256) {
+            const f32x4 a = *reinterpret_cast<const f32x4*>(red + t * 4), b = *reinterpret_cast<const f32x4*>(red + (HM * 2 + t) * 4);
+            *reinterpret_cast<f32x4*>(dst + t * 4) = a + b;
         }
     }
     R3_CLOCK(3);
@@ -522,11 +578,27 @@
     return 0;
 }
 
+bool conv_row3_fits(const ConvProblem& q, int hm) {
+    const int OW = q.OW, N = q.N;
+    if (q.dtype != MSG_BF16 || q.stride != 1 || q.pad != 1 || q.in_up != 1 || q.pixel_shuffle) return false;
+    if (q.kh != 3 || q.kw != 3 || q.IH != q.OH || q.IW != OW || q.Ck % 64 || q.Cx % 64) return false;
+    if ((hm != 256 && hm != 128) || N % hm) return false;
+    if (!((OW >= 64 && hm % OW == 0) || OW % hm == 0 || (OW == 32 && hm == 128))) return false;
+    const long long mtot = q.mtot();
+    if (mtot >= (1ll << 31) || mtot % hm) return false;
+    if (!q.fits31()) return false;
+    if ((long long)9 * (q.Ck / 64) * HROW >= (1ll << 24)) return false;
+    if ((mtot / hm) * (N / hm) >= (1ll << 31)) return false;
+    const int seg_len = OW < hm ? OW : hm, seg_magic = 65536 / (seg_len + 2) + 1;
+    for (int row = 0; row < hm + 16; ++row)
+        if (((row * seg_magic) >> 16) != row / (seg_len + 2)) return false;
+    return true;
+}
+
 bool conv_row3_eligible(const ConvProblem& q, const ActEpilogue* act, bool has_bias, ConvPlan* plan) {
     static const int enabled = msg_tunable("MSG_CONV_ROW3", 1);
-    const int IH = q.IH, IW = q.IW, Cx = q.Cx, Ck = q.Ck, OH = q.OH, OW = q.OW, N = q.N;
-    if (q.dtype != MSG_BF16 || q.stride != 1 || q.pad != 1 || q.in_up != 1 || q.pixel_shuffle) return false;
-    if (!enabled || q.kh != 3 || q.kw != 3 || IH != OH || IW != OW || Ck % 64 || Cx % 64) return false;
+    const int Ck = q.Ck, OW = q.OW, N = q.N;
+    if (!enabled || q.kh != 3 || q.kw != 3) return false;
     if (conv_act_mode(act) == 3 && has_bias) return false;
     const long long mtot = q.mtot();
     static const int narrow = msg_tunable("MSG_CONV_ROW3_NARROW", 1);
@@ -537,21 +609,15 @@
     if (OW == 32 && w32 && N >= 128 && (long long)((N + 127) / 128) * 128 * 100 <= (long long)N * 115) hn = 128;
     if (!hn || (hn == 128 && !narrow) || N % hn) return false;
     const int hm = hn;
-    if (!((OW >= 64 && hm % OW == 0) || OW % hm == 0 || (OW == 32 && hm == 128))) return false;
-    if (mtot < 1024 || mtot >= (1ll << 31) || mtot % hm) return false;
-    if (!q.fits31()) return false;
-    if ((long long)9 * (Ck / 64) * HROW >= (1ll << 24)) return false;
+    if (!conv_row3_fits(q, hm) || mtot < 1024) return false;
     const long long blocks = (mtot / hm) * ((N + hn - 1) / hn);
-    if (blocks * q.samples() < (hm == 256 ? 224 : 448) || blocks >= (1ll << 31)) return false;
-    const int seg_len = OW < hm ? OW : hm, seg_magic = 65536 / (seg_len + 2) + 1;
-    for (int row = 0; row < hm + 16; ++row)
-        if (((row * seg_magic) >> 16) != row / (seg_len + 2)) return false;
+    if (blocks * q.samples() < (hm == 256 ? 224 : 448)) return false;
     *plan = ConvPlan{hm == 256 ? CONV_ROW3 : CONV_ROW3N, hm, hn, true};
     return true;
 }
 
 void conv_row3_launch(const ConvProblem& q, const ConvPlan& plan, const void* x, const void* w, const float* bias, void* y,
-                      const ActEpilogue* act, void* stream) {
+                      const ActEpilogue* act, void* stream, const void* head_w, float* head_part) {
     const int hm = plan.tile_m, hn = plan.tile_n, n_chunks = q.Ck / 64;
     ConvParamsR3 p{};
     conv_fill_common(p, q, act);
@@ -566,12 +632,16 @@
     p.ohw_shift = log2_exact((long long)q.OH * q.OW);
     if (p.ohw_shift < 0) p.ow_shift = -1;
     p.n_tiles = (q.N + hn - 1) / hn;
+    p.head_w = (const bf16_t*)head_w;
+    p.head_part = head_part;
     dim3 grid((unsigned)((long long)p.m_tiles * p.n_tiles), 1, q.samples());
     static const int s16 = msg_tunable("MSG_CONV_ROW3_S16", 1);
     static const int s16n = msg_tunable("MSG_CONV_ROW3N_S16", 1);
 #define ROW3(...) hipLaunchKernelGGL((conv_fprop_row3_kernel<__VA_ARGS__>), grid, dim3(256), 0, (hipStream_t)stream, (const bf16_t*)x, \
                                      (const bf16_t*)w, (bf16_t*)y, bias, p)
-    if (p.act.enabled == 3 && hn == 256) ROW3(4, 4, true, 1);
+    if (head_part && hn == 256) ROW3(4, 4, true, 2);
+    else if (head_part) ROW3(2, 2, true, 2);
+    else if (p.act.enabled == 3 && hn == 256) ROW3(4, 4, true, 1);
     else if (p.act.enabled == 3) ROW3(2, 2, true, 1);
     else if (hn == 256 && s16) ROW3(4, 4, true);
     else if (hn == 256) ROW3(4, 4, false);
diff --git a/multi_stylegan_amd/csrc/rgb_skip.hip b/multi_stylegan_amd/csrc/rgb_skip.hip
--- a/multi_stylegan_amd/csrc/rgb_skip.hip
+++ b/multi_stylegan_amd/csrc/rgb_skip.hip
@@ -5,6 +5,7 @@
 struct RgbSkipParams {
     int B, C, H, W, ld;
     const float* fir;
+    int n_parts;
 };
 
 struct Taps {
@@ -22,7 +23,7 @@
 template <> __device__ __forceinline__ void st_elem<float>(float* p, float v) { *p = v; }
 template <> __device__ __forceinline__ void st_elem<bf16_t>(bf16_t* p, float v) { *p = f2bf(v); }
 
-template <typename T, int MAXC>
+template <typename T, int MAXC, bool PARTS = false>
 __global__ __launch_bounds__(256) void rgb_skip_fwd_kernel(const T* __restrict__ conv, const float* __restrict__ bias,
                                                           const float* __restrict__ skip, float* __restrict__ out,
                                                           RgbSkipParams p) {
@@ -39,7 +40,20 @@
     const int sy0 = (oy >> 1) - 1 + py;
     const int sx0 = (x0 >> 1) - 1;
     float cv[4][MAXC];
-    if (sizeof(T) == 2 && p.ld == 8 && !((uintptr_t)conv & 15u)) {
+    if constexpr (PARTS) {
+        static_assert(MAXC == 8 && sizeof(T) == 4, "partials are [pixel][8] fp32");
+        const long long pstride = (long long)p.B * p.H * p.W * 8;
+#pragma unroll
+        for (int e = 0; e < 4; ++e) {
+            f32x4 lo = *reinterpret_cast<const f32x4*>(cp + e * 8), hi = *reinterpret_cast<const f32x4*>(cp + e * 8 + 4);
+            for (int t = 1; t < p.n_parts; ++t) {
+                lo += *reinterpret_cast<const f32x4*>(cp + t * pstride + e * 8);
+                hi += *reinterpret_cast<const f32x4*>(cp + t * pstride + e * 8 + 4);
+            }
+#pragma unroll
+            for (int c = 0; c < 4; ++c) { cv[e][c] = bf2f(f2bf(lo[c])); cv[e][4 + c] = bf2f(f2bf(hi[c])); }
+        }
+    } else if (sizeof(T) == 2 && p.ld == 8 && !((uintptr_t)conv & 15u)) {
 #pragma unroll
         for (int e = 0; e < 4; ++e) {
             Vec16<bf16_t> q;
@@ -136,7 +150,7 @@
 
 bool fill(RgbSkipParams& p, const float* fir, int B, int C, int H, int W, int ld) {
     if (B <= 0 || C <= 0 || C > 8 || H <= 0 || W <= 0 || (W & 3) || (H & 1) || ld < C) return false;
-    p = RgbSkipParams{B, C, H, W, ld, fir};
+    p = RgbSkipParams{B, C, H, W, ld, fir, 0};
     return true;
 }
 
@@ -159,6 +173,20 @@
     return MSG_CHECK_LAUNCH();
 }
 
+extern "C" int msg_rgb_skip_merge_partials(const float* parts, int n_parts, const float* bias, const float* skip,
+                                           const float* fir, float* out, int B, int C, int H, int W, void* stream) {
+    if (B == 0) return MSG_OK;
+    if (!parts || !out || n_parts <= 0 || (skip && !fir)) return MSG_EINVAL;
+    RgbSkipParams p;
+    if (!fill(p, fir, B, C, H, W, 8)) return MSG_EUNSUPPORTED;
+    if (((uintptr_t)out & 15u) || ((uintptr_t)parts & 15u)) return MSG_EUNSUPPORTED;
+    p.n_parts = n_parts;
+    const long long threads = (long long)B * H * (W / 4);
+    const dim3 grid((unsigned)((threads + 255) / 256));
+    hipLaunchKernelGGL((rgb_skip_fwd_kernel<float, 8, true>), grid, dim3(256), 0, (hipStream_t)stream, parts, bias, skip, out, p);
+    return MSG_CHECK_LAUNCH();
+}
+
 extern "C" int msg_rgb_skip_merge_backward(const float* g, void* g_conv, int dtype, int ld, float* g_skip,
                                            const float* fir, int B, int C, int H, int W, void* stream) {
     if (B == 0) return MSG_OK;
diff --git a/multi_stylegan_amd/multi_stylegan_generator.py b/multi_stylegan_amd/multi_stylegan_generator.py
--- a/multi_stylegan_amd/multi_stylegan_generator.py
+++ b/multi_stylegan_amd/multi_stylegan_generator.py
@@ -128,7 +128,7 @@
         self.activation = FusedLeakyReLU(out_channels)
 
     def forward(self, input: torch.Tensor, style: torch.Tensor, noise: torch.Tensor = None, head_slot=None, act_handle=None,
-                input_act=None):
+                input_act=None, head_fwd=None):
         mc = self.modulated_convolution
         if not mc.upsampling and input.is_cuda:
             bsz = input.shape[0]
@@ -138,7 +138,7 @@
             output = conv_ops.modulated_conv2d_bias_act(
                 input, mc.weight, style_out.reshape(bsz, mc.in_channels), mc.demodulate, self.activation.bias, noise,
                 self.noise_injection.weight, self.activation.negative_slope, self.activation.scale, head_slot=head_slot,
-                input_act=input_act)
+                input_act=input_act, head_fwd=head_fwd)
             return (output, style_out) if self.modulation_mapping else output
         if mc.upsampling and input.is_cuda:
             result = mc(input, style, skip_blur=True)
@@ -162,12 +162,15 @@
         return output
 
 
-def _merge_rgb(conv: torch.Tensor, bias: torch.Tensor, skip: Optional[torch.Tensor], upsampling: nn.Module) -> torch.Tensor:
+def _merge_rgb(conv: torch.Tensor, bias: torch.Tensor, skip: Optional[torch.Tensor], upsampling: nn.Module,
+               parts: Optional[torch.Tensor] = None) -> torch.Tensor:
     fir = getattr(upsampling, "kernel", None) if skip is not None else None
     if skip is None or isinstance(upsampling, Upsample):
         factor, pad = (upsampling.factor, upsampling.padding) if skip is not None else (2, (2, 1))
         if rgb_skip.supported(conv, skip, fir, factor, pad):
-            return rgb_skip.rgb_skip_merge(conv, bias.reshape(-1).float(), skip, fir)
+            return rgb_skip.rgb_skip_merge(conv, bias.reshape(-1).float(), skip, fir, parts)
+    if parts is not None:
+        raise RuntimeError("image head: partial planes of the head stage, but no merge kernel for this skip path")
     output = conv.float().contiguous() + bias
     if skip is not None:
         output = output + upsampling(skip)
@@ -302,16 +305,32 @@
         return True
 
     @staticmethod
+    def _head_forward(head1: "OutputBlock", head2: "OutputBlock", latent_w, features: torch.Tensor, skip: torch.Tensor):
+        mc1, mc2 = head1.modulated_convolution, head2.modulated_convolution
+        bsz, (h, w) = features.shape[0], features.shape[2:]
+        up = head1.upsampling
+        if not (features.is_cuda and features.dtype == torch.bfloat16 and isinstance(up, Upsample) and up.factor == 2 and
+                tuple(up.padding) == (2, 1) and tuple(up.kernel.shape) == (4, 4) and w % 4 == 0 and h % 2 == 0 and
+                mc1.out_channels + mc2.out_channels <= 8 and skip.dtype == torch.float32 and
+                tuple(skip.shape) == (bsz, mc1.out_channels + mc2.out_channels, h // 2, w // 2)):
+            return None
+        style = _modulated_style(mc1, latent_w, bsz)
+        return conv_ops.HeadForward(torch.cat([mc1.weight, mc2.weight], dim=1), style.reshape(bsz, mc1.in_channels), style)
+
+    @staticmethod
     def _paired_heads(head1: "OutputBlock", head2: "OutputBlock", features: torch.Tensor, latent_w, skip: torch.Tensor,
-                      head_slot=None):
+                      head_slot=None, head_fwd=None):
         mc1, mc2 = head1.modulated_convolution, head2.modulated_convolution
         bsz, o1, o2 = features.shape[0], mc1.out_channels, mc2.out_channels
-        style = _modulated_style(mc1, latent_w, bsz)
-        both = conv_ops.modulated_conv2d(features, torch.cat([mc1.weight, mc2.weight], dim=1),
-                                         style.reshape(bsz, mc1.in_channels), demodulate=False, upsample=False,
-                                         head_slot=head_slot)
+        if head_fwd is not None:
+            weight, style2d, style = head_fwd.weight, head_fwd.style, head_fwd.style_out
+        else:
+            style = _modulated_style(mc1, latent_w, bsz)
+            weight, style2d = torch.cat([mc1.weight, mc2.weight], dim=1), style.reshape(bsz, mc1.in_channels)
+        both = conv_ops.modulated_conv2d(features, weight, style2d, demodulate=False, upsample=False, head_slot=head_slot,
+                                         head_fwd=head_fwd)
         bias = torch.cat([head1.bias.expand(1, o1, 1, 1), head2.bias.expand(1, o2, 1, 1)], dim=1)
-        return _merge_rgb(both, bias, skip, head1.upsampling), style
+        return _merge_rgb(both, bias, skip, head1.upsampling, None if head_fwd is None else head_fwd.parts), style
 
     def forward(self, input: Union[List[torch.Tensor], torch.Tensor], return_main_style_vectors: bool = False,
                 noise: Optional[List[torch.Tensor]] = None, randomize_noise: bool = True,
@@ -373,13 +392,16 @@
                 out2 = self.main_convolutions_2[2 * i](out2, style, noise=(layer_noise_2 or layer_noise)[2 * i])
             slot = conv_ops.HeadGradSlot() if paired and out1.dtype == torch.bfloat16 and torch.is_grad_enabled() and \
                 not return_path_length_grads else None
+            head_fwd = self._head_forward(self.output_blocks_1[i], self.output_blocks_2[i], w_of(4 + 3 * i, 2 * i + 3), out1,
+                                          skip) if paired and not return_path_length_grads else None
             out1, style = self.main_convolutions_1[2 * i + 1](out1, w_of(3 + 3 * i, 2 * i + 2),
-                                                               noise=layer_noise[2 * i + 1], head_slot=slot, input_act=handle)
+                                                               noise=layer_noise[2 * i + 1], head_slot=slot, input_act=handle,
+                                                               head_fwd=head_fwd)
             if run_stream2:
                 out2 = self.main_convolutions_2[2 * i + 1](out2, style, noise=(layer_noise_2 or layer_noise)[2 * i + 1])
             if paired:
                 skip, style = self._paired_heads(self.output_blocks_1[i], self.output_blocks_2[i], out1,
-                                                 w_of(4 + 3 * i, 2 * i + 3), skip, head_slot=slot)
+                                                 w_of(4 + 3 * i, 2 * i + 3), skip, head_slot=slot, head_fwd=head_fwd)
             else:
                 skip1, style = self.output_blocks_1[i](out1, w_of(4 + 3 * i, 2 * i + 3), skip=skip1)
                 skip2 = self.output_blocks_2[i](out1, style, skip=skip2)
diff --git a/multi_stylegan_amd/op_static/rgb_skip.py b/multi_stylegan_amd/op_static/rgb_skip.py
--- a/multi_stylegan_amd/op_static/rgb_skip.py
+++ b/multi_stylegan_amd/op_static/rgb_skip.py
@@ -36,6 +36,23 @@
     return out
 
 
+def _launch_fwd_parts(conv, parts, bias, skip, fir):
+    dev = _lib.require_gpu(parts, bias, skip, fir)
+    b, c, h, w = conv.shape
+    if parts.shape[1:] != (b, h, w, 8) or parts.dtype != torch.float32 or not parts.is_contiguous():
+        raise _lib.MsgHipError(f"rgb_skip_merge: partial maps {tuple(parts.shape)} for a {(b, c, h, w)} result")
+    out = torch.empty((b, c, h, w), dtype=torch.float32, device=dev)
+    skip_c = skip.contiguous() if skip is not None else None
+    bias_c = bias.contiguous() if bias is not None else None
+    nbytes = parts.numel() * 4 + out.numel() * 4 + (skip.numel() * 4 if skip is not None else 0)
+    with _lib.on_device(dev), _lib.kernel_clock.span("rgb_skip_merge_partials/f32", nbytes):
+        code = _lib.lib().msg_rgb_skip_merge_partials(parts.data_ptr(), parts.shape[0], _lib.ptr(bias_c), _lib.ptr(skip_c),
+                                                      _lib.ptr(fir if skip is not None else None), out.data_ptr(), b, c, h, w,
+                                                      _lib.stream_of(dev))
+    _lib.check(code, "msg_rgb_skip_merge_partials")
+    return out
+
+
 def _launch_bwd(g, conv_dtype, want_conv, want_skip, fir):
     from .. import conv_ops
     dev = _lib.require_gpu(g, fir)
@@ -55,9 +72,11 @@
 
 class _RgbSkipMerge(Function):
     @staticmethod
-    def forward(ctx, conv, bias, skip, fir):
+    def forward(ctx, conv, bias, skip, fir, parts=None):
         ctx.save_for_backward(fir)
         ctx.meta = (conv.dtype, skip is not None, bias is not None)
+        if parts is not None:
+            return _launch_fwd_parts(conv, parts, bias, skip, fir)
         return _launch_fwd(conv, bias, skip, fir)
 
     @staticmethod
@@ -68,7 +87,7 @@
         g_conv, g_bias, g_skip = _derive(_RgbSkipMergeBackward, g, fir, conv_dtype, need[0], has_bias and need[1],
                                                              has_skip and need[2])
         return g_conv if need[0] else None, g_bias if has_bias and need[1] else None, \
-            g_skip if has_skip and need[2] else None, None
+            g_skip if has_skip and need[2] else None, None, None
 
 
 class _RgbSkipMergeBackward(Function):
@@ -94,10 +113,10 @@
         if not want_conv:
             gg_conv = torch.zeros((b, c, h, w), dtype=torch.float32, device=fir.device).contiguous(
                 memory_format=torch.channels_last)
-        gg = _RgbSkipMerge.apply(gg_conv, gg_bias if want_bias else None, gg_skip if want_skip else None, fir)
+        gg = _RgbSkipMerge.apply(gg_conv, gg_bias if want_bias else None, gg_skip if want_skip else None, fir, None)
         return gg, None, None, None, None, None
 
 
 def rgb_skip_merge(conv: torch.Tensor, bias: Optional[torch.Tensor], skip: Optional[torch.Tensor],
-                   fir: Optional[torch.Tensor]) -> torch.Tensor:
-    return _RgbSkipMerge.apply(conv, bias, skip, fir)
+                   fir: Optional[torch.Tensor], parts: Optional[torch.Tensor] = None) -> torch.Tensor:
+    return _RgbSkipMerge.apply(conv, bias, skip, fir, parts)
```
